# jonassibbesen/rpvg

Measured on AMD Instinct MI355X. Metric: read-pairs quantified/sec, higher is better.
Workload: dtype f64

## Files before the change

include/rpvg_hip.h:

```cpp
#ifndef RPVG_HIP_H
#define RPVG_HIP_H

#include <stdint.h>

#include "rpvg_batch.h"
#include "rpvg_rows.h"
#include "rpvg_index.h"
#include "rpvg_table.h"
#include "rpvg_samples.h"
#include "rpvg_text.h"

#ifdef __cplusplus
extern "C" {
#endif

typedef enum rpvg_hip_status {
    RPVG_HIP_OK = 0,
    RPVG_HIP_ERR_NO_DEVICE = -1,
    RPVG_HIP_ERR_RUNTIME = -2,
    RPVG_HIP_ERR_INVALID = -3,
    RPVG_HIP_ERR_ALLOC = -4,
    RPVG_HIP_ERR_UNSUPPORTED = -5
} rpvg_hip_status;

// ... 354 lines not shown
int rpvg_hip_gibbs_table_view(rpvg_hip_ctx * ctx, rpvg_hip_gibbs_table * table, rpvg_gibbs_table_view * view_out);
int rpvg_hip_gibbs_table_rows(rpvg_hip_ctx * ctx, rpvg_hip_gibbs_table * table, uint64_t first_path, uint64_t num_paths, double * rows_out);
void rpvg_hip_gibbs_table_limits(rpvg_gibbs_table_limits * limits_out);
void rpvg_hip_gibbs_table_free(rpvg_hip_ctx * ctx, rpvg_hip_gibbs_table * table);
int rpvg_hip_gibbs_read_counts_resident(rpvg_hip_ctx * ctx, const rpvg_hip_batch * batch, const rpvg_hip_em_problems * problems,
                                        const double * init_abundances, const double * init_noise_count, const uint32_t * num_samples,
                                        const uint64_t * seeds, uint32_t gibbs_thin_its, double gamma, rpvg_hip_gibbs_samples ** samples_out);
int rpvg_hip_gibbs_samples_get(rpvg_hip_ctx * ctx, const rpvg_hip_gibbs_samples * samples, double * noise_samples, double * abundance_samples);
void rpvg_hip_gibbs_samples_free(rpvg_hip_ctx * ctx, rpvg_hip_gibbs_samples * samples);
int rpvg_hip_gibbs_table_build_resident(rpvg_hip_ctx * ctx, const rpvg_hip_gibbs_samples * samples, const rpvg_hip_em_problems * problems,
                                        uint32_t num_clusters, const uint64_t * cluster_path_off, const double * total_count,
                                        uint32_t num_gibbs_samples, rpvg_hip_gibbs_table ** table_out);

int rpvg_hip_gibbs_table_text(rpvg_hip_ctx * ctx, const rpvg_hip_gibbs_table * table, const rpvg_table_labels * labels, int32_t precision,
                              rpvg_hip_table_text ** text_out);
int rpvg_hip_estimates_table_text(rpvg_hip_ctx * ctx, const rpvg_hip_estimates_table * table, const rpvg_estimates_flat * estimates,
                                  const rpvg_table_labels * labels, int32_t kind, int32_t precision, rpvg_hip_table_text ** text_out);
int rpvg_hip_estimates_set_text(rpvg_hip_ctx * ctx, const rpvg_hip_estimates_table * table, const rpvg_estimates_flat * estimates,
                                const rpvg_table_labels * labels, int32_t kind, uint32_t ploidy, double min_posterior, int32_t precision,
                                rpvg_hip_table_text ** text_out);
int rpvg_hip_table_text_view(rpvg_hip_table_text * text, rpvg_table_text_view * view_out);
int rpvg_hip_table_text_get(rpvg_hip_table_text * text, uint64_t byte_begin, uint64_t byte_end, char * dst);
int rpvg_hip_table_text_guards(rpvg_hip_table_text * text, int32_t * intact_out);
void rpvg_hip_table_text_free(rpvg_hip_table_text * text);

#define RPVG_HIP_COMM_ID_BYTES 128
int rpvg_hip_comm_unique_id(uint8_t * id_out);
int rpvg_hip_comm_init(rpvg_hip_ctx * ctx, const uint8_t * id, int world_size, int rank);
int rpvg_hip_comm_destroy(rpvg_hip_ctx * ctx);
int rpvg_hip_comm_init_all(rpvg_hip_ctx * const * ctxs, int num_contexts);
int rpvg_hip_comm_allreduce_sum_f64(rpvg_hip_ctx * ctx, double * device_buf, uint64_t n);
int rpvg_hip_gather(rpvg_hip_ctx * ctx, const double * local_values, uint64_t local_count, const uint64_t * counts, double * all_values);

int rpvg_hip_synth_dense_cluster(rpvg_hip_ctx * ctx, uint64_t seed, uint64_t num_rows, uint32_t num_paths,
                                 double * device_matrix, uint64_t ld, double * device_counts);
int rpvg_hip_synth_dense_rows(rpvg_hip_ctx * ctx, uint64_t seed, uint64_t row_begin, uint64_t num_rows, uint32_t num_paths,
                              double * device_matrix, uint64_t ld, double * device_counts);

int rpvg_hip_synth_dense_cluster_batch(rpvg_hip_ctx * ctx, uint64_t seed, uint64_t num_rows, uint32_t num_paths,
                                       rpvg_hip_batch ** batch_out);

int rpvg_hip_debug_log(rpvg_hip_ctx * ctx, uint64_t n, const double * x, double * out, int32_t use_table);

#define RPVG_HIP_EM_KERNELS 12
typedef struct rpvg_hip_em_kernel_stats {
    double ms;
    uint64_t launches;
    uint64_t problems;
    uint64_t iterations;
    uint64_t max_iterations;
    double alg_bytes;
} rpvg_hip_em_kernel_stats;
const char * rpvg_hip_em_kernel_name(int index);

typedef struct rpvg_hip_kernel_stats {
    double em_sparse_ms;      uint64_t em_sparse_launches;   double em_sparse_alg_bytes;
    double em_dense_ms;       uint64_t em_dense_launches;    double em_dense_alg_bytes;
    double loglik_ms;         uint64_t loglik_launches;      double loglik_evals;
    double build_ms;          uint64_t build_launches;
    double h2d_ms;            double h2d_bytes;
    uint64_t em_iterations_total;
    double search_pairs_possible; double search_pairs_table; double search_pairs_kept;
    rpvg_hip_em_kernel_stats em_kernel[RPVG_HIP_EM_KERNELS];
    double collapse_ms;
    double busy_ms;
    double gibbs_ms;
    double search_tile_ms;    uint64_t search_tile_launches;
    uint64_t gibbs_calls_completed;
    uint64_t gibbs_count_grid_problems;
    uint64_t gibbs_count_grid_iterations;
    uint64_t cover_grid_problems;
    uint64_t cover_grid_rounds;
    uint64_t text_exact_cells;
    uint64_t nested_full_calls;
    uint64_t nested_full_sets;
    uint64_t nested_full_retained;
} rpvg_hip_kernel_stats;

int rpvg_hip_stats_get(rpvg_hip_ctx * ctx, rpvg_hip_kernel_stats * stats_out);
int rpvg_hip_stats_reset(rpvg_hip_ctx * ctx);
int rpvg_hip_stats_intervals(rpvg_hip_ctx * ctx, uint64_t capacity, double * start_ms, double * stop_ms, int32_t * family,
                             uint64_t * count_out);

#ifdef __cplusplus
}
#endif

#endif
```

rpvg_amd/csrc/bounded_search.hip:

```cpp

#include "common.hpp"
#include "search_plan.hpp"

#include <algorithm>
#include <cstdlib>
#include <map>
#include <memory>
#include <mutex>
#include <numeric>

using namespace rpvg_hip_detail;
using namespace rpvg_search;

namespace {
std::mutex g_search_gate_mutex;
const rpvg_hip_ctx * g_search_gate_owner = nullptr;
}

static bool searchLaunchesEarly() {
    static const bool early = RPVG_EXPERIMENT_ENV("RPVG_HIP_SEARCH_LAUNCH_EARLY") != nullptr;
    return early;
}

constexpr uint64_t kSearchGateRows = 1ull << 17;

static void searchGateEnter(rpvg_hip_ctx * ctx, hipStream_t stream, const uint64_t matrix_rows) {
    static const bool open_gate = RPVG_EXPERIMENT_ENV("RPVG_HIP_NO_SEARCH_GATE") != nullptr;
    ctx->search_gate_held = !open_gate && matrix_rows >= kSearchGateRows;
    if (!ctx->search_gate_held) return;
    hipEvent_t previous = nullptr;
    {
        std::lock_guard<std::mutex> lock(g_search_gate_mutex);
        if (g_search_gate_owner && g_search_gate_owner != ctx && g_search_gate_owner->device == ctx->device) {
            previous = g_search_gate_owner->search_done;
            (void) hipStreamWaitEvent(stream, previous, 0);
        }
    }
    if (previous && !searchLaunchesEarly()) (void) waitEvent(previous);
}

static void searchGateLeave(rpvg_hip_ctx * ctx, hipStream_t stream) {
    if (!ctx->search_gate_held) return;
    ctx->search_gate_held = false;
    std::lock_guard<std::mutex> lock(g_search_gate_mutex);
    (void) hipEventRecord(ctx->search_done, stream);
    g_search_gate_owner = ctx;
}

void searchGateForget(const rpvg_hip_ctx * ctx) {
    std::lock_guard<std::mutex> lock(g_search_gate_mutex);
    if (g_search_gate_owner == ctx) g_search_gate_owner = nullptr;
}

struct rpvg_hip_pair_posteriors {
    std::vector<uint64_t> pair_off;
    void * block = nullptr;
    bool block_pinned = false;
    const uint32_t * first = nullptr, * second = nullptr;
    const double * posterior = nullptr;
    ~rpvg_hip_pair_posteriors() {
        if (block && block_pinned) pinnedFree(block);
        else std::free(block);
    }
};

namespace {

constexpr uint32_t kLdsRows = 2048;
constexpr uint32_t kSmallRowLdsCols = 128;
constexpr uint32_t kRowLdsCols = 512;

__device__ __forceinline__ double waveSum(double v) { return waveSumF64(v); }

__device__ __forceinline__ double addLog(const double log_x, const double log_y) {
    return log_x > log_y ? log_x + log1p(exp(log_y - log_x)) : log_y + log1p(exp(log_x - log_y));
}


template <int kBlock, typename ValueFn>
__device__ __forceinline__ double blockLogSumExp(const uint32_t n, ValueFn value, double * scratch) {
    const double lowest = -1.7976931348623157e308;
    const int lane = threadIdx.x & 63, wave = threadIdx.x >> 6;
    double mx = lowest;
    for (uint32_t k = threadIdx.x; k < n; k += kBlock) mx = fmax(mx, value(k));
#pragma unroll
    for (int d = 32; d >= 1; d >>= 1) mx = fmax(mx, __shfl_xor(mx, d, 64));
    __syncthreads();
    if (lane == 0) scratch[wave] = mx;
    __syncthreads();
#pragma unroll
    for (int w2 = 0; w2 < kBlock / 64; ++w2) mx = fmax(mx, scratch[w2]);
    double sum = 0.0;
    for (uint32_t k = threadIdx.x; k < n; k += kBlock) {
        const double v = value(k);
        if (v > lowest) sum += exp(v - mx);
    }
    sum = waveSum(sum);
    __syncthreads();
    if (lane == 0) scratch[wave] = sum;
    __syncthreads();
    double total = 0.0;
#pragma unroll
    for (int w2 = 0; w2 < kBlock / 64; ++w2) total += scratch[w2];
    return (n == 0 || !(mx > lowest)) ? lowest : mx + log(total);
}

struct SearchArgs {
    const uint32_t * order;
    uint32_t count;
    GroupMatricesView g;
    const uint64_t * col_off;
    const uint32_t * col_count;
    const uint64_t * pair_cap_off;
    double min_log_likelihood_diff;
    uint32_t stage_rows;
    uint32_t row_lds_cols;
    double * log_freq;
    double * marginal;
    double * optimistic_raw;
    double * optimistic;
    uint32_t * col_order;
    uint32_t * out_first;
    uint32_t * out_second;
    double * out_value;
    uint32_t * out_count;
    unsigned long long * log_evals;
};

constexpr int kTileFirst = 4;

template <int kGroup>
__device__ __forceinline__ void tilePairSums(const LogTableEntry * lt, const double * lds_count, const double * lds_base, const uint32_t stride,
                                             const double * __restrict__ cnt, const double * __restrict__ nz,
                                             const double * const (&col_a)[kTileFirst], const double * __restrict__ col_b, const uint32_t staged,
// ... 803 lines not shown
}

int searchFailed(const hipError_t e) {
    setError("rpvg_hip_bounded_pair_posteriors: %s", hipGetErrorString(e));
    return (e == hipErrorOutOfMemory) ? RPVG_HIP_ERR_ALLOC : RPVG_HIP_ERR_RUNTIME;
}

void showSearchClasses(const rpvg_hip_groups * groups, const PairSearchPlan & plan) {
    const std::vector<uint32_t> & order = plan.order;
    const uint32_t M = static_cast<uint32_t>(order.size()), num_big = plan.num_big, num_medium = plan.num_medium;
    auto show = [&](const char * name, uint32_t first, uint32_t count) {
        double evals = 0;
        for (uint32_t i = first; i < first + count; ++i) evals += 0.5 * groups->h_num_rows[order[i]] * groups->h_num_cols[order[i]] * groups->h_num_cols[order[i]];
        std::fprintf(stderr, "[search classes] %-6s %6u matrices, %.3g pair-row evaluations if nothing is skipped; largest:", name, count, evals);
        for (uint32_t i = first; i < first + std::min<uint32_t>(count, 6); ++i) std::fprintf(stderr, " %llux%u", static_cast<unsigned long long>(groups->h_num_rows[order[i]]), groups->h_num_cols[order[i]]);
        std::fprintf(stderr, "\n");
    };
    show("table", 0, num_big);
    if (plan.pair_tiles) {
        struct Bucket { uint64_t matrices = 0; double rows = 0, evals = 0, lane_rows = 0, slot_rows = 0; };
        std::map<uint32_t, Bucket> buckets;
        for (uint32_t i = 0; i < num_big; ++i) {
            const double R = static_cast<double>(groups->h_num_rows[order[i]]);
            const uint32_t G = groups->h_num_cols[order[i]];
            uint32_t key = 1;
            while (key < G) key <<= 1;
            Bucket & b = buckets[key];
            const uint32_t tiles = tileCount(G);
            b.matrices += 1;
            b.rows += R;
            b.evals += R * (0.5 * G * (G + 1));
            std::vector<std::pair<uint32_t, uint32_t> > ranges;
            planTileRanges(tiles, &ranges);
            for (auto & range : ranges) b.lane_rows += R / (kTileBlock / range.second) * kTileBlock;
            b.slot_rows += R * tiles * 16;
        }
        for (auto & kv : buckets) {
            const Bucket & b = kv.second;
            std::fprintf(stderr, "[search classes]   columns <= %4u: %6llu matrices, %9.0f rows, %.3g evaluations, pairs / tile slots %.2f, tile slots / lane slots %.2f\n",
                         kv.first, static_cast<unsigned long long>(b.matrices), b.rows, b.evals, b.evals / b.slot_rows, b.slot_rows / (16.0 * b.lane_rows));
        }
    }
    show("medium", num_big, num_medium);
    show("small", num_big + num_medium, M - num_big - num_medium);
}

unsigned long long * searchLogEvals(const PairSearchWork & w) { return reinterpret_cast<unsigned long long *>(w.d_tail.ptr + w.evals_word); }

hipError_t launchTablePart(rpvg_hip_ctx * ctx, const rpvg_hip_groups * groups, const GroupMatricesView & view, const PairSearchPlan & plan,
                           PairSearchWork & w, const bool runs_behind_search) {
    hipError_t e = hipSuccess;
    auto ok = [&](hipError_t r) { if (e == hipSuccess) e = r; return e == hipSuccess; };
    hipStream_t st = ctx->stream;
    const SearchParts parts = {w.d_part_pair.ptr, w.d_part_marg.ptr, w.d_part_opt.ptr, w.d_big_pair_part_off.ptr, w.d_big_col_part_off.ptr, plan.chunk_rows};
    const uint32_t items = static_cast<uint32_t>(plan.item_matrix.size());
    if (plan.pair_tiles) {
        PairTileWork pw;
        pw.item_matrix = w.d_item_matrix.ptr;
        pw.item_chunk = w.d_item_chunk.ptr;
        pw.item_tiles = w.d_item_col.ptr;
        pw.count = items;
        pw.g = view;
        pw.parts = parts;
        pw.log_evals = searchLogEvals(w);
#ifdef RPVG_HIP_EXPERIMENTS
        pw.debug_skip = RPVG_EXPERIMENT_ENV("RPVG_HIP_PAIR_DEBUG") ? static_cast<uint32_t>(std::atoi(RPVG_EXPERIMENT_ENV("RPVG_HIP_PAIR_DEBUG"))) : 0u;
#endif
        static const size_t tile_lds_bytes = []() {
            const char * env = RPVG_EXPERIMENT_ENV("RPVG_HIP_PAIR_LDS_KB");
            return std::max<size_t>(kTileLdsDoubles * sizeof(double), env ? static_cast<size_t>(std::atoi(env)) * 1024 : 0);
        }();
        if (tile_lds_bytes > 64 * 1024) {
            e = hipFuncSetAttribute(reinterpret_cast<const void *>(&pairTile2Kernel), hipFuncAttributeMaxDynamicSharedMemorySize, static_cast<int>(tile_lds_bytes));
            if (e != hipSuccess) return e;
        }
        const int tile_span = ctx->spanBegin(FAM_TILE, st);
        pairTile2Kernel<<<dim3(pw.count), dim3(kTileBlock), tile_lds_bytes, st>>>(pw);
        ctx->spanEnd(tile_span);
#ifdef RPVG_HIP_EXPERIMENTS
        for (int k = RPVG_EXPERIMENT_ENV("RPVG_HIP_PAIR_REPEAT") ? std::atoi(RPVG_EXPERIMENT_ENV("RPVG_HIP_PAIR_REPEAT")) : 0; k > 0; --k) {
            pairTile2Kernel<<<dim3(pw.count), dim3(kTileBlock), tile_lds_bytes, st>>>(pw);
        }
#endif
    } else {
        TableWork tw;
        tw.item_matrix = w.d_item_matrix.ptr;
        tw.item_col = w.d_item_col.ptr;
        tw.item_chunk = w.d_item_chunk.ptr;
        tw.count = items;
        tw.g = view;
        tw.parts = parts;
        tw.log_evals = searchLogEvals(w);
        pairTableKernel<<<dim3(((tw.count + 7) / 8) * 8), dim3(256), 0, st>>>(tw);
    }
    if (runs_behind_search) {
        if (groups->collapse_done) {
            HostScope wait_scope("search: wait for the runs of the matrices' collapse");
            ok(searchLaunchesEarly() ? hipStreamWaitEvent(st, groups->collapse_done, 0) : waitEvent(groups->collapse_done));
        }
        ok(groups->held_back_runs(st, &parts));
        groups->held_back_runs = nullptr;
    }

    ResolveArgs ra;
    ra.big_matrix = w.d_order.ptr;
    ra.count = plan.num_big;
    ra.g = view;
    ra.col_off = w.d_col_off.ptr;
    ra.col_count = w.d_col_count.ptr;
    ra.pair_cap_off = w.d_pair_cap_off.ptr;
    ra.parts = parts;
    ra.min_log_likelihood_diff = w.min_log_likelihood_diff;
    ra.log_freq = w.d_lf.ptr;
    ra.marginal = w.d_marg.ptr;
    ra.col_order = w.d_col_order.ptr;
    ra.seq_value = w.d_seq.ptr;
    ra.out_first = w.d_out_first.ptr;
    ra.out_second = w.d_out_second.ptr;
    ra.out_value = w.d_out_value.ptr;
    ra.out_count = w.d_tail.ptr;
    resolveTableKernel<<<dim3(plan.num_big), dim3(256), 0, st>>>(ra);
    return e;
}

void launchSequentialParts(rpvg_hip_ctx * ctx, const GroupMatricesView & view, const PairSearchPlan & plan, PairSearchWork & w) {
    static const int search_streams = []() {
        const char * env = RPVG_EXPERIMENT_ENV("RPVG_HIP_SEARCH_STREAMS");
        return env ? std::max(1, std::min(3, std::atoi(env))) : 3;
    }();
    hipStream_t s_medium = search_streams == 1 ? ctx->stream : ctx->aux[0];
    hipStream_t s_small = search_streams == 1 ? ctx->stream : (search_streams == 2 ? ctx->aux[0] : ctx->aux[1]);
    SearchArgs args;
    args.g = view;
    args.col_off = w.d_col_off.ptr;
    args.col_count = w.d_col_count.ptr;
    args.pair_cap_off = w.d_pair_cap_off.ptr;
    args.min_log_likelihood_diff = w.min_log_likelihood_diff;
    args.log_freq = w.d_lf.ptr;
    args.marginal = w.d_marg.ptr;
    args.optimistic_raw = w.d_opt_raw.ptr;
    args.optimistic = w.d_opt.ptr;
    args.col_order = w.d_col_order.ptr;
    args.out_first = w.d_out_first.ptr;
    args.out_second = w.d_out_second.ptr;
    args.out_value = w.d_out_value.ptr;
    args.out_count = w.d_tail.ptr;
    args.log_evals = searchLogEvals(w);
    auto search_lds_bytes = [](uint32_t stage_rows, uint32_t row_cols) { return static_cast<size_t>((kTileFirst + 1) * stage_rows + kTileFirst * row_cols) * sizeof(double); };
    {
        static std::once_flag once;
        std::call_once(once, [&]() {
            (void) hipFuncSetAttribute(reinterpret_cast<const void *>(&boundedSearchKernel<1024, 64>), hipFuncAttributeMaxDynamicSharedMemorySize,
                                       static_cast<int>(search_lds_bytes(kLdsRows, kRowLdsCols)));
        });
    }
    const uint32_t num_small = w.M - plan.num_big - plan.num_medium;
    if (plan.num_medium > 0) {
        args.order = w.d_order.ptr + plan.num_big;
        args.count = plan.num_medium;
        args.stage_rows = kLdsRows;
        args.row_lds_cols = kRowLdsCols;
        boundedSearchKernel<1024, 64><<<dim3(plan.num_medium), dim3(1024), search_lds_bytes(kLdsRows, kRowLdsCols), s_medium>>>(args);
    }
    if (num_small > 0) {
        args.order = w.d_order.ptr + plan.num_big + plan.num_medium;
        args.count = num_small;
// ... 3 lines not shown
    }
}

}

namespace rpvg_hip_detail {

int queuePairSearch(rpvg_hip_ctx * ctx, const rpvg_hip_groups * groups, const uint32_t * column_counts, const double min_rel_likelihood,
                    PairSearchWork & w) {
    std::unique_ptr<HostScope> scope(new HostScope("bounded search: host order + work items"));
    const uint32_t M = groups->num_matrices;
    w.M = M;
    w.min_log_likelihood_diff = std::log(min_rel_likelihood);
    if (!column_counts && M > 0 && !groups->d_column_counts) {
        setError("rpvg_hip_bounded_pair_posteriors: column_counts is NULL");
        return RPVG_HIP_ERR_INVALID;
    }
    const uint64_t num_columns = std::accumulate(groups->h_num_cols.begin(), groups->h_num_cols.begin() + M, uint64_t(0));
    for (uint64_t c = 0; column_counts && c < num_columns; ++c) {
        if (column_counts[c] == 0) {
            setError("rpvg_hip_bounded_pair_posteriors: column %llu has a zero count", static_cast<unsigned long long>(c));
            return RPVG_HIP_ERR_INVALID;
        }
    }
    w.plan = planPairSearch(groups->h_num_rows.data(), groups->h_num_cols.data(), M, min_rel_likelihood, pairSearchKnobs());
    const PairSearchPlan & plan = w.plan;
    if (RPVG_EXPERIMENT_ENV("RPVG_HIP_SEARCH_CLASSES")) showSearchClasses(groups, plan);

    scope.reset(new HostScope("bounded search: uploads + launches"));
    hipError_t e = hipSetDevice(ctx->device);
    hipStream_t st = ctx->stream;
    auto ok = [&](hipError_t r) { if (e == hipSuccess) e = r; return e == hipSuccess; };

    UploadPack & pack = w.pack;
    const uint64_t columns = plan.col_off[M], pair_cap = plan.pair_cap_off[M];
    pack.add(w.d_order, plan.order.data(), M);
    pack.add(w.d_col_off, plan.col_off.data(), M + 1);
    pack.add(w.d_pair_cap_off, plan.pair_cap_off.data(), M + 1);
    if (column_counts) pack.add(w.d_col_count, column_counts, columns);
    if (plan.num_big > 0) {
        pack.add(w.d_item_matrix, plan.item_matrix.data(), plan.item_matrix.size());
        pack.add(w.d_item_col, plan.item_col.data(), plan.item_col.size());
        pack.add(w.d_item_chunk, plan.item_chunk.data(), plan.item_chunk.size());
        pack.add(w.d_big_col_part_off, plan.big_col_part_off.data(), M);
        pack.add(w.d_big_pair_part_off, plan.big_pair_part_off.data(), M);
    }
    w.evals_word = (M + 1) & ~1u;
    w.tail_words = w.evals_word + 4;
    pack.addZero(w.d_tail, w.tail_words);
    if (w.extra_u64_count) pack.add(w.d_extra_u64, w.extra_u64, w.extra_u64_count);
    if (w.extra_zero_bytes) pack.addZero(w.d_extra_zero, w.extra_zero_bytes);
    int span = ctx->spanBegin(FAM_H2D);
    ok(pack.commit(st));
    if (!column_counts) w.d_col_count.borrow(const_cast<uint32_t *>(groups->d_column_counts), columns);
    ctx->spanEnd(span);
    ctx->stats.h2d_bytes += static_cast<double>(M * 20 + columns * 4);
    ok(w.d_lf.alloc(columns));
    ok(w.d_marg.alloc(columns));
    ok(w.d_opt_raw.alloc(columns));
    ok(w.d_opt.alloc(columns));
    ok(w.d_col_order.alloc(columns));
    ok(w.d_out_first.alloc(pair_cap));
    ok(w.d_out_second.alloc(pair_cap));
    ok(w.d_out_value.alloc(pair_cap));
    if (e != hipSuccess) return searchFailed(e);
    if (plan.num_big > 0) {
        ok(w.d_part_marg.alloc(plan.col_part_total));
        ok(w.d_part_opt.alloc(plan.col_part_total));
        ok(w.d_part_pair.alloc(plan.pair_part_total));
        ok(w.d_seq.alloc(pair_cap));
    }
    if (e != hipSuccess) return searchFailed(e);

    const bool side_kernels = M > plan.num_big;
    const bool runs_behind_search = static_cast<bool>(groups->held_back_runs) && plan.pair_tiles && plan.num_big == M;
    if (!runs_behind_search) {
        ok(groups->waitCollapse(st));
        if (groups->collapse_done && !searchLaunchesEarly()) {
            HostScope wait_scope("search: wait for the collapse of the matrices");
            ok(waitEvent(groups->collapse_done));
        }
    }
    span = ctx->spanBegin(FAM_LOGLIK);
    searchGateEnter(ctx, st, std::accumulate(groups->h_num_rows.begin(), groups->h_num_rows.end(), uint64_t(0)));
    if (side_kernels) ok(ctx->forkAux());
    const GroupMatricesView view = groups->view();
    if (plan.num_big > 0) ok(launchTablePart(ctx, groups, view, plan, w, runs_behind_search && e == hipSuccess));
    launchSequentialParts(ctx, view, plan, w);
    if (side_kernels) ok(ctx->joinAux());
    ctx->spanEnd(span);
    ctx->stats.loglik_launches += (plan.num_big > 0 ? 2 : 0) + (plan.num_medium > 0) + (M > plan.num_big + plan.num_medium);
    ok(hipGetLastError());
    if (e != hipSuccess) {
        (void) hipStreamSynchronize(st);
        searchFailed(e);
        return RPVG_HIP_ERR_RUNTIME;
    }
    return RPVG_HIP_OK;
}

void leavePairSearch(rpvg_hip_ctx * ctx) { searchGateLeave(ctx, ctx->stream); }

void accountPairSearch(rpvg_hip_ctx * ctx, const rpvg_hip_groups * groups, const PairSearchWork & w, const unsigned long long log_evals,
                       const uint64_t kept_pairs) {
    ctx->stats.loglik_evals += static_cast<double>(log_evals);
    for (uint32_t i = 0; i < w.M; ++i) {
        const double G = groups->h_num_cols[w.plan.order[i]];
        ctx->stats.search_pairs_possible += G * (G + 1) / 2;
        if (i < w.plan.num_big) ctx->stats.search_pairs_table += G * (G + 1) / 2;
    }
    ctx->stats.search_pairs_kept += static_cast<double>(kept_pairs);
}

}

extern "C" int rpvg_hip_bounded_pair_posteriors(rpvg_hip_ctx * ctx, const rpvg_hip_groups * groups,
                                                const uint32_t * column_counts, double min_rel_likelihood,
                                                rpvg_hip_pair_posteriors ** result_out) {
    RPVG_REQUIRE(ctx && groups && result_out, "rpvg_hip_bounded_pair_posteriors: NULL argument");
    *result_out = nullptr;
    RPVG_REQUIRE(min_rel_likelihood > 0, "rpvg_hip_bounded_pair_posteriors: min_rel_likelihood must be positive");
    const uint32_t M = groups->num_matrices;
    rpvg_hip_pair_posteriors * res = new (std::nothrow) rpvg_hip_pair_posteriors();
    if (!res) {
        setError("rpvg_hip_bounded_pair_posteriors: out of host memory");
        return RPVG_HIP_ERR_ALLOC;
    }
    res->pair_off.assign(M + 1, 0);
    if (M == 0) {
        *result_out = res;
        return RPVG_HIP_OK;
    }
    if (!column_counts && !groups->d_column_counts) {
        delete res;
        setError("rpvg_hip_bounded_pair_posteriors: column_counts is NULL");
        return RPVG_HIP_ERR_INVALID;
    }

    std::lock_guard<std::mutex> lock(ctx->mutex);
    PairSearchWork w;
    {
        const int rc = queuePairSearch(ctx, groups, column_counts, min_rel_likelihood, w);
        if (rc != RPVG_HIP_OK) {
            delete res;
            return rc;
        }
    }
    hipError_t e = hipSuccess;
    hipStream_t st = ctx->stream;
    auto ok = [&](hipError_t r) { if (e == hipSuccess) e = r; return e == hipSuccess; };
    std::unique_ptr<HostScope> scope;
    const std::vector<uint64_t> & pair_cap_off = w.plan.pair_cap_off;
    const uint32_t evals_word = w.evals_word, tail_words = w.tail_words;
    auto & d_tail = w.d_tail; auto & d_pair_cap_off = w.d_pair_cap_off; auto & d_out_first = w.d_out_first;
    auto & d_out_second = w.d_out_second; auto & d_out_value = w.d_out_value;
    DeviceBuffer<uint64_t> d_pair_off;

    const char * with_counts_env = std::getenv("RPVG_HIP_PAIRS_WITH_COUNTS");
    const size_t kPairsWithTheCounts = with_counts_env ? static_cast<size_t>(std::atof(with_counts_env)) : (size_t(1) << 20);
    const size_t tail_bytes = tail_words * sizeof(uint32_t), tail_room = (tail_bytes + 255) & ~size_t(255);
    const size_t block_capacity = static_cast<size_t>(pair_cap_off[M]) * 16;
    const size_t first_copy = tail_room + std::min(block_capacity, kPairsWithTheCounts);
    DeviceBuffer<unsigned char> d_result;
    ok(d_pair_off.alloc(M + 1));
    ok(d_result.alloc(tail_room + block_capacity));
    void * host_result = nullptr;
    if (e == hipSuccess && pinnedAlloc(&host_result, first_copy) != hipSuccess) e = hipErrorOutOfMemory;
    if (e == hipSuccess) {
        const bool check_build = !groups->build_checked && groups->build_error_flag.ptr;
        pairOffsetsKernel<<<dim3(1), dim3(1024), 0, st>>>(M, d_tail.ptr, d_pair_off.ptr, check_build ? groups->build_error_flag.ptr : nullptr,
                                                         d_tail.ptr + evals_word + 2, reinterpret_cast<uint32_t *>(d_result.ptr), tail_words);
        compactPairsBlockKernel<<<dim3(M), dim3(64), 0, st>>>(M, d_pair_cap_off.ptr, d_pair_off.ptr, d_out_first.ptr, d_out_second.ptr,
                                                             d_out_value.ptr, d_result.ptr + tail_room);
        ok(hipGetLastError());
        ok(hipMemcpyAsync(host_result, d_result.ptr, first_copy, hipMemcpyDeviceToHost, st));
    }
    searchGateLeave(ctx, st);
    scope.reset(new HostScope("bounded search: wait for the kernels"));
    ok(waitStream(st));
    if (e == hipSuccess) {
        const uint32_t * counts = static_cast<const uint32_t *>(host_result);
        unsigned long long log_evals = 0;
        std::memcpy(&log_evals, counts + evals_word, sizeof(log_evals));
        const uint32_t build_bad = counts[evals_word + 2];
        for (uint32_t m = 0; m < M; ++m) res->pair_off[m + 1] = res->pair_off[m] + counts[m];
        if (build_bad) {
            pinnedFree(host_result);
            delete res;
            setError(build_bad == 2 ? "rpvg_hip_groups_build: a group lists a path twice" : "rpvg_hip_groups_build: a group refers to a path outside its cluster");
            return RPVG_HIP_ERR_INVALID;
        }
        groups->build_checked = true;
        const uint64_t total = res->pair_off[M];
        const unsigned char * pairs = nullptr;
        if (total * 16 <= first_copy - tail_room) {
            res->block = host_result;
            res->block_pinned = true;
            host_result = nullptr;
            pairs = static_cast<const unsigned char *>(res->block) + tail_room;
        } else {
            scope.reset(new HostScope("bounded search: download pairs"));
            if (pinnedAlloc(&res->block, total * 16) == hipSuccess) {
                res->block_pinned = true;
            } else {
                res->block = std::malloc(total * 16);
                if (!res->block) e = hipErrorOutOfMemory;
            }
            if (e == hipSuccess) {
                ok(hipMemcpyAsync(res->block, d_result.ptr + tail_room, total * 16, hipMemcpyDeviceToHost, st));
                ok(waitStream(st));
                pairs = static_cast<const unsigned char *>(res->block);
            }
        }
        if (e == hipSuccess) {
            res->posterior = reinterpret_cast<const double *>(pairs);
            res->first = reinterpret_cast<const uint32_t *>(pairs + total * sizeof(double));
            res->second = res->first + total;
        }
        accountPairSearch(ctx, groups, w, log_evals, total);
    }
    if (host_result) pinnedFree(host_result);
    if (e != hipSuccess) {
        delete res;
// ... 18 lines not shown
```

rpvg_amd/csrc/common.hpp:

```cpp
#ifndef RPVG_HIP_COMMON_HPP
#define RPVG_HIP_COMMON_HPP

#include <hip/hip_runtime.h>

#include <algorithm>
#include <chrono>
#include <cstdarg>
#include <cstdint>
#include <cstdio>
#include <cstdlib>
#include <cstring>
#include <memory>
#include <mutex>
#include <new>
#include <string>
#include <functional>
#include <vector>

#include "../../include/rpvg_hip.h"
#include "search_plan.hpp"
#include "em_plan.hpp"
#include "batch_forms.hpp"

namespace rpvg_hip_detail {

void setError(const char * fmt, ...);

#define RPVG_HIP_CHECK(expr)                                                                                  \
    do {                                                                                                      \
        hipError_t err__ = (expr);                                                                            \
        if (err__ != hipSuccess) {                                                                            \
            rpvg_hip_detail::setError("%s failed at %s:%d: %s", #expr, __FILE__, __LINE__, hipGetErrorString(err__)); \
               \
            (void) hipDeviceSynchronize();                                                                    \
            return RPVG_HIP_ERR_RUNTIME;                                                                      \
        }                                                                                                     \
    } while (0)

#define RPVG_REQUIRE(cond, ...)                       \
    do {                                              \
        if (!(cond)) {                                \
            rpvg_hip_detail::setError(__VA_ARGS__);   \
            return RPVG_HIP_ERR_INVALID;              \
        }                                             \
    } while (0)

#ifdef RPVG_HIP_EXPERIMENTS
#define RPVG_EXPERIMENT_ENV(name) std::getenv(name)
#else
#define RPVG_EXPERIMENT_ENV(name) (static_cast<const char *>(nullptr))
#endif

int hardwareQueues();

hipError_t waitEvent(hipEvent_t event);
hipError_t waitStream(hipStream_t stream);

hipError_t zeroAsync(void * ptr, size_t bytes, hipStream_t stream);

hipError_t poolAlloc(void ** ptr, size_t bytes);
void poolFree(void * ptr);
void poolTrim(int device);

hipError_t pinnedAlloc(void ** ptr, size_t bytes);
void pinnedFree(void * ptr);
size_t pinnedCapacity(const void * ptr);
void pinnedTrim();
bool stagedUploads();
bool hostIsPinned(const void * host, size_t bytes);
void copyToStaging(void * staging, const void * host, size_t bytes);
void registerCopyStream(hipStream_t stream, hipStream_t copy_stream, hipEvent_t copied);
void forgetCopyStream(hipStream_t stream);
hipError_t stagedCopy(void * device_dst, const void * pinned_src, size_t bytes, hipStream_t stream);

template <typename T>
struct DeviceBuffer {
    T * ptr = nullptr;
    size_t count = 0;
    void * staging = nullptr;
    bool borrowed = false;
    DeviceBuffer() {}
    DeviceBuffer(const DeviceBuffer &) = delete;
    DeviceBuffer & operator=(const DeviceBuffer &) = delete;
    ~DeviceBuffer() { release(); }
    void release() {
        if (ptr && !borrowed) poolFree(ptr);
        if (staging) pinnedFree(staging);
        ptr = nullptr;
        staging = nullptr;
        count = 0;
        borrowed = false;
    }
    hipError_t alloc(size_t n) {
        release();
        count = n;
        if (n == 0) return hipSuccess;
        return poolAlloc(reinterpret_cast<void **>(&ptr), n * sizeof(T));
    }
    void borrow(T * p, size_t n) {
        release();
        ptr = n ? p : nullptr;
        count = n;
        borrowed = true;
// ... 309 lines not shown
                                                  LogProduct (&pr)[kOut], double (&acc)[kOut]) {
    constexpr uint32_t kSegment = kGroup * kFoldFactors;
    for (IndexT seg = begin; seg < fast_end; seg += kSegment) {
        const IndexT seg_end = (fast_end - seg) < kSegment ? fast_end : seg + kSegment;
        for (IndexT i = seg + lane; i < seg_end; i += kGroup) {
            double xs[kOut];
            x(i, xs);
#pragma unroll
            for (int t = 0; t < kOut; ++t) pr[t].mul(xs[t]);
        }
#pragma unroll
        for (int t = 0; t < kOut; ++t) pr[t].fold();
    }
    for (IndexT i = (begin < fast_end ? fast_end : begin) + lane; i < mid_end; i += kGroup) {
        double xs[kOut];
        x(i, xs);
        const int c = static_cast<int>(cnt[i]);
        for (int k = 0; k < c; ++k) {
#pragma unroll
            for (int t = 0; t < kOut; ++t) pr[t].mul(xs[t]);
        }
#pragma unroll
        for (int t = 0; t < kOut; ++t) pr[t].fold();
    }
    for (IndexT i = (begin < mid_end ? mid_end : begin) + lane; i < end; i += kGroup) {
        double xs[kOut];
        x(i, xs);
        const double c = cnt[i];
#pragma unroll
        for (int t = 0; t < kOut; ++t) acc[t] = fma(c, logPositive(xs[t], lt), acc[t]);
    }
}

constexpr int kCollapseKeyFractionBits = 22;
constexpr int kCollapseProjectionBits = kCollapseKeyFractionBits + 2;
constexpr int kCollapseLargestBits = 20;
constexpr int kCollapseLargestFractionBits = 27;
constexpr int kCollapseMatrixShift = kCollapseProjectionBits + kCollapseLargestBits;
constexpr uint32_t kCollapseMaxMatrices = 1u << 20;

__host__ __device__ inline double collapseWeight(const uint32_t column) {
    return static_cast<double>(((column * 0x9E3779B1u) >> 8) & 0xFFFFu) * (1.0 / 32768.0);
}

__host__ __device__ inline uint64_t collapseSortKey(const uint32_t matrix, const double key, const double largest) {
    const double k = key < 0.0 ? 0.0 : (key > 3.999999 ? 3.999999 : key);
    const double l = largest < 0.0 ? 0.0 : (largest > 0.999999 ? 0.999999 : largest);
    return (static_cast<uint64_t>(matrix) << kCollapseMatrixShift) |
           (static_cast<uint64_t>(k * static_cast<double>(1ull << kCollapseKeyFractionBits)) << kCollapseLargestBits) |
           (static_cast<uint64_t>(l * static_cast<double>(1ull << kCollapseLargestFractionBits)) & ((1ull << kCollapseLargestBits) - 1));
}

__device__ __forceinline__ double mulRounded(const double a, const double b) {
#pragma clang fp contract(off)
    return a * b;
}
__device__ __forceinline__ double addRounded(const double a, const double b) {
#pragma clang fp contract(off)
    return a + b;
}

template <int BLOCK>
__device__ __forceinline__ uint32_t blockExclusiveSum(const uint32_t v, uint32_t & total, uint32_t * scratch) {
    const int lane = threadIdx.x & 63, wave = threadIdx.x >> 6;
    uint32_t incl = v;
#pragma unroll
    for (int d = 1; d < 64; d <<= 1) {
        const uint32_t up = __shfl_up(incl, d, 64);
        if (lane >= d) incl += up;
    }
    __syncthreads();
    if (lane == 63) scratch[wave] = incl;
    __syncthreads();
    uint32_t before = 0, all = 0;
#pragma unroll
    for (int w = 0; w < BLOCK / 64; ++w) {
        if (w < wave) before += scratch[w];
        all += scratch[w];
    }
    total = all;
    return before + incl - v;
}

enum KernelFamily { FAM_EM_SPARSE = 0, FAM_EM_DENSE, FAM_LOGLIK, FAM_BUILD, FAM_H2D, FAM_COLLAPSE, FAM_EM_KERNEL, FAM_GIBBS, FAM_TILE, FAM_COUNT };

struct TimedSpan {
    hipEvent_t start, stop;
    int family;
    int sub;
};

struct TimedInterval {
    double start_ms, stop_ms;
    int family;
    uint64_t clock;
};

}

namespace rpvg_hip_detail {
struct SubsetEmHints {
    double subsets_per_matrix = 0, list_per_path = 0, rows_per_row = 0, entries_per_entry = 0;
    bool retry = false;
    unsigned long long retry_subsets = 0, retry_list_length = 0, retry_rows = 0, retry_entries = 0;
};
}

struct rpvg_hip_ctx {
    static constexpr int kAuxStreams = 6;
    rpvg_hip_detail::SubsetEmHints subset_hints;
    rpvg_hip_detail::SubsetEmHints subset_full_hints;
    bool search_gate_held = false;
    int device = 0;
    hipStream_t stream = nullptr;
    hipStream_t aux[kAuxStreams] = {};
    int aux_count = kAuxStreams;
    hipStream_t grid_stream[2] = {nullptr, nullptr};
    hipEvent_t grid_ready = nullptr;
    hipStream_t collapse_stream = nullptr;
    hipStream_t copy_stream = nullptr;
    hipEvent_t copied = nullptr;
    hipEvent_t fork_event = nullptr;
    hipEvent_t search_done = nullptr;
    hipEvent_t join_event[kAuxStreams] = {};
    hipError_t forkAux();
    hipError_t joinAux();
    hipError_t joinAuxOnHost();
    hipDeviceProp_t props;
    std::mutex mutex;
    void * comm = nullptr;
    int comm_world = 1, comm_rank = 0;
    int allReduceSumF64(double * device_buf, uint64_t n);
    std::vector<rpvg_hip_detail::TimedSpan> spans;
    std::vector<hipStream_t> span_streams;
    int span_level = 2;
    int open_spans = 0;
    void accountSpan(const rpvg_hip_detail::TimedSpan & span, const void * clock_base, uint64_t clock_id);
    void foldFinishedSpans();
    std::vector<rpvg_hip_detail::TimedInterval> intervals;
    rpvg_hip_kernel_stats stats;
    rpvg_hip_independent_stats independent_stats{};
    rpvg_hip_detail::SubsetEmHints subset_independent_hints;

    int spanBegin(int family, hipStream_t on = nullptr, int sub = -1);
    void spanEnd(int idx);
    int foldSpans();
};

namespace rpvg_hip_detail {
struct PathSourcesPending {
    DeviceBuffer<uint64_t> d_path_source_off;
    DeviceBuffer<uint32_t> d_source_id, d_sizes;
    DeviceBuffer<uint16_t> d_source_id16;
    DeviceBuffer<unsigned long long> d_arena;
    unsigned long long arena_words = 0, num_sources = 0, num_sources_narrow = 0;
    void * h_sizes = nullptr;
    uint32_t K = 0;
    bool copied = false, queued = false;
    ~PathSourcesPending() { if (h_sizes) pinnedFree(h_sizes); }
};
}

struct rpvg_hip_batch {
    uint32_t num_clusters = 0;
    uint64_t num_rows = 0, num_entries = 0, num_paths = 0;
    std::vector<uint64_t> h_cluster_row_off, h_cluster_path_off, h_cluster_ent_off;
    rpvg_hip_detail::DeviceBuffer<uint64_t> cluster_row_off;
    rpvg_hip_detail::DeviceBuffer<uint64_t> cluster_path_off;
    rpvg_hip_detail::DeviceBuffer<double> row_count;
    rpvg_hip_detail::DeviceBuffer<double> row_noise;
    rpvg_hip_detail::DeviceBuffer<uint64_t> row_ent_off;
    rpvg_hip_detail::DeviceBuffer<uint32_t> ent_path;
    rpvg_hip_detail::DeviceBuffer<double> ent_prob;
    std::vector<double> h_cluster_total;
    bool has_source_columns = false;
    rpvg_hip_detail::DeviceBuffer<uint32_t> path_group_id;
    rpvg_hip_detail::DeviceBuffer<uint64_t> cluster_src_off;
    rpvg_hip_detail::DeviceBuffer<uint32_t> src_col_count;
    rpvg_hip_detail::DeviceBuffer<uint32_t> src_col_end;
    rpvg_hip_detail::DeviceBuffer<uint32_t> src_col_path;
    std::vector<uint64_t> h_cluster_src_off;
    std::vector<uint32_t> h_src_num_cols, h_src_col_paths, h_src_max_col_paths;
    struct UploadInProgress {
        rpvg_batch_forms::BatchForms forms;
        rpvg_hip_detail::DeviceBuffer<uint32_t> d_row_count_u32, d_row_grp_off32, d_grp_idx_off32;
        rpvg_hip_detail::DeviceBuffer<uint64_t> d_row_grp_off, d_grp_idx_off;
        rpvg_hip_detail::DeviceBuffer<double> d_grp_prob;
        rpvg_hip_detail::DeviceBuffer<uint8_t> d_row_grp_count8, d_grp_idx_count8;
        rpvg_hip_detail::DeviceBuffer<uint16_t> d_path_idx16, d_row_noise16;
        rpvg_hip_detail::DeviceBuffer<double> d_row_noise_table;
        rpvg_hip_detail::DeviceBuffer<uint8_t> d_row_count8;
        rpvg_hip_detail::DeviceBuffer<uint32_t> d_escape_row, d_escape_count;
        rpvg_hip_detail::PathSourcesPending path_sources;
        rpvg_hip_detail::DeviceBuffer<unsigned long long> d_first_bad_row;
        rpvg_hip_detail::DeviceBuffer<double> d_cluster_total;
        rpvg_hip_detail::DeviceBuffer<uint64_t> d_cluster_ent_off;
        rpvg_hip_detail::DeviceBuffer<unsigned char> scan_scratch_rows, scan_scratch_groups;
        void * h_results = nullptr;
        hipEvent_t finished = nullptr;
        ~UploadInProgress() {
            if (finished) {
                (void) hipEventSynchronize(finished);
                (void) hipEventDestroy(finished);
            }
            if (h_results) rpvg_hip_detail::pinnedFree(h_results);
        }
    };
    std::unique_ptr<UploadInProgress> upload;
};

void searchGateForget(const rpvg_hip_ctx * ctx);

struct GroupMatrix {
    const double * values, * rowmax, * row_count, * row_noise;
    uint64_t R, fast_end, mid_end;
    uint32_t G;
};
struct GroupMatricesView {
    const uint64_t * mat_val_off;
    const uint64_t * mat_row_off;
    const uint32_t * mat_fast;
    const uint32_t * mat_mid;
    const uint64_t * mat_rows;
    const uint32_t * mat_cols;
// ... 206 lines not shown
    uint32_t rows, entries;
    uint32_t merged, pad;
    uint64_t row_base, ent_base, col_begin;
    double total_mass, zero_mass;
};

struct EmGridStorage {
    EmProblemsView problems;
    double * abundances;
    double * noise_count;
    uint32_t * iterations;
    const EmFusedDense * fused = nullptr;
    uint32_t num_fused = 0;
};

uint64_t emGridMinWork();
uint64_t gibbsGridMinWork();
bool emGridDenseRoute(uint32_t columns, uint32_t rows, uint32_t entries);
int runEmGridProblems(rpvg_hip_ctx * ctx, hipStream_t st, const EmGridProblem * problems, uint32_t count, const EmGridStorage & storage,
                      uint32_t max_em_its, double max_rel_em_conv);

struct GibbsGridProblem {
    uint32_t problem, columns;
    uint32_t rows, entries;
    uint32_t num_samples, pad;
    uint64_t col_begin;
    uint64_t sample_off, abund_sample_off;
    uint64_t seed;
};
struct GibbsGridStorage {
    EmProblemsView problems;
    const double * init_abundances;
    const double * init_noise_count;
    double * noise_samples;
    double * abundance_samples;
};
int runGibbsGridProblems(rpvg_hip_ctx * ctx, hipStream_t st, const GibbsGridProblem * problems, uint32_t count, const GibbsGridStorage & storage,
                         uint32_t gibbs_thin_its, double gamma);

struct DenseEmRun {
    const double * matrix = nullptr;
    uint64_t num_rows = 0;
    uint32_t num_cols = 0;
    uint64_t ld = 0;
    const double * counts = nullptr;
    double total_count = 0, zero_mass = 0;
    uint32_t max_em_its = 0;
    double max_rel_em_conv = 0;
    bool sharded = false;
    DeviceBuffer<double> d_a;
    EmGridControl control = {};
};
int emDenseIterate(rpvg_hip_ctx * ctx, const char * who, DenseEmRun & run);

int queueEmSolve(rpvg_hip_ctx * ctx, const rpvg_hip_batch * batch, const EmProblemList & list, uint32_t max_em_its,
                 double max_rel_em_conv, const EmOutputs & out, EmSolveWork & work, double collapse_precision = 0.0);
EmSolveKnobs emSolveKnobs();
int queueEmFill(rpvg_hip_ctx * ctx, const rpvg_hip_batch * batch, const EmProblemList & list, const EmOutputs & out, EmSolveWork & work,
                const EmSolveKnobs & knobs, const EmFillPlan & plan, bool fused_look, int & build_span);
EmSolveShape emSolveShape(const rpvg_hip_ctx * ctx, const EmProblemList & list, bool collapse_wanted);

struct HostProblemSet {
    EmProblemList list;
    EmSolveWork work;
    DeviceBuffer<uint32_t> d_cluster, d_col_path, d_item_problem;
    DeviceBuffer<uint64_t> d_col_off, d_row_base, d_ent_base, d_seg_first;
    UploadPack uploads;
    uint64_t n_cols_total = 0;
};
int prepareHostProblems(rpvg_hip_ctx * ctx, const rpvg_hip_batch * batch, const rpvg_hip_em_problems * problems,
                        HostProblemSet & ps, const EmOutputs & out, const char * who);
void accountEmSolve(rpvg_hip_ctx * ctx, uint32_t P, const uint64_t * col_off, const uint32_t * kept_rows, const uint32_t * kept_entries,
                    const uint32_t * iterations);

struct PairSearchWork {
    uint32_t M = 0, evals_word = 0, tail_words = 0;
    double min_log_likelihood_diff = 0;
    rpvg_search::PairSearchPlan plan;
    DeviceBuffer<uint32_t> d_order, d_col_count, d_col_order, d_out_first, d_out_second, d_item_matrix, d_item_col, d_item_chunk;
    DeviceBuffer<uint32_t> d_tail;
    DeviceBuffer<uint64_t> d_col_off, d_pair_cap_off, d_big_col_part_off, d_big_pair_part_off;
    DeviceBuffer<double> d_lf, d_marg, d_opt_raw, d_opt, d_out_value, d_part_marg, d_part_opt, d_part_pair, d_seq;
    UploadPack pack;
    const uint64_t * extra_u64 = nullptr;
    size_t extra_u64_count = 0, extra_zero_bytes = 0;
    DeviceBuffer<uint64_t> d_extra_u64;
    DeviceBuffer<unsigned char> d_extra_zero;
};
int queuePairSearch(rpvg_hip_ctx * ctx, const rpvg_hip_groups * groups, const uint32_t * column_counts, double min_rel_likelihood,
                    PairSearchWork & w);
void leavePairSearch(rpvg_hip_ctx * ctx);
void accountPairSearch(rpvg_hip_ctx * ctx, const rpvg_hip_groups * groups, const PairSearchWork & w, unsigned long long log_evals, uint64_t kept_pairs);

struct CsrCollapseInput {
    uint32_t num_problems_bound = 0;
    const uint32_t * num_problems_dev = nullptr;
    uint64_t rows_capacity = 0;
    EmProblemsView problems;
    uint32_t num_items_bound = 0;
    const uint32_t * num_items_dev = nullptr;
    const uint64_t * seg_first = nullptr;
    const uint32_t * item_problem = nullptr;
    uint32_t segment_rows = 0;
    uint64_t max_rows_bound = 0;
};
struct CsrCollapseWork {
    DeviceBuffer<double> merged_count;
    DeviceBuffer<uint32_t> problem_merged;
    DeviceBuffer<uint32_t> info;
    std::shared_ptr<void> temporaries;
};
hipError_t queueCsrCollapse(rpvg_hip_ctx * ctx, const CsrCollapseInput & in, double precision, CsrCollapseWork & work, hipStream_t stream,
                            hipEvent_t sorted = nullptr);

std::unique_ptr<rpvg_hip_batch> newBatchShell(uint32_t num_clusters, uint64_t num_rows, uint64_t num_entries, uint64_t num_paths, hipError_t & e);
struct GroupedRows {
    uint64_t num_groups = 0;
    const void * row_grp_off = nullptr;
    const void * grp_idx_off = nullptr;
    bool row_off32 = false, grp_off32 = false;
    const double * grp_prob = nullptr;
    const uint32_t * row_count_u32 = nullptr;
};
hipError_t queueGroupedRows(hipStream_t stream, const GroupedRows & rows, rpvg_hip_batch * b, unsigned long long * d_first_bad_row, uint64_t * d_cluster_ent_off);

hipError_t queueClusterTotals(hipStream_t stream, uint32_t num_clusters, const uint64_t * d_cluster_row_off, const uint32_t * d_row_count_u32, double * d_totals);
hipError_t queuePathSourceCopies(rpvg_hip_ctx * ctx, rpvg_hip_batch * b, const rpvg_cluster_batch * hb, PathSourcesPending & pending);
hipError_t queuePathSourceKernels(rpvg_hip_ctx * ctx, rpvg_hip_batch * b, PathSourcesPending & pending, hipStream_t stream);
hipError_t reservePathSources(rpvg_hip_batch * b, uint32_t num_clusters, uint64_t num_paths, uint64_t num_sources, PathSourcesPending & pending);
int finishPathSources(rpvg_hip_batch * b, PathSourcesPending & pending);

hipError_t queueRowCollapse(rpvg_hip_ctx * ctx, rpvg_hip_groups * groups, uint64_t total_rows, double precision, hipStream_t stream, bool hold_back_runs = false);
}

#endif
```

rpvg_amd/csrc/context.hip:

```cpp

#include "common.hpp"

#include <sys/prctl.h>
#include <time.h>

#include <algorithm>
#include <thread>

#include <map>

namespace rpvg_hip_detail {

static thread_local char g_last_error[1024] = "";

void setError(const char * fmt, ...) {
    va_list ap;
    va_start(ap, fmt);
    vsnprintf(g_last_error, sizeof(g_last_error), fmt, ap);
    va_end(ap);
}

namespace {

struct DevicePool {
// ... 290 lines not shown

hipError_t rpvg_hip_ctx::joinAux() {
    hipError_t e = hipSuccess;
    for (int i = 0; i < aux_count && e == hipSuccess; ++i) {
        e = hipEventRecord(join_event[i], aux[i]);
        if (e == hipSuccess) e = hipStreamWaitEvent(stream, join_event[i], 0);
    }
    return e;
}

hipError_t rpvg_hip_ctx::joinAuxOnHost() {
    hipError_t e = hipSuccess;
    for (int i = 0; i < aux_count && e == hipSuccess; ++i) e = hipEventRecord(join_event[i], aux[i]);
    for (int i = 0; i < aux_count && e == hipSuccess; ++i) e = rpvg_hip_detail::waitEvent(join_event[i]);
    for (int i = 0; i < aux_count && e == hipSuccess; ++i) e = hipStreamWaitEvent(stream, join_event[i], 0);
    return e;
}

namespace rpvg_hip_detail {
namespace {
struct DeviceClock {
    hipEvent_t base = nullptr;
    uint64_t id = 0;
    std::chrono::steady_clock::time_point taken;
};
std::mutex g_clock_mutex;
std::map<int, DeviceClock> g_clocks;

DeviceClock deviceClock(const int device, hipStream_t stream, const bool renew_if_old) {
    std::lock_guard<std::mutex> lock(g_clock_mutex);
    DeviceClock & clock = g_clocks[device];
    const auto now = std::chrono::steady_clock::now();
    if (!clock.base || (renew_if_old && now - clock.taken > std::chrono::seconds(5))) {
        hipEvent_t base = nullptr;
        if (hipEventCreate(&base) == hipSuccess && hipEventRecord(base, stream) == hipSuccess && hipEventSynchronize(base) == hipSuccess) {
            clock.base = base;
            clock.id++;
            clock.taken = now;
        }
    }
    return clock;
}
}
}

int rpvg_hip_ctx::spanBegin(int family, hipStream_t on, int sub) {
    if (span_level <= 0 || (span_level == 1 && family != FAM_EM_KERNEL)) return -1;
    if (open_spans == 0 && spans.size() >= 1024) foldFinishedSpans();
    TimedSpan s;
    s.family = family;
    s.sub = sub;
    if (hipEventCreate(&s.start) != hipSuccess) return -1;
    if (hipEventCreate(&s.stop) != hipSuccess) {
        (void) hipEventDestroy(s.start);
        return -1;
    }
    if (!on) on = stream;
    (void) hipEventRecord(s.start, on);
    spans.push_back(s);
    span_streams.push_back(on);
    ++open_spans;
    return static_cast<int>(spans.size()) - 1;
}

void rpvg_hip_ctx::spanEnd(int idx) {
    if (idx < 0) return;
    (void) hipEventRecord(spans[idx].stop, span_streams[idx]);
    if (open_spans > 0) --open_spans;
}

void rpvg_hip_ctx::accountSpan(const rpvg_hip_detail::TimedSpan & s, const void * clock_base, const uint64_t clock_id) {
    constexpr size_t kMaxIntervals = 1u << 20;
    float ms = 0;
    if (hipEventElapsedTime(&ms, s.start, s.stop) != hipSuccess) return;
    switch (s.family) {
        case FAM_EM_SPARSE: stats.em_sparse_ms += ms; break;
        case FAM_EM_DENSE: stats.em_dense_ms += ms; break;
        case FAM_LOGLIK: stats.loglik_ms += ms; break;
        case FAM_BUILD: stats.build_ms += ms; break;
        case FAM_H2D: stats.h2d_ms += ms; break;
        case FAM_COLLAPSE: stats.collapse_ms += ms; break;
        case FAM_GIBBS: stats.gibbs_ms += ms; break;
        case FAM_TILE: stats.search_tile_ms += ms; stats.search_tile_launches += 1; break;
        case FAM_EM_KERNEL:
            if (s.sub >= 0 && s.sub < RPVG_HIP_EM_KERNELS) stats.em_kernel[s.sub].ms += ms;
            break;
        default: break;
    }
    float at = 0;
    hipEvent_t base = static_cast<hipEvent_t>(const_cast<void *>(clock_base));
    if (s.family != FAM_EM_KERNEL && s.family != FAM_GIBBS && base && intervals.size() < kMaxIntervals &&
        hipEventElapsedTime(&at, base, s.start) == hipSuccess) {
        intervals.push_back(TimedInterval{static_cast<double>(at), static_cast<double>(at) + ms, s.family, clock_id});
    }
}

void rpvg_hip_ctx::foldFinishedSpans() {
    const DeviceClock clock = deviceClock(device, stream, false);
    size_t kept = 0;
    for (size_t i = 0; i < spans.size(); ++i) {
        if (hipEventQuery(spans[i].stop) == hipSuccess) {
            accountSpan(spans[i], clock.base, clock.id);
            (void) hipEventDestroy(spans[i].start);
            (void) hipEventDestroy(spans[i].stop);
        } else {
            (void) hipGetLastError();
            spans[kept] = spans[i];
            span_streams[kept] = span_streams[i];
            ++kept;
        }
    }
    (void) hipGetLastError();
    spans.resize(kept);
    span_streams.resize(kept);
}

int rpvg_hip_ctx::foldSpans() {
    RPVG_HIP_CHECK(hipStreamSynchronize(stream));
    if (collapse_stream) RPVG_HIP_CHECK(hipStreamSynchronize(collapse_stream));
    const DeviceClock clock = deviceClock(device, stream, false);
    for (auto & s : spans) {
        (void) hipEventSynchronize(s.stop);
        accountSpan(s, clock.base, clock.id);
        (void) hipGetLastError();
        (void) hipEventDestroy(s.start);
        (void) hipEventDestroy(s.stop);
    }
    spans.clear();
    span_streams.clear();
    open_spans = 0;
    std::vector<std::pair<double, double>> iv;
    for (auto & t : intervals) {
        if (t.clock == clock.id) iv.emplace_back(t.start_ms, t.stop_ms);
    }
    std::sort(iv.begin(), iv.end());
    double busy = 0, cur_s = 0, cur_e = -1;
    for (auto & x : iv) {
        if (cur_e < cur_s || x.first > cur_e) {
            if (cur_e >= cur_s) busy += cur_e - cur_s;
            cur_s = x.first;
            cur_e = x.second;
        } else if (x.second > cur_e) {
            cur_e = x.second;
        }
    }
    if (cur_e >= cur_s) busy += cur_e - cur_s;
    stats.busy_ms = busy;
    return RPVG_HIP_OK;
}

extern "C" {

int rpvg_hip_device_count(int * count) {
    RPVG_REQUIRE(count != nullptr, "rpvg_hip_device_count: count is NULL");
    int n = 0;
    hipError_t e = hipGetDeviceCount(&n);
    if (e != hipSuccess) {
        setError("hipGetDeviceCount failed: %s", hipGetErrorString(e));
        *count = 0;
        return RPVG_HIP_ERR_NO_DEVICE;
    }
    *count = n;
    return RPVG_HIP_OK;
}

namespace {
hipError_t createMainStream(hipStream_t * stream, const bool highest_priority) {
    const char * env = RPVG_EXPERIMENT_ENV("RPVG_HIP_MAIN_PRIORITY");
    if (!highest_priority && (!env || std::atoi(env) == 0)) return hipStreamCreateWithFlags(stream, hipStreamNonBlocking);
    int least = 0, greatest = 0;
    if (hipDeviceGetStreamPriorityRange(&least, &greatest) != hipSuccess || least == greatest) {
        (void) hipGetLastError();
        return hipStreamCreateWithFlags(stream, hipStreamNonBlocking);
    }
    return hipStreamCreateWithPriority(stream, hipStreamNonBlocking, greatest);
}

bool ownQueueForMainStream(const bool uploader, const int side_streams) {
    static const bool pooled = std::getenv("RPVG_HIP_POOLED_MAIN_QUEUE") != nullptr && std::atoi(std::getenv("RPVG_HIP_POOLED_MAIN_QUEUE")) != 0;
    return !uploader && side_streams < rpvg_hip_ctx::kAuxStreams && !pooled;
}

hipError_t createOwnQueueStream(hipStream_t * stream, const int num_cus) {
    uint32_t every_cu[32];
    for (uint32_t & word : every_cu) word = 0xffffffffu;
    const uint32_t words = static_cast<uint32_t>(std::min(32, std::max(1, (num_cus + 31) / 32)));
    hipError_t e = hipExtStreamCreateWithCUMask(stream, words, every_cu);
    if (e != hipSuccess) {
        (void) hipGetLastError();
        e = hipStreamCreateWithFlags(stream, hipStreamNonBlocking);
    }
    return e;
}

int createContext(int device, bool uploader, int side_streams, rpvg_hip_ctx ** ctx_out);
}

int rpvg_hip_create(int device, rpvg_hip_ctx ** ctx_out) { return createContext(device, false, rpvg_hip_ctx::kAuxStreams, ctx_out); }

int rpvg_hip_create_uploader(int device, rpvg_hip_ctx ** ctx_out) { return createContext(device, true, 1, ctx_out); }

int rpvg_hip_create_with_streams(int device, int side_streams, rpvg_hip_ctx ** ctx_out) {
    RPVG_REQUIRE(side_streams >= 1 && side_streams <= rpvg_hip_ctx::kAuxStreams, "rpvg_hip_create_with_streams: 1 to %d side streams", rpvg_hip_ctx::kAuxStreams);
    return createContext(device, false, side_streams, ctx_out);
}

namespace {
int createContext(int device, const bool uploader, const int side_streams, rpvg_hip_ctx ** ctx_out) {
    RPVG_REQUIRE(ctx_out != nullptr, "rpvg_hip_create: ctx_out is NULL");
    *ctx_out = nullptr;
    int n = 0;
    hipError_t e = hipGetDeviceCount(&n);
    if (e != hipSuccess || n <= 0) {
        setError("rpvg_hip_create: no HIP device available (%s); this engine has no CPU fallback",
                 e != hipSuccess ? hipGetErrorString(e) : "device count is 0");
        return RPVG_HIP_ERR_NO_DEVICE;
    }
    RPVG_REQUIRE(device >= 0 && device < n, "rpvg_hip_create: device %d out of range [0, %d)", device, n);
    rpvg_hip_ctx * ctx = new (std::nothrow) rpvg_hip_ctx();
    if (!ctx) {
        setError("rpvg_hip_create: out of host memory");
        return RPVG_HIP_ERR_ALLOC;
    }
    ctx->device = device;
    memset(&ctx->stats, 0, sizeof(ctx->stats));
    {
        const char * env = std::getenv("RPVG_HIP_SPANS");
        ctx->span_level = env ? std::max(0, std::min(2, std::atoi(env))) : ((uploader || side_streams < rpvg_hip_ctx::kAuxStreams) ? 1 : 2);
    }
    if ((e = hipSetDevice(device)) != hipSuccess || (e = hipGetDeviceProperties(&ctx->props, device)) != hipSuccess ||
        (e = ownQueueForMainStream(uploader, side_streams) ? createOwnQueueStream(&ctx->stream, ctx->props.multiProcessorCount) : createMainStream(&ctx->stream, uploader)) != hipSuccess) {
        setError("rpvg_hip_create: %s", hipGetErrorString(e));
        delete ctx;
        return RPVG_HIP_ERR_RUNTIME;
    }
    ctx->aux_count = side_streams;
    for (int i = 0; i < rpvg_hip_ctx::kAuxStreams && e == hipSuccess; ++i) {
        if (i < side_streams) {
            e = hipStreamCreateWithFlags(&ctx->aux[i], hipStreamNonBlocking);
            if (e == hipSuccess) e = hipEventCreateWithFlags(&ctx->join_event[i], hipEventDisableTiming);
        } else {
            ctx->aux[i] = ctx->aux[i % side_streams];
        }
    }
    if (e == hipSuccess) e = createMainStream(&ctx->collapse_stream, RPVG_EXPERIMENT_ENV("RPVG_HIP_COLLAPSE_PRIORITY") == nullptr || std::atoi(RPVG_EXPERIMENT_ENV("RPVG_HIP_COLLAPSE_PRIORITY")) != 0);
    if (e == hipSuccess) e = hipEventCreateWithFlags(&ctx->fork_event, hipEventDisableTiming);
    if (e == hipSuccess) e = hipEventCreateWithFlags(&ctx->search_done, hipEventDisableTiming);
    if (e == hipSuccess) e = hipStreamCreateWithFlags(&ctx->copy_stream, hipStreamNonBlocking);
    if (e == hipSuccess) e = hipEventCreateWithFlags(&ctx->copied, hipEventDisableTiming);
    if (e == hipSuccess) {
        registerCopyStream(ctx->stream, ctx->copy_stream, ctx->copied);
        for (int i = 0; i < ctx->aux_count; ++i) registerCopyStream(ctx->aux[i], ctx->copy_stream, ctx->copied);
    }
    if (e != hipSuccess) {
        setError("rpvg_hip_create: %s", hipGetErrorString(e));
        delete ctx;
        return RPVG_HIP_ERR_RUNTIME;
    }
    if (strncmp(ctx->props.gcnArchName, "gfx950", 6) != 0) {
        setError("rpvg_hip_create: device %d is %s; this library is built for gfx950 only", device, ctx->props.gcnArchName);
        (void) hipStreamDestroy(ctx->stream);
        delete ctx;
        return RPVG_HIP_ERR_NO_DEVICE;
    }
    {
        std::lock_guard<std::mutex> lock(g_pool_mutex);
        g_device_contexts[device]++;
    }
    *ctx_out = ctx;
    return RPVG_HIP_OK;
}
}

void rpvg_hip_destroy(rpvg_hip_ctx * ctx) {
    if (!ctx) return;
    const bool trace = std::getenv("RPVG_AMD_TRACE_EXIT") != nullptr;
#define RPVG_EXIT_STEP(what) do { if (trace) std::fprintf(stderr, "[exit]   rpvg_hip_destroy: %s\n", what); } while (0)
    RPVG_EXIT_STEP("begin");
    (void) hipSetDevice(ctx->device);
    (void) ctx->foldSpans();
    RPVG_EXIT_STEP("spans folded");
    (void) rpvg_hip_comm_destroy(ctx);
    if (ctx->stream) forgetCopyStream(ctx->stream);
    for (int i = 0; i < ctx->aux_count; ++i) {
        if (ctx->aux[i]) forgetCopyStream(ctx->aux[i]);
    }
    if (ctx->copy_stream) {
        (void) hipStreamSynchronize(ctx->copy_stream);
        (void) hipStreamDestroy(ctx->copy_stream);
    }
    RPVG_EXIT_STEP("copy stream destroyed");
    if (ctx->copied) (void) hipEventDestroy(ctx->copied);
    if (ctx->stream) (void) hipStreamSynchronize(ctx->stream);
    for (int i = 0; i < ctx->aux_count; ++i) {
        if (ctx->aux[i]) (void) hipStreamSynchronize(ctx->aux[i]);
    }
    if (ctx->collapse_stream) (void) hipStreamSynchronize(ctx->collapse_stream);
    RPVG_EXIT_STEP("streams drained");
    for (int i = 0; i < ctx->aux_count; ++i) {
        if (ctx->aux[i]) (void) hipStreamDestroy(ctx->aux[i]);
        RPVG_EXIT_STEP("a side stream destroyed");
        if (ctx->join_event[i]) (void) hipEventDestroy(ctx->join_event[i]);
    }
    if (ctx->collapse_stream) (void) hipStreamDestroy(ctx->collapse_stream);
    RPVG_EXIT_STEP("side and collapse streams destroyed");
    if (ctx->stream) (void) hipStreamDestroy(ctx->stream);
    RPVG_EXIT_STEP("main stream destroyed");
    if (ctx->fork_event) (void) hipEventDestroy(ctx->fork_event);
    for (hipStream_t grid_stream : ctx->grid_stream) {
        if (grid_stream) {
            (void) hipStreamSynchronize(grid_stream);
            (void) hipStreamDestroy(grid_stream);
        }
    }
    if (ctx->grid_ready) (void) hipEventDestroy(ctx->grid_ready);
    searchGateForget(ctx);
    if (ctx->search_done) (void) hipEventDestroy(ctx->search_done);
    bool last = false;
    {
        std::lock_guard<std::mutex> lock(g_pool_mutex);
        last = (--g_device_contexts[ctx->device] <= 0);
    }
    RPVG_EXIT_STEP("events destroyed");
    if (last) {
        poolTrim(ctx->device);
        RPVG_EXIT_STEP("pool trimmed");
        bool any = false;
        {
            std::lock_guard<std::mutex> lock(g_pool_mutex);
            for (auto & kv : g_device_contexts) any = any || kv.second > 0;
        }
        if (!any) pinnedTrim();
        RPVG_EXIT_STEP("pinned blocks trimmed");
    }
    delete ctx;
    RPVG_EXIT_STEP("done");
#undef RPVG_EXIT_STEP
}

const char * rpvg_hip_last_error(void) { return g_last_error; }

int rpvg_hip_synchronize(rpvg_hip_ctx * ctx) {
    RPVG_REQUIRE(ctx != nullptr, "rpvg_hip_synchronize: ctx is NULL");
    std::lock_guard<std::mutex> lock(ctx->mutex);
    RPVG_HIP_CHECK(hipSetDevice(ctx->device));
    RPVG_HIP_CHECK(hipStreamSynchronize(ctx->stream));
    if (ctx->collapse_stream) RPVG_HIP_CHECK(hipStreamSynchronize(ctx->collapse_stream));
    return RPVG_HIP_OK;
}

int rpvg_hip_device_info(rpvg_hip_ctx * ctx, char * name, uint32_t name_cap, uint32_t * num_cus, uint64_t * mem_bytes) {
    RPVG_REQUIRE(ctx != nullptr, "rpvg_hip_device_info: ctx is NULL");
    if (name && name_cap) {
        snprintf(name, name_cap, "%s (%s)", ctx->props.name, ctx->props.gcnArchName);
    }
    if (num_cus) *num_cus = ctx->props.multiProcessorCount;
    if (mem_bytes) *mem_bytes = ctx->props.totalGlobalMem;
    return RPVG_HIP_OK;
}

int rpvg_hip_malloc(rpvg_hip_ctx * ctx, uint64_t bytes, void ** device_ptr_out) {
    RPVG_REQUIRE(ctx != nullptr && device_ptr_out != nullptr, "rpvg_hip_malloc: NULL argument");
    std::lock_guard<std::mutex> lock(ctx->mutex);
    RPVG_HIP_CHECK(hipSetDevice(ctx->device));
    hipError_t e = hipMalloc(device_ptr_out, bytes);
    if (e != hipSuccess) {
        setError("rpvg_hip_malloc: %llu bytes: %s", static_cast<unsigned long long>(bytes), hipGetErrorString(e));
        return RPVG_HIP_ERR_ALLOC;
    }
    return RPVG_HIP_OK;
}

int rpvg_hip_free(rpvg_hip_ctx * ctx, void * device_ptr) {
    RPVG_REQUIRE(ctx != nullptr, "rpvg_hip_free: ctx is NULL");
    std::lock_guard<std::mutex> lock(ctx->mutex);
    RPVG_HIP_CHECK(hipSetDevice(ctx->device));
    RPVG_HIP_CHECK(hipStreamSynchronize(ctx->stream));
    RPVG_HIP_CHECK(hipFree(device_ptr));
    return RPVG_HIP_OK;
}

int rpvg_hip_memcpy_h2d(rpvg_hip_ctx * ctx, void * device_dst, const void * host_src, uint64_t bytes) {
    RPVG_REQUIRE(ctx != nullptr, "rpvg_hip_memcpy_h2d: ctx is NULL");
    std::lock_guard<std::mutex> lock(ctx->mutex);
    RPVG_HIP_CHECK(hipSetDevice(ctx->device));
    RPVG_HIP_CHECK(hipMemcpyAsync(device_dst, host_src, bytes, hipMemcpyHostToDevice, ctx->stream));
    RPVG_HIP_CHECK(hipStreamSynchronize(ctx->stream));
    return RPVG_HIP_OK;
}

int rpvg_hip_memcpy_d2h(rpvg_hip_ctx * ctx, void * host_dst, const void * device_src, uint64_t bytes) {
    RPVG_REQUIRE(ctx != nullptr, "rpvg_hip_memcpy_d2h: ctx is NULL");
    std::lock_guard<std::mutex> lock(ctx->mutex);
    RPVG_HIP_CHECK(hipSetDevice(ctx->device));
    RPVG_HIP_CHECK(hipMemcpyAsync(host_dst, device_src, bytes, hipMemcpyDeviceToHost, ctx->stream));
    RPVG_HIP_CHECK(hipStreamSynchronize(ctx->stream));
    return RPVG_HIP_OK;
}

extern "C" int rpvg_hip_host_register(void * host, uint64_t bytes) {
    RPVG_REQUIRE(host && bytes > 0, "rpvg_hip_host_register: NULL or empty range");
    RPVG_HIP_CHECK(hipHostRegister(host, bytes, hipHostRegisterDefault));
    std::lock_guard<std::mutex> lock(g_registered_mutex);
    g_registered[static_cast<const char *>(host)] = bytes;
    return RPVG_HIP_OK;
}

extern "C" int rpvg_hip_host_unregister(void * host) {
    RPVG_REQUIRE(host, "rpvg_hip_host_unregister: NULL");
    {
        std::lock_guard<std::mutex> lock(g_registered_mutex);
        RPVG_REQUIRE(g_registered.erase(static_cast<const char *>(host)) == 1, "rpvg_hip_host_unregister: the range was not registered here");
    }
    RPVG_HIP_CHECK(hipHostUnregister(host));
    return RPVG_HIP_OK;
}

void rpvg_hip_thread_wait_spin_us(uint32_t microseconds) { t_spin_us = microseconds; }

int rpvg_hip_pinned_alloc(uint64_t bytes, void ** host_out) {
    RPVG_REQUIRE(host_out != nullptr, "rpvg_hip_pinned_alloc: host_out is NULL");
    *host_out = nullptr;
    const hipError_t e = pinnedAlloc(host_out, std::max<uint64_t>(bytes, 8));
    if (e != hipSuccess) {
        setError("rpvg_hip_pinned_alloc: %llu bytes: %s", static_cast<unsigned long long>(bytes), hipGetErrorString(e));
        return RPVG_HIP_ERR_ALLOC;
    }
    return RPVG_HIP_OK;
}

void rpvg_hip_pinned_free(void * host) { pinnedFree(host); }

int rpvg_hip_stats_get(rpvg_hip_ctx * ctx, rpvg_hip_kernel_stats * stats_out) {
    RPVG_REQUIRE(ctx != nullptr && stats_out != nullptr, "rpvg_hip_stats_get: NULL argument");
    std::lock_guard<std::mutex> lock(ctx->mutex);
    RPVG_HIP_CHECK(hipSetDevice(ctx->device));
    int rc = ctx->foldSpans();
    if (rc != RPVG_HIP_OK) return rc;
    *stats_out = ctx->stats;
    return RPVG_HIP_OK;
}

int rpvg_hip_stats_reset(rpvg_hip_ctx * ctx) {
    RPVG_REQUIRE(ctx != nullptr, "rpvg_hip_stats_reset: ctx is NULL");
    std::lock_guard<std::mutex> lock(ctx->mutex);
    RPVG_HIP_CHECK(hipSetDevice(ctx->device));
    int rc = ctx->foldSpans();
    if (rc != RPVG_HIP_OK) return rc;
    memset(&ctx->stats, 0, sizeof(ctx->stats));
    ctx->independent_stats = rpvg_hip_independent_stats{};
    ctx->intervals.clear();
    (void) deviceClock(ctx->device, ctx->stream, true);
    return RPVG_HIP_OK;
}

int rpvg_hip_stats_intervals(rpvg_hip_ctx * ctx, uint64_t capacity, double * start_ms, double * stop_ms, int32_t * family,
                             uint64_t * count_out) {
    RPVG_REQUIRE(ctx != nullptr && count_out != nullptr, "rpvg_hip_stats_intervals: NULL argument");
    std::lock_guard<std::mutex> lock(ctx->mutex);
    RPVG_HIP_CHECK(hipSetDevice(ctx->device));
    int rc = ctx->foldSpans();
    if (rc != RPVG_HIP_OK) return rc;
    const DeviceClock clock = deviceClock(ctx->device, ctx->stream, false);
    uint64_t n = 0;
    for (auto & t : ctx->intervals) {
        if (t.clock != clock.id) continue;
        if (n < capacity) {
            if (start_ms) start_ms[n] = t.start_ms;
            if (stop_ms) stop_ms[n] = t.stop_ms;
            if (family) family[n] = t.family;
        }
        ++n;
    }
    *count_out = n;
    return RPVG_HIP_OK;
}

}
```

rpvg_amd/csrc/subset_em.hip:

```cpp

#include "common.hpp"
#include "subset_pack.hpp"

#include <cmath>
#include <memory>

using namespace rpvg_hip_detail;

namespace {

constexpr uint32_t kMaxSelected = 1024;

struct MergedList {
    const uint32_t * a;
    const uint32_t * b;
    uint32_t na, nb, i, j;
    __device__ __forceinline__ MergedList(const uint32_t * a_in, uint32_t na_in, const uint32_t * b_in, uint32_t nb_in)
        : a(a_in), b(b_in), na(na_in), nb(nb_in), i(0), j(0) {}
    __device__ __forceinline__ bool done() const { return i >= na && j >= nb; }
    __device__ __forceinline__ uint32_t next() {
        if (j >= nb || (i < na && a[i] <= b[j])) return a[i++];
        return b[j++];
    }
};
// ... 472 lines not shown
    }
    if (tid == 0) set_count[m] = Q;
}

}


static int nestedSubsetEmAttempt(rpvg_hip_ctx * ctx, const rpvg_hip_batch * batch, const rpvg_hip_groups * groups,
                                 const uint32_t * column_counts, double min_rel_likelihood, double min_hap_prob,
                                 uint32_t max_em_its, double max_rel_em_conv, double collapse_precision,
                                 rpvg_hip_subset_em ** result_out, bool * did_not_fit, PairSearchWork & search, const bool second_attempt) {
    *did_not_fit = false;
    RPVG_REQUIRE(min_rel_likelihood > 0, "rpvg_hip_nested_subset_em: min_rel_likelihood must be positive");
    RPVG_REQUIRE(max_em_its > 0, "rpvg_hip_nested_subset_em: max_em_its must be positive");
    RPVG_REQUIRE(groups->batch == batch, "rpvg_hip_nested_subset_em: the matrices were built on another batch");
    const uint32_t M = groups->num_matrices;
    RPVG_REQUIRE(M == 0 || column_counts || groups->d_column_counts, "rpvg_hip_nested_subset_em: column_counts is NULL");
    std::unique_ptr<rpvg_hip_subset_em> res(new (std::nothrow) rpvg_hip_subset_em());
    if (!res) {
        setError("rpvg_hip_nested_subset_em: out of host memory");
        return RPVG_HIP_ERR_ALLOC;
    }
    res->num_matrices = M;

    const bool disabled = std::getenv("RPVG_HIP_NO_DEVICE_SUBSETS") != nullptr;
    if (disabled || !(min_hap_prob * kMaxSelected >= 1.0)) {
        setError("rpvg_hip_nested_subset_em: not taken (min_hap_prob %g admits more than %u subsets per cluster, or RPVG_HIP_NO_DEVICE_SUBSETS)",
                 min_hap_prob, kMaxSelected);
        return RPVG_HIP_ERR_UNSUPPORTED;
    }
    std::unique_ptr<HostScope> scope(new HostScope("subset em: bounds"));
    uint64_t slots = 0, lane_rows = 0, lane_entries = 0, lane_paths = 0, max_cluster_work = 0;
    uint32_t max_paths = 0;
    std::vector<uint64_t> slot_off(M + 1, 0);
    for (uint32_t m = 0; m < M; ++m) {
        const uint64_t G = groups->h_num_cols[m];
        slot_off[m + 1] = slot_off[m] + std::min<uint64_t>(G * (G + 1) / 2, kMaxSelected);
        const uint32_t k = groups->h_cluster[m];
        lane_rows += batch->h_cluster_row_off[k + 1] - batch->h_cluster_row_off[k];
        lane_entries += batch->h_cluster_ent_off[k + 1] - batch->h_cluster_ent_off[k];
        lane_paths += groups->h_num_paths[m];
        max_paths = std::max(max_paths, groups->h_num_paths[m]);
        max_cluster_work = std::max<uint64_t>(max_cluster_work, (batch->h_cluster_row_off[k + 1] - batch->h_cluster_row_off[k]) +
                                                                    (batch->h_cluster_ent_off[k + 1] - batch->h_cluster_ent_off[k]));
    }
    slots = slot_off[M];
    if (M > 0 && 8ull * (5ull * (static_cast<uint64_t>(max_paths) + 1) + 6) > 156 * 1024) {
        setError("rpvg_hip_nested_subset_em: not taken (a cluster with %u paths: EM vectors in global memory)", max_paths);
        return RPVG_HIP_ERR_UNSUPPORTED;
    }

    std::lock_guard<std::mutex> lock(ctx->mutex);
    RPVG_HIP_CHECK(hipSetDevice(ctx->device));
    hipStream_t st = ctx->stream;
    if (M == 0) {
        *result_out = res.release();
        return RPVG_HIP_OK;
    }
    SubsetEmHints & hints = ctx->subset_hints;
    auto planned = [](const double per_unit, const unsigned long long units, const double headroom) {
        return static_cast<unsigned long long>(std::ceil(per_unit * headroom * static_cast<double>(units)));
    };
    unsigned long long cap_subsets = std::min<unsigned long long>(slots, hints.subsets_per_matrix > 0 ? planned(hints.subsets_per_matrix, M, 1.25) + 256 : std::max<unsigned long long>(8ull * M, 16384));
    unsigned long long cap_length = std::max<unsigned long long>(planned(hints.list_per_path, lane_paths, 2.0), std::max<unsigned long long>(8 * lane_paths, 1u << 20));
    unsigned long long cap_rows = hints.rows_per_row > 0 ? planned(hints.rows_per_row, lane_rows, 1.25) + 65536 : 8 * lane_rows;
    unsigned long long cap_entries = hints.entries_per_entry > 0 ? planned(hints.entries_per_entry, lane_entries, 1.25) + 65536 : 8 * lane_entries;
    if (hints.retry) {
        cap_subsets = std::min<unsigned long long>(slots, std::max(cap_subsets, hints.retry_subsets + 64));
        cap_length = std::max(cap_length, hints.retry_list_length + 64);
        cap_rows = std::max(cap_rows, hints.retry_rows + 64);
        cap_entries = std::max(cap_entries, hints.retry_entries + 64);
        hints.retry = false;
    }
    const unsigned long long cap_columns = cap_length;
    const unsigned long long cap_items = cap_rows / emFillSegmentRows() + cap_subsets;

    scope.reset(new HostScope("subset em: search + kernels queued"));
    const size_t header_room = 256;
    int rc = RPVG_HIP_OK;
    if (!second_attempt) {
        search.extra_u64 = slot_off.data();
        search.extra_u64_count = M + 1;
        search.extra_zero_bytes = header_room + emQueuesBytes();
        rc = queuePairSearch(ctx, groups, column_counts, min_rel_likelihood, search);
        if (rc != RPVG_HIP_OK) return rc;
    } else {
        const hipError_t zeroed = zeroAsync(search.d_extra_zero.ptr, search.extra_zero_bytes, st);
        if (zeroed != hipSuccess) {
            setError("rpvg_hip_nested_subset_em: %s", hipGetErrorString(zeroed));
            return RPVG_HIP_ERR_RUNTIME;
        }
    }

    hipError_t e = hipSuccess;
    auto ok = [&](hipError_t r) { if (e == hipSuccess) e = r; return e == hipSuccess; };
    const uint64_t * d_slot_off = search.d_extra_u64.ptr;
    SubsetHeader * header = reinterpret_cast<SubsetHeader *>(search.d_extra_zero.ptr);
    static_assert(sizeof(SubsetHeader) <= 256, "room for the header");
    DeviceBuffer<uint32_t> d_slot_first, d_slot_second, d_slot_length, d_slot_columns;
    DeviceBuffer<double> d_slot_weight;
    DeviceBuffer<unsigned char> d_totals, d_bases, d_packed;
    ok(d_slot_first.alloc(slots));
    ok(d_slot_second.alloc(slots));
    ok(d_slot_length.alloc(slots));
    ok(d_slot_columns.alloc(slots));
    ok(d_slot_weight.alloc(slots));
    ok(d_totals.alloc(sizeof(MatrixTotals) * M));
    ok(d_bases.alloc(sizeof(MatrixTotals) * M));
    DeviceBuffer<uint32_t> d_big_matrices;
    ok(d_big_matrices.alloc(M));
    DeviceBuffer<uint32_t> d_sub_cluster, d_path, d_col_path, d_iters, d_kept_rows, d_kept_entries;
    DeviceBuffer<double> d_sub_weight, d_abund, d_noise, d_total;
    DeviceBuffer<uint64_t> d_path_off, d_col_off, d_row_base, d_ent_base, d_subset_off, d_seg_first;
    DeviceBuffer<uint32_t> d_item_problem;
    ok(d_sub_cluster.alloc(cap_subsets));
    ok(d_sub_weight.alloc(cap_subsets));
    ok(d_path_off.alloc(cap_subsets + 1));
    ok(d_col_off.alloc(cap_subsets + 1));
    ok(d_row_base.alloc(cap_subsets));
    ok(d_ent_base.alloc(cap_subsets));
    ok(d_subset_off.alloc(M + 1));
    ok(d_seg_first.alloc(cap_subsets + 1));
    ok(d_item_problem.alloc(cap_items));
    ok(d_path.alloc(cap_length));
    ok(d_col_path.alloc(cap_columns));
    ok(d_abund.alloc(cap_columns));
    ok(d_noise.alloc(cap_subsets));
    ok(d_total.alloc(cap_subsets));
    ok(d_iters.alloc(cap_subsets));
    ok(d_kept_rows.alloc(cap_subsets));
    ok(d_kept_entries.alloc(cap_subsets));
    const size_t packed_capacity = packedLayout(M, cap_subsets, cap_length, cap_columns).bytes;
    ok(d_packed.alloc(packed_capacity));
    const bool merge_here = batch->path_group_id.ptr != nullptr && max_paths < (1u << kMergePathBits) - 2;
    DeviceBuffer<unsigned long long> d_merge_key;
    DeviceBuffer<uint32_t> d_merge_pos;
    DeviceBuffer<double> d_merge_a0, d_merge_a1;
    if (merge_here) {
        ok(d_merge_key.alloc(2 * cap_length + 2));
        ok(d_merge_pos.alloc(2 * cap_length + 2));
        ok(d_merge_a0.alloc(cap_length));
        ok(d_merge_a1.alloc(cap_length));
    }
    void * pinned_header = nullptr;
    if (e == hipSuccess && pinnedAlloc(&pinned_header, sizeof(SubsetHeader)) != hipSuccess) e = hipErrorOutOfMemory;
    hipEvent_t header_here = nullptr;
    if (e == hipSuccess) ok(hipEventCreateWithFlags(&header_here, hipEventDisableTiming));
    if (e != hipSuccess) {
        setError("rpvg_hip_nested_subset_em: %s", hipGetErrorString(e));
        (void) hipStreamSynchronize(st);
        leavePairSearch(ctx);
        if (pinned_header) pinnedFree(pinned_header);
        if (header_here) (void) hipEventDestroy(header_here);
        return (e == hipErrorOutOfMemory) ? RPVG_HIP_ERR_ALLOC : RPVG_HIP_ERR_RUNTIME;
    }
    MatrixTotals * totals = reinterpret_cast<MatrixTotals *>(d_totals.ptr);
    MatrixTotals * bases = reinterpret_cast<MatrixTotals *>(d_bases.ptr);

    std::unique_ptr<HostScope> part_scope(new HostScope("subset em: select + offsets + expand queued"));
    int span = ctx->spanBegin(FAM_BUILD);
    SelectArgs sa;
    sa.num_matrices = M;
    sa.pair_count = search.d_tail.ptr;
    sa.pair_cap_off = search.d_pair_cap_off.ptr;
    sa.pair_first = search.d_out_first.ptr;
    sa.pair_second = search.d_out_second.ptr;
    sa.pair_value = search.d_out_value.ptr;
    sa.group_off = groups->d_group_off;
    sa.group_path_off = groups->d_group_path_off;
    sa.group_path = groups->d_group_path;
    sa.cluster = groups->d_cluster;
    sa.mat_rows = groups->mat_rows.ptr;
    sa.cluster_row_off = batch->cluster_row_off.ptr;
    sa.row_ent_off = batch->row_ent_off.ptr;
    sa.slot_off = d_slot_off;
    sa.min_hap_prob = min_hap_prob;
    sa.segment_rows = emFillSegmentRows();
    sa.slot_first = d_slot_first.ptr;
    sa.slot_second = d_slot_second.ptr;
    sa.slot_weight = d_slot_weight.ptr;
    sa.slot_length = d_slot_length.ptr;
    sa.slot_columns = d_slot_columns.ptr;
    sa.totals = totals;
    sa.header = header;
    sa.big_matrices = d_big_matrices.ptr;
    subsetSelectSmallKernel<<<dim3(M), dim3(64), 0, st>>>(sa);
    subsetSelectWideKernel<<<dim3(std::min<uint32_t>(M, 128)), dim3(256), 0, st>>>(sa);
    const bool check_build = !groups->build_checked && groups->build_error_flag.ptr;
    OffsetsArgs oa;
    oa.pair_count = search.d_tail.ptr;
    oa.log_evals = reinterpret_cast<const unsigned long long *>(search.d_tail.ptr + search.evals_word);
    oa.build_error = check_build ? groups->build_error_flag.ptr : nullptr;
    oa.num_matrices = M;
    oa.totals = totals;
    oa.bases = bases;
    oa.header = header;
    oa.cap_subsets = cap_subsets;
    oa.cap_length = cap_length;
    oa.cap_columns = cap_columns;
    oa.cap_rows = cap_rows;
    oa.cap_entries = cap_entries;
    oa.cap_items = cap_items;
    oa.seg_first = d_seg_first.ptr;
    oa.path_off = d_path_off.ptr;
    oa.col_off = d_col_off.ptr;
    subsetOffsetsKernel<<<dim3(1), dim3(1024), 0, st>>>(oa);
    SubsetHeader * h_header = static_cast<SubsetHeader *>(pinned_header);
    ok(hipMemcpyAsync(h_header, header, sizeof(SubsetHeader), hipMemcpyDeviceToHost, st));
    ok(hipEventRecord(header_here, st));
    ExpandArgs ea;
    ea.num_matrices = M;
    ea.header = header;
    ea.totals = totals;
    ea.bases = bases;
    ea.slot_off = d_slot_off;
    ea.slot_first = d_slot_first.ptr;
    ea.slot_second = d_slot_second.ptr;
    ea.slot_weight = d_slot_weight.ptr;
    ea.slot_length = d_slot_length.ptr;
    ea.slot_columns = d_slot_columns.ptr;
    ea.group_off = groups->d_group_off;
    ea.group_path_off = groups->d_group_path_off;
    ea.group_path = groups->d_group_path;
    ea.cluster = groups->d_cluster;
    ea.cluster_row_off = batch->cluster_row_off.ptr;
    ea.row_ent_off = batch->row_ent_off.ptr;
    ea.sub_cluster = d_sub_cluster.ptr;
    ea.sub_weight = d_sub_weight.ptr;
    ea.path_off = d_path_off.ptr;
    ea.path = d_path.ptr;
    ea.col_off = d_col_off.ptr;
    ea.col_path = d_col_path.ptr;
    ea.row_base = d_row_base.ptr;
    ea.ent_base = d_ent_base.ptr;
    ea.seg_first = d_seg_first.ptr;
    ea.item_problem = d_item_problem.ptr;
    ea.segment_rows = emFillSegmentRows();
    ea.subset_off = d_subset_off.ptr;
    subsetExpandKernel<<<dim3(M), dim3(256), 0, st>>>(ea);
    ok(hipGetLastError());
    ctx->spanEnd(span);
    ctx->stats.build_launches += 4;
    leavePairSearch(ctx);

    part_scope.reset();
    EmProblemList list;
    list.P_bound = static_cast<uint32_t>(std::min<unsigned long long>(cap_subsets, 0xfffffffeull));
    list.d_num_problems = &header->num_problems;
    list.d_cluster = d_sub_cluster.ptr;
    list.d_col_off = d_col_off.ptr;
    list.d_col_path = d_col_path.ptr;
    list.d_row_base = d_row_base.ptr;
    list.d_ent_base = d_ent_base.ptr;
    list.rows_capacity = cap_rows;
    list.entries_capacity = cap_entries;
    list.d_seg_first = d_seg_first.ptr;
    list.d_item_problem = d_item_problem.ptr;
    list.items_bound = static_cast<uint32_t>(std::min<unsigned long long>(cap_items, 0xfffffffeull));
    list.d_num_items = &header->num_items;
    list.max_cols = max_paths + 1;
    list.max_cluster_paths = max_paths;
    list.max_cluster_work = max_cluster_work;
    list.wide_capacity = 0;
    EmOutputs out{d_abund.ptr, d_noise.ptr, d_iters.ptr, d_kept_rows.ptr, d_kept_entries.ptr, d_total.ptr};
    EmSolveWork work;
    work.zeroed_queues = search.d_extra_zero.ptr + header_room;
    if (e == hipSuccess) {
        rc = queueEmSolve(ctx, batch, list, max_em_its, max_rel_em_conv, out, work, collapse_precision);
        if (rc != RPVG_HIP_OK) {
            (void) hipStreamSynchronize(st);
            (void) hipEventDestroy(header_here);
            pinnedFree(pinned_header);
            return rc;
        }
    }
    part_scope.reset(new HostScope("subset em: merge + pack queued"));
    static_assert(sizeof(SubsetHeader) <= 192, "the merge's flag word sits behind the header");
    uint32_t * d_merge_bad = reinterpret_cast<uint32_t *>(search.d_extra_zero.ptr + 192);
    if (merge_here && e == hipSuccess) {
        MergeArgs ma;
        ma.header = header;
        ma.num_matrices = M;
        ma.subset_off = d_subset_off.ptr;
        ma.weight = d_sub_weight.ptr;
        ma.path_off = d_path_off.ptr;
        ma.path = d_path.ptr;
        ma.col_off = d_col_off.ptr;
        ma.col_path = d_col_path.ptr;
        ma.abundances = d_abund.ptr;
        ma.noise = d_noise.ptr;
        ma.total = d_total.ptr;
        ma.cluster = groups->d_cluster;
        ma.cluster_path_off = batch->cluster_path_off.ptr;
        ma.path_group_id = batch->path_group_id.ptr;
        ma.sort_key = d_merge_key.ptr;
        ma.sort_pos = d_merge_pos.ptr;
        ma.rec_a0 = d_merge_a0.ptr;
        ma.rec_a1 = d_merge_a1.ptr;
        ma.merge_bad = d_merge_bad;
        ma.packed = d_packed.ptr;
        const int merge_span = ctx->spanBegin(FAM_BUILD);
        subsetMergeKernel<<<dim3(M), dim3(256), 0, st>>>(ma);
        ctx->spanEnd(merge_span);
        ctx->stats.build_launches += 1;
    }
    PackArgs pa;
    pa.merge_bad = merge_here ? d_merge_bad : nullptr;
    pa.header = header;
    pa.num_matrices = M;
    pa.subset_off = d_subset_off.ptr;
    pa.weight = d_sub_weight.ptr;
    pa.path_off = d_path_off.ptr;
    pa.col_off = d_col_off.ptr;
    pa.abundances = d_abund.ptr;
    pa.noise = d_noise.ptr;
    pa.total = d_total.ptr;
    pa.path = d_path.ptr;
    pa.col_path = d_col_path.ptr;
    pa.iterations = d_iters.ptr;
    pa.kept_rows = d_kept_rows.ptr;
    pa.kept_entries = d_kept_entries.ptr;
    pa.packed = d_packed.ptr;
// ... 121 lines not shown
```

rpvg_amd/engine.py:

```python
from __future__ import annotations

import ctypes as C
import os
from typing import List, NamedTuple, Optional, Tuple

import numpy as np

from . import hip
from .batch import CClusterBatch, CEstimatesView, CParams, ClusterBatch, ClusterEstimates, decode_view

_HERE = os.path.dirname(os.path.abspath(__file__))
LIB_PATH = os.path.join(_HERE, "host", "librpvg_amd_harness.so")

MODELS = ("transcripts", "strains", "haplotype-transcripts", "haplotypes")

_lib = None


def lib() -> C.CDLL:
    global _lib
    if _lib is None:
        if not os.path.exists(LIB_PATH):
            raise hip.EngineError(f"{LIB_PATH} is missing: build it with __graft_entry__.build() (there is no CPU fallback)")
        hip.lib()
        L = C.CDLL(LIB_PATH)
        L.rpvg_amd_last_error.restype = C.c_char_p
        L.rpvg_amd_engine_create.restype = C.c_void_p
        L.rpvg_amd_engine_create.argtypes = [C.c_int]
        L.rpvg_amd_engine_create_uploader.restype = C.c_void_p
        L.rpvg_amd_engine_create_uploader.argtypes = [C.c_int]
        L.rpvg_amd_engine_destroy.argtypes = [C.c_void_p]
        L.rpvg_amd_engine_ctx.restype = C.c_void_p
        L.rpvg_amd_engine_ctx.argtypes = [C.c_void_p]
        L.rpvg_amd_engine_stats_get.argtypes = [C.c_void_p, C.c_void_p]
        L.rpvg_amd_engine_stats_reset.argtypes = [C.c_void_p]
        L.rpvg_amd_engine_independent_stats_get.argtypes = [C.c_void_p, C.c_void_p]
        L.rpvg_amd_run_generators_after.restype = C.c_int
        L.rpvg_amd_run_generators_after.argtypes = [C.c_void_p, C.c_void_p, C.c_char_p, C.POINTER(CParams), C.POINTER(C.c_uint32)]
        L.rpvg_amd_host_threads.restype = C.c_int
        L.rpvg_amd_batch_prepare.restype = C.c_void_p
        L.rpvg_amd_batch_prepare.argtypes = [C.c_void_p, C.POINTER(CClusterBatch), C.c_int]
        L.rpvg_amd_batch_free.argtypes = [C.c_void_p]
        L.rpvg_amd_batch_reupload.argtypes = [C.c_void_p, C.c_void_p, C.POINTER(CClusterBatch), C.POINTER(C.c_double)]
        L.rpvg_amd_batch_prepare_from_alignments.restype = C.c_void_p
        L.rpvg_amd_batch_prepare_from_alignments.argtypes = [C.c_void_p, C.c_void_p, C.POINTER(CClusterBatch), C.c_double, C.c_double,
                                                             C.c_double, C.c_uint32, C.c_int, C.c_double, C.c_double,
                                                             C.POINTER(C.c_double)]
        L.rpvg_amd_batch_prepare_from_alignments_fit.restype = C.c_void_p
        L.rpvg_amd_batch_prepare_from_alignments_fit.argtypes = [C.c_void_p, C.c_void_p, C.POINTER(CClusterBatch), C.c_void_p, C.c_uint32, C.c_int,
                                                                 C.c_void_p, C.c_double, C.c_double, C.POINTER(hip.CFragLengthFit),
                                                                 C.c_void_p, C.POINTER(C.c_double)]
        L.rpvg_amd_batch_prepare_from_alignments_fitted.restype = C.c_void_p
        L.rpvg_amd_batch_prepare_from_alignments_fitted.argtypes = [C.c_void_p, C.c_void_p, C.POINTER(CClusterBatch), C.c_double, C.c_double,
                                                                    C.c_double, C.c_double, C.c_double, C.POINTER(C.c_double)]
        L.rpvg_amd_batch_prepare_from_fragments.restype = C.c_void_p
        L.rpvg_amd_batch_prepare_from_fragments.argtypes = [C.c_void_p, C.c_void_p, C.c_uint32, C.c_void_p, C.c_void_p, C.c_void_p, C.c_uint64,
                                                            C.POINTER(CClusterBatch), C.c_double, C.c_double, C.c_double, C.c_uint32,
                                                            C.c_double, C.c_double, C.c_void_p, C.c_void_p, C.c_void_p, C.c_void_p,
                                                            C.POINTER(C.c_double)]
        L.rpvg_amd_batch_prepare_from_fragments_table.restype = C.c_void_p
        L.rpvg_amd_batch_prepare_from_fragments_table.argtypes = [C.c_void_p, C.c_void_p, C.c_uint32, C.c_void_p, C.c_void_p, C.c_void_p, C.c_uint64,
                                                                  C.c_void_p, C.c_int, C.c_double, C.c_double, C.c_double, C.c_uint32,
                                                                  C.c_double, C.c_double, C.c_void_p, C.c_void_p, C.c_void_p, C.c_void_p,
                                                                  C.POINTER(C.c_double)]
        L.rpvg_amd_batch_has_source_columns.restype = C.c_int
        L.rpvg_amd_batch_has_source_columns.argtypes = [C.c_void_p]
        L.rpvg_amd_batch_prepare_synth_dense.restype = C.c_void_p
        L.rpvg_amd_batch_prepare_synth_dense.argtypes = [C.c_void_p, C.c_uint64, C.c_uint64, C.c_uint32]
        L.rpvg_amd_run.restype = C.c_void_p
        L.rpvg_amd_run.argtypes = [C.c_void_p, C.c_void_p, C.c_char_p, C.POINTER(CParams), C.POINTER(C.c_double)]
        L.rpvg_amd_run_team.restype = C.c_int
        L.rpvg_amd_run_team.argtypes = [C.c_void_p, C.c_void_p, C.c_char_p, C.POINTER(CParams), C.c_int, C.POINTER(C.c_double)]
        L.rpvg_amd_run_team_result.restype = C.c_void_p
        L.rpvg_amd_run_team_result.argtypes = [C.c_void_p]
        L.rpvg_amd_run_inplace.restype = C.c_int
        L.rpvg_amd_run_inplace.argtypes = [C.c_void_p, C.c_void_p, C.c_char_p, C.POINTER(CParams), C.POINTER(C.c_double)]
        L.rpvg_amd_run_from_alignments_inplace.restype = C.c_int
        L.rpvg_amd_run_from_alignments_inplace.argtypes = [C.c_void_p, C.c_void_p, C.c_char_p, C.POINTER(CParams), C.POINTER(C.c_double),
                                                           C.POINTER(C.c_double)]
        L.rpvg_amd_group_create.restype = C.c_void_p
        L.rpvg_amd_group_create.argtypes = [C.POINTER(C.c_int), C.c_int]
        L.rpvg_amd_group_destroy.argtypes = [C.c_void_p]
        L.rpvg_amd_group_has_communicator.argtypes = [C.c_void_p]
        L.rpvg_amd_group_run.restype = C.c_void_p
        L.rpvg_amd_group_run.argtypes = [C.c_void_p, C.POINTER(CClusterBatch), C.c_char_p, C.POINTER(CParams), C.POINTER(C.c_double)]
        L.rpvg_amd_group_partition.argtypes = [C.c_void_p, C.c_void_p, C.c_uint64]
        L.rpvg_amd_group_gather.argtypes = [C.c_void_p, C.c_void_p, C.c_uint64, C.POINTER(C.c_uint64), C.POINTER(C.c_double)]
        L.rpvg_amd_pipeline_create.restype = C.c_void_p
        L.rpvg_amd_pipeline_create.argtypes = [C.c_int, C.c_char_p, C.POINTER(CParams), C.c_int]
        L.rpvg_amd_pipeline_destroy.argtypes = [C.c_void_p]
        L.rpvg_amd_pipeline_workers.argtypes = [C.c_void_p]
        L.rpvg_amd_pipeline_prepare_slots.argtypes = [C.c_void_p, C.POINTER(CClusterBatch), C.c_int]
        L.rpvg_amd_pipeline_submit.argtypes = [C.c_void_p, C.POINTER(CClusterBatch), C.c_int]
        L.rpvg_amd_pipeline_prepare_slot.argtypes = [C.c_void_p, C.POINTER(CClusterBatch), C.c_int]
        L.rpvg_amd_pipeline_wait.argtypes = [C.c_void_p]
        L.rpvg_amd_pipeline_result.restype = C.c_void_p
        L.rpvg_amd_pipeline_result.argtypes = [C.c_void_p, C.c_int]
        L.rpvg_amd_pipeline_stats_get.argtypes = [C.c_void_p, C.c_void_p, C.POINTER(C.c_double)]
        L.rpvg_amd_pipeline_stats_reset.argtypes = [C.c_void_p]
        L.rpvg_amd_pipeline_completions.argtypes = [C.c_void_p, C.c_void_p, C.c_uint64, C.POINTER(C.c_uint64)]
        L.rpvg_amd_result_view.argtypes = [C.c_void_p, C.POINTER(CEstimatesView)]
        L.rpvg_amd_result_free.argtypes = [C.c_void_p]
        _lib = L
    return _lib


class FragLengthFit(NamedTuple):
    loc: float
    scale: float
    shape: float
    max_length: int
    valid: bool
    stats: dict


def _fit_tuple(fit) -> FragLengthFit:
    return FragLengthFit(fit.loc, fit.scale, fit.shape, fit.max_length, bool(fit.valid),
                         dict(sample_size=fit.sample_size, iterations=fit.iterations, evaluations=fit.evaluations))


def _err() -> str:
    return lib().rpvg_amd_last_error().decode()


class Engine:

    def __init__(self, device: int = 0, uploader: bool = False):
        self.handle = lib().rpvg_amd_engine_create_uploader(device) if uploader else lib().rpvg_amd_engine_create(device)
        if not self.handle:
            raise hip.EngineError(f"engine create failed: {_err()}")

    def close(self):
        if self.handle:
            lib().rpvg_amd_engine_destroy(self.handle)
            self.handle = None

    def __del__(self):
        try:
            self.close()
        except Exception:
            pass

    def _ctx(self):
        return C.c_void_p(lib().rpvg_amd_engine_ctx(self.handle))

    def stats(self) -> dict:
        s = hip.CKernelStats()
        if lib().rpvg_amd_engine_stats_get(self.handle, C.byref(s)) != 0:
            raise hip.EngineError(f"stats failed: {_err()}")
        return s.as_dict()

    def independent_stats(self) -> dict:
        s = hip.CIndependentStats()
        if lib().rpvg_amd_engine_independent_stats_get(self.handle, C.byref(s)) != 0:
            raise hip.EngineError(f"stats failed: {_err()}")
        return {n: int(getattr(s, n)) for n, _ in s._fields_}

    def reset_stats(self):
        if lib().rpvg_amd_engine_stats_reset(self.handle) != 0:
            raise hip.EngineError(f"stats reset failed: {_err()}")

    def info(self) -> Tuple[str, int, int]:
        name = C.create_string_buffer(256)
        cus, mem = C.c_uint32(0), C.c_uint64(0)
        hip._check(hip.lib().rpvg_hip_device_info(self._ctx(), name, 256, C.byref(cus), C.byref(mem)), "rpvg_hip_device_info")
        return name.value.decode(), cus.value, mem.value

    def prepare(self, batch: ClusterBatch, per_cluster: bool = False) -> "PreparedBatch":
        return PreparedBatch(self, batch, per_cluster)

    def fit_frag_length(self, counts, skew_normal: bool = True) -> FragLengthFit:
        return _fit_tuple(hip.frag_length_fit(self._ctx(), counts, skew_normal))

    def effective_lengths(self, path_lengths, frag) -> np.ndarray:
        return hip.effective_lengths(self._ctx(), path_lengths, float(frag[0]), float(frag[1]), float(frag[2]))

    def prepare_from_alignments(self, alignments, path_info: ClusterBatch, frag=None, is_single_end: bool = False,
                                min_noise_prob: float = 1e-4, prob_precision: float = 1e-8, frag_counts=None, path_lengths=None,
                                skew_normal: bool = True) -> "PreparedBatch":
        if frag is not None and frag_counts is not None:
            raise ValueError("prepare_from_alignments: frag and frag_counts exclude each other")
        if (frag_counts is None) != (path_lengths is None):
            raise ValueError("prepare_from_alignments: frag_counts and path_lengths come together")
        if frag_counts is not None and is_single_end:
            raise ValueError("prepare_from_alignments: a single-end run has no fragment lengths to fit")
        prep = PreparedBatch.__new__(PreparedBatch)
        prep.engine = self
        prep.batch = path_info
        ca, cb = alignments.as_c(), path_info.as_c()
        secs = C.c_double(0)
        if frag_counts is not None:
            counts = np.ascontiguousarray(frag_counts, dtype=np.uint32)
            lengths = np.ascontiguousarray(path_lengths, dtype=np.uint32)
            if lengths.size != len(alignments.path_effective_length):
                raise ValueError("prepare_from_alignments: one path length per path")
            fit = hip.CFragLengthFit()
            eff = np.zeros(lengths.size, dtype=np.float64)
            prep.handle = lib().rpvg_amd_batch_prepare_from_alignments_fit(
                self.handle, C.byref(ca), C.byref(cb), C.c_void_p(counts.ctypes.data if counts.size else None), counts.size,
                1 if skew_normal else 0, C.c_void_p(lengths.ctypes.data if lengths.size else None), min_noise_prob, prob_precision,
                C.byref(fit), C.c_void_p(eff.ctypes.data if eff.size else None), C.byref(secs))
            if not prep.handle:
                raise hip.EngineError(f"batch prepare from alignments failed: {_err()}")
            prep.frag_fit = _fit_tuple(fit)
            prep.path_effective_length = eff
            prep.row_construction_seconds = secs.value
            return prep
        if isinstance(frag, FragLengthFit):
            if is_single_end or not frag.valid:
                raise ValueError("prepare_from_alignments: a fitted distribution must be valid and belongs to a paired-end run")
            prep.handle = lib().rpvg_amd_batch_prepare_from_alignments_fitted(
                self.handle, C.byref(ca), C.byref(cb), frag.loc, frag.scale, frag.shape, min_noise_prob, prob_precision, C.byref(secs))
            if not prep.handle:
                raise hip.EngineError(f"batch prepare from alignments failed: {_err()}")
            prep.row_construction_seconds = secs.value
            return prep
        if frag is None:
            frag = (300.0, 50.0, 0.0, 10)
        prep.handle = lib().rpvg_amd_batch_prepare_from_alignments(
            self.handle, C.byref(ca), C.byref(cb), frag[0], frag[1], frag[2], int(frag[3]), 1 if is_single_end else 0,
            min_noise_prob, prob_precision, C.byref(secs))
        if not prep.handle:
            raise hip.EngineError(f"batch prepare from alignments failed: {_err()}")
        prep.row_construction_seconds = secs.value
        return prep

    def prepare_from_fragments(self, chunks, index_params, path_info: Optional[ClusterBatch] = None, extra_sets=None, frag=None,
                               min_noise_prob: float = 1e-4, prob_precision: float = 1e-8, path_table=None,
                               collapse_names: bool = False) -> "PreparedBatch":
        from . import index as index_mod
        if (path_table is None) == (path_info is None):
            raise ValueError("prepare_from_fragments: either path_info or path_table")
        if collapse_names and (path_table is None or path_table.name_id is None):
            raise ValueError("prepare_from_fragments: collapse_names needs a path_table with name_id")
        chunks = list(chunks)
        cchunks = (index_mod.CFragmentLists * max(len(chunks), 1))(*[c.as_c() for c in chunks])
        cparams = index_params.as_c()
        sets = list(extra_sets or [])
        off = np.zeros(len(sets) + 1, dtype=np.uint64)
# ... 121 lines not shown
            raise hip.EngineError(f"group run({model}) failed: {_err()}")
        try:
            view = CEstimatesView()
            lib().rpvg_amd_result_view(h, C.byref(view))
            out = decode_view(view)
        finally:
            lib().rpvg_amd_result_free(h)
        self.num_clusters = batch.num_clusters
        return out, secs.value

    def partition(self):
        import numpy as np
        out = np.zeros(self.num_clusters, dtype=np.uint32)
        if lib().rpvg_amd_group_partition(self.handle, C.c_void_p(out.ctypes.data), self.num_clusters) != 0:
            raise hip.EngineError(f"group partition failed: {_err()}")
        return out

    def gather(self, capacity: int):
        import numpy as np
        out = np.zeros(max(1, capacity), dtype=np.float64)
        count, total = C.c_uint64(0), C.c_double(0)
        if lib().rpvg_amd_group_gather(self.handle, C.c_void_p(out.ctypes.data), capacity, C.byref(count), C.byref(total)) != 0:
            raise hip.EngineError(f"group gather failed: {_err()}")
        return out[:count.value].copy(), total.value


class Pipeline:

    def __init__(self, model: str, params: CParams, device: int = 0, workers: int = 0):
        self.handle = lib().rpvg_amd_pipeline_create(device, model.encode(), C.byref(params), workers)
        if not self.handle:
            raise hip.EngineError(f"pipeline create failed: {_err()}")
        self._keep = []

    @property
    def workers(self) -> int:
        return int(lib().rpvg_amd_pipeline_workers(self.handle))

    def prepare_slots(self, batch: ClusterBatch, slots: int):
        cb = batch.as_c()
        if lib().rpvg_amd_pipeline_prepare_slots(self.handle, C.byref(cb), slots) != 0:
            raise hip.EngineError(f"pipeline prepare failed: {_err()}")

    def prepare_slot(self, slot: int, part):
        cb = part.as_c(True)
        if lib().rpvg_amd_pipeline_prepare_slot(self.handle, C.byref(cb), slot) != 0:
            raise hip.EngineError(f"pipeline prepare failed: {_err()}")

    def submit(self, batch, slot: int, compact: bool = False, narrow: bool = False):
        cb = batch.as_c(compact, narrow) if narrow else batch.as_c(compact)
        self._keep.append((batch, cb))
        if lib().rpvg_amd_pipeline_submit(self.handle, C.byref(cb), slot) != 0:
            raise hip.EngineError(f"pipeline submit failed: {_err()}")

    def wait(self):
        rc = lib().rpvg_amd_pipeline_wait(self.handle)
        self._keep.clear()
        if rc != 0:
            raise hip.EngineError(f"pipeline batch failed: {_err()}")

    def result(self, slot: int) -> List[ClusterEstimates]:
        h = lib().rpvg_amd_pipeline_result(self.handle, slot)
        if not h:
            raise hip.EngineError(f"pipeline result failed: {_err()}")
        try:
            view = CEstimatesView()
            lib().rpvg_amd_result_view(h, C.byref(view))
            return decode_view(view)
        finally:
            lib().rpvg_amd_result_free(h)

    def stats(self) -> dict:
        s = hip.CKernelStats()
        up = (C.c_double * 6)()
        if lib().rpvg_amd_pipeline_stats_get(self.handle, C.byref(s), up) != 0:
            raise hip.EngineError(f"pipeline stats failed: {_err()}")
        out = s.as_dict()
        out["upload_seconds_per_batch"] = up[0]
        out["upload_copies_ms_per_batch"] = up[1]
        out["upload_kernels_ms_per_batch"] = up[2]
        out["worker_finish_ms_per_batch"], out["worker_estimate_ms_per_batch"], out["worker_idle_ms_per_batch"] = up[3] * 1e3, up[4] * 1e3, up[5] * 1e3
        return out

    def reset_stats(self):
        if lib().rpvg_amd_pipeline_stats_reset(self.handle) != 0:
            raise hip.EngineError(f"pipeline stats reset failed: {_err()}")

    def completions(self, capacity: int = 4096):
        import numpy as np
        out = np.zeros(capacity, dtype=np.float64)
        count = C.c_uint64(0)
        lib().rpvg_amd_pipeline_completions(self.handle, C.c_void_p(out.ctypes.data), capacity, C.byref(count))
        return out[:min(capacity, count.value)].copy()

    def close(self):
        if self.handle:
            lib().rpvg_amd_pipeline_destroy(self.handle)
            self.handle = None

    def __del__(self):
        try:
            self.close()
        except Exception:
            pass


class PreparedBatch:
    def __init__(self, engine: Engine, batch: ClusterBatch, per_cluster: bool):
        self.engine = engine
        self.batch = batch
        cb = batch.as_c()
        self.handle = lib().rpvg_amd_batch_prepare(engine.handle, C.byref(cb), 1 if per_cluster else 0)
        if not self.handle:
            raise hip.EngineError(f"batch prepare failed: {_err()}")

    def reupload(self, engine: "Engine", batch: Optional[ClusterBatch] = None, compact: bool = False) -> float:
        if batch is None and self.batch is None:
            raise ValueError("reupload: this batch was prepared without a host batch (path_table=...): pass the batch to upload")
        cb = (batch or self.batch).as_c(compact)
        secs = C.c_double(0)
        if lib().rpvg_amd_batch_reupload(engine.handle, self.handle, C.byref(cb), C.byref(secs)) != 0:
            raise hip.EngineError(f"batch reupload failed: {_err()}")
        return secs.value

    @property
    def has_source_columns(self) -> bool:
        return bool(lib().rpvg_amd_batch_has_source_columns(self.handle))

    def free(self):
        if self.handle:
            lib().rpvg_amd_batch_free(self.handle)
            self.handle = None

    def __del__(self):
        try:
            self.free()
        except Exception:
            pass


def run(model: str, params: CParams, batch: ClusterBatch, device: int = 0, per_cluster: bool = False) -> List[ClusterEstimates]:
    eng = Engine(device)
    try:
        prep = eng.prepare(batch, per_cluster)
        try:
            out, _ = eng.run(model, params, prep)
        finally:
            prep.free()
    finally:
        eng.close()
    return out
```

rpvg_amd/hip.py:

```python
from __future__ import annotations

import ctypes as C
import os
from typing import List, Optional, Sequence, Tuple

import numpy as np

from .batch import CClusterBatch, ClusterBatch

_HERE = os.path.dirname(os.path.abspath(__file__))
LIB_PATH = os.path.join(_HERE, "csrc", "librpvg_hip.so")

EXPORTS = [
    "rpvg_hip_device_count", "rpvg_hip_create", "rpvg_hip_create_uploader", "rpvg_hip_destroy", "rpvg_hip_last_error", "rpvg_hip_synchronize",
    "rpvg_hip_device_info", "rpvg_hip_malloc", "rpvg_hip_free", "rpvg_hip_memcpy_h2d", "rpvg_hip_memcpy_d2h",
    "rpvg_hip_batch_upload", "rpvg_hip_batch_free", "rpvg_hip_em_solve", "rpvg_hip_em_dense",
    "rpvg_hip_dense_from_cluster", "rpvg_hip_groups_build", "rpvg_hip_groups_free", "rpvg_hip_groups_collapse_info", "rpvg_hip_group_loglik",
    "rpvg_hip_synth_dense_cluster", "rpvg_hip_stats_get", "rpvg_hip_stats_reset", "rpvg_hip_stats_intervals", "rpvg_hip_em_kernel_name",
    "rpvg_hip_gibbs_read_counts", "rpvg_hip_min_path_cover", "rpvg_hip_min_path_cover_any", "rpvg_hip_cover_limits", "rpvg_hip_bounded_pair_posteriors", "rpvg_hip_pair_posteriors_get", "rpvg_hip_pair_posteriors_free",
    "rpvg_hip_em_dense_sharded", "rpvg_hip_synth_dense_rows", "rpvg_hip_synth_dense_cluster_batch", "rpvg_hip_comm_unique_id", "rpvg_hip_comm_init",
    "rpvg_hip_comm_destroy", "rpvg_hip_comm_allreduce_sum_f64", "rpvg_hip_comm_init_all", "rpvg_hip_gather", "rpvg_hip_host_register", "rpvg_hip_host_unregister", "rpvg_hip_group_conditionals",
    "rpvg_hip_group_gibbs", "rpvg_hip_group_gibbs_polyploid", "rpvg_hip_gibbs_sets_get", "rpvg_hip_gibbs_sets_free",
    "rpvg_hip_alignments_upload", "rpvg_hip_alignments_free", "rpvg_hip_read_rows_build", "rpvg_hip_read_rows_to_batch",
    "rpvg_hip_read_rows_view", "rpvg_hip_read_rows_sizes", "rpvg_hip_read_rows_free", "rpvg_hip_path_clusters", "rpvg_hip_debug_log",
    "rpvg_hip_nested_subset_em", "rpvg_hip_subset_em_get", "rpvg_hip_subset_em_free",
    "rpvg_hip_nested_full_subset_em", "rpvg_hip_subset_em_get_sets",
    "rpvg_hip_nested_independent_subset_em", "rpvg_hip_subset_em_get_independent", "rpvg_hip_independent_draws_get",
    "rpvg_hip_independent_limits", "rpvg_hip_independent_stats_get",
    "rpvg_hip_batch_cluster_totals", "rpvg_hip_batch_has_source_columns", "rpvg_hip_batch_source_columns_sizes",
    "rpvg_hip_batch_source_columns_get", "rpvg_hip_groups_build_from_sources", "rpvg_hip_groups_build_single_paths", "rpvg_hip_batch_upload_begin", "rpvg_hip_batch_upload_finish", "rpvg_hip_create_with_streams",
    "rpvg_hip_batch_upload_finish_queue", "rpvg_hip_batch_upload_finish_wait",
    "rpvg_hip_batch_upload_segments", "rpvg_hip_pinned_alloc", "rpvg_hip_pinned_free", "rpvg_hip_thread_wait_spin_us",
    "rpvg_hip_group_full_posteriors", "rpvg_hip_full_set_count",
    "rpvg_hip_frag_length_fit", "rpvg_hip_frag_length_table", "rpvg_hip_frag_length_table_get", "rpvg_hip_frag_length_table_free",
    "rpvg_hip_effective_lengths", "rpvg_hip_alignments_set_effective_lengths", "rpvg_hip_frag_length_eval",
    "rpvg_hip_align_index_create", "rpvg_hip_align_index_free", "rpvg_hip_align_index_add", "rpvg_hip_align_index_finish",
    "rpvg_hip_align_index_frag_counts", "rpvg_hip_align_index_view", "rpvg_hip_align_index_alignments",
    "rpvg_hip_path_table_upload", "rpvg_hip_path_table_free", "rpvg_hip_read_rows_to_batch_with_paths", "rpvg_hip_batch_path_group_ids",
    "rpvg_hip_name_groups_limits", "rpvg_hip_align_index_name_groups", "rpvg_hip_name_groups_view", "rpvg_hip_name_groups_free",
    "rpvg_hip_estimates_table_build", "rpvg_hip_estimates_table_tpm", "rpvg_hip_estimates_table_view", "rpvg_hip_estimates_table_limits",
    "rpvg_hip_estimates_table_free",
    "rpvg_hip_gibbs_table_build", "rpvg_hip_gibbs_table_view", "rpvg_hip_gibbs_table_rows", "rpvg_hip_gibbs_table_limits", "rpvg_hip_gibbs_table_free",
    "rpvg_hip_gibbs_read_counts_resident", "rpvg_hip_gibbs_samples_get", "rpvg_hip_gibbs_samples_free", "rpvg_hip_gibbs_table_build_resident",
    "rpvg_hip_gibbs_table_text", "rpvg_hip_estimates_table_text", "rpvg_hip_table_text_view", "rpvg_hip_table_text_get", "rpvg_hip_table_text_guards",
    "rpvg_hip_table_text_free", "rpvg_hip_estimates_set_text",
    "rpvg_hip_align_index_alignments_collapsed",
    "rpvg_hip_batch_rows_sizes", "rpvg_hip_batch_rows_get",
    "rpvg_hip_segment_sort_words",
]

COMM_ID_BYTES = 128


class EngineError(RuntimeError):
    pass


class CEmProblems(C.Structure):
    _fields_ = [("num_problems", C.c_uint32), ("cluster", C.c_void_p), ("col_off", C.c_void_p), ("col_path", C.c_void_p),
                ("collapse_precision", C.c_double)]


class CEmResults(C.Structure):
    _fields_ = [("abundances", C.c_void_p), ("noise_count", C.c_void_p), ("total_count", C.c_void_p),
                ("iterations", C.c_void_p)]


class CGroupSpec(C.Structure):
    _fields_ = [("num_matrices", C.c_uint32), ("cluster", C.c_void_p), ("group_off", C.c_void_p),
                ("group_path_off", C.c_void_p), ("group_path", C.c_void_p), ("normalise", C.c_int32),
                ("collapse_precision", C.c_double)]


class CGibbsSpec(C.Structure):
    _fields_ = [("num_problems", C.c_uint32), ("group_size", C.c_uint32), ("matrix", C.c_void_p), ("num_chains", C.c_void_p),
                ("num_burn_its", C.c_void_p), ("num_gibbs_its", C.c_void_p), ("log_freq", C.c_void_p), ("num_generators", C.c_uint32),
                ("generator_problem_off", C.c_void_p), ("generator_problem", C.c_void_p), ("generator_words", C.c_void_p)]


class CGibbsSetsView(C.Structure):
    _fields_ = [("num_problems", C.c_uint32), ("group_size", C.c_uint32), ("set_off", C.POINTER(C.c_uint64)),
                ("first", C.POINTER(C.c_uint32)), ("second", C.POINTER(C.c_uint32)), ("count", C.POINTER(C.c_uint32)),
                ("words_consumed", C.POINTER(C.c_uint64)), ("generator_state", C.POINTER(C.c_uint32)), ("rounds", C.c_uint32),
                ("conditionals", C.c_uint64), ("members", C.POINTER(C.c_uint32))]


class CPairPosteriorsView(C.Structure):
    _fields_ = [("num_matrices", C.c_uint32), ("pair_off", C.POINTER(C.c_uint64)), ("first", C.POINTER(C.c_uint32)),
                ("second", C.POINTER(C.c_uint32)), ("posterior", C.POINTER(C.c_double))]


class CSubsetEmSetsView(C.Structure):
    _fields_ = [("num_matrices", C.c_uint32), ("group_size", C.c_uint32), ("subset_off", C.POINTER(C.c_uint64)),
                ("weight", C.POINTER(C.c_double)), ("path_off", C.POINTER(C.c_uint64)), ("path", C.POINTER(C.c_uint32)),
                ("col_off", C.POINTER(C.c_uint64)), ("col_path", C.POINTER(C.c_uint32)), ("abundances", C.POINTER(C.c_double)),
                ("noise_count", C.POINTER(C.c_double)), ("total_count", C.POINTER(C.c_double)), ("iterations", C.POINTER(C.c_uint32)),
                ("retained_off", C.POINTER(C.c_uint64)), ("retained_rank", C.POINTER(C.c_uint64)),
                ("retained_posterior", C.POINTER(C.c_double)), ("set_count", C.POINTER(C.c_uint32)),
                ("cluster_noise_count", C.POINTER(C.c_double)), ("set_size", C.POINTER(C.c_uint32)), ("set_member", C.POINTER(C.c_uint32)),
                ("set_posterior", C.POINTER(C.c_double)), ("set_abundance", C.POINTER(C.c_double))]


class CIndependentSpec(C.Structure):
    _fields_ = [("num_clusters", C.c_uint32), ("matrix_off", C.c_void_p), ("group_size", C.c_uint32), ("column_counts", C.c_void_p),
                ("log_freq", C.c_void_p), ("min_hap_prob", C.c_double), ("max_em_its", C.c_uint32), ("max_rel_em_conv", C.c_double),
                ("collapse_precision", C.c_double), ("generator_words", C.c_void_p), ("keep_draws", C.c_int32)]


class CSubsetEmIndependentView(C.Structure):
    _fields_ = [("num_clusters", C.c_uint32), ("group_size", C.c_uint32), ("num_samples", C.c_uint32), ("subset_off", C.POINTER(C.c_uint64)),
                ("weight", C.POINTER(C.c_double)), ("path_off", C.POINTER(C.c_uint64)), ("path", C.POINTER(C.c_uint32)),
                ("col_off", C.POINTER(C.c_uint64)), ("col_path", C.POINTER(C.c_uint32)), ("abundances", C.POINTER(C.c_double)),
                ("noise_count", C.POINTER(C.c_double)), ("total_count", C.POINTER(C.c_double)), ("iterations", C.POINTER(C.c_uint32)),
                ("set_count", C.POINTER(C.c_uint32)), ("cluster_noise_count", C.POINTER(C.c_double)), ("set_size", C.POINTER(C.c_uint32)),
                ("set_member", C.POINTER(C.c_uint32)), ("set_posterior", C.POINTER(C.c_double)), ("set_abundance", C.POINTER(C.c_double)),
                ("sample_count", C.POINTER(C.c_uint32)), ("words_consumed", C.POINTER(C.c_uint64)), ("generator_state", C.POINTER(C.c_uint32))]


class CIndependentLimits(C.Structure):
    _fields_ = [("max_group_size", C.c_uint32), ("max_samples", C.c_uint32), ("max_transcript_sets", C.c_uint64), ("words_per_draw", C.c_uint32),
                ("state_words", C.c_uint32), ("max_work_bytes", C.c_uint64)]


class CIndependentStats(C.Structure):
    _fields_ = [("calls_completed", C.c_uint64), ("draws", C.c_uint64), ("subsets", C.c_uint64)]


def independent_limits() -> CIndependentLimits:
    out = CIndependentLimits()
    lib().rpvg_hip_independent_limits(C.byref(out))
    return out


EM_KERNELS = 12


class CEmKernelStats(C.Structure):
    _fields_ = [("ms", C.c_double), ("launches", C.c_uint64), ("problems", C.c_uint64), ("iterations", C.c_uint64),
                ("max_iterations", C.c_uint64), ("alg_bytes", C.c_double)]


class CKernelStats(C.Structure):
    _fields_ = [
        ("em_sparse_ms", C.c_double), ("em_sparse_launches", C.c_uint64), ("em_sparse_alg_bytes", C.c_double),
        ("em_dense_ms", C.c_double), ("em_dense_launches", C.c_uint64), ("em_dense_alg_bytes", C.c_double),
        ("loglik_ms", C.c_double), ("loglik_launches", C.c_uint64), ("loglik_evals", C.c_double),
        ("build_ms", C.c_double), ("build_launches", C.c_uint64),
        ("h2d_ms", C.c_double), ("h2d_bytes", C.c_double),
        ("em_iterations_total", C.c_uint64),
        ("search_pairs_possible", C.c_double), ("search_pairs_table", C.c_double), ("search_pairs_kept", C.c_double),
        ("em_kernel", CEmKernelStats * EM_KERNELS),
        ("collapse_ms", C.c_double), ("busy_ms", C.c_double), ("gibbs_ms", C.c_double),
        ("search_tile_ms", C.c_double), ("search_tile_launches", C.c_uint64),
        ("gibbs_calls_completed", C.c_uint64),
        ("gibbs_count_grid_problems", C.c_uint64), ("gibbs_count_grid_iterations", C.c_uint64),
        ("cover_grid_problems", C.c_uint64), ("cover_grid_rounds", C.c_uint64),
        ("text_exact_cells", C.c_uint64),
        ("nested_full_calls", C.c_uint64), ("nested_full_sets", C.c_uint64), ("nested_full_retained", C.c_uint64),
    ]

    def as_dict(self):
        d = {n: getattr(self, n) for n, _ in self._fields_ if n != "em_kernel"}
        d["em_kernel"] = {em_kernel_name(i): {n: getattr(self.em_kernel[i], n) for n, _ in CEmKernelStats._fields_} for i in range(EM_KERNELS)}
        return d


GRID_NEVER = 2 ** 64 - 1


class CCoverLimits(C.Structure):
    _fields_ = [("workgroup_max_paths", C.c_uint32), ("chunk_rounds", C.c_uint32), ("default_grid_min_work", C.c_uint64),
                ("grid_max_rows", C.c_uint64), ("grid_max_entries", C.c_uint64), ("pick_block", C.c_uint32), ("pick_per_thread", C.c_uint32),
                ("pick_max_blocks", C.c_uint32), ("strike_block", C.c_uint32), ("strike_max_blocks", C.c_uint32), ("hist_max_paths", C.c_uint32)]


def cover_limits() -> CCoverLimits:
    out = CCoverLimits()
    lib().rpvg_hip_cover_limits(C.byref(out))
    return out


def em_kernel_name(index: int) -> str:
    f = lib().rpvg_hip_em_kernel_name
    f.restype = C.c_char_p
    return f(index).decode()


_lib = None


def lib() -> C.CDLL:
    global _lib
    if _lib is None:
        if not os.path.exists(LIB_PATH):
            raise EngineError(f"{LIB_PATH} is missing: build it with `python -c 'import __graft_entry__ as g; g.build()'` "
                              "(there is no CPU fallback)")
        L = C.CDLL(LIB_PATH)
        L.rpvg_hip_last_error.restype = C.c_char_p
        L.rpvg_hip_full_set_count.restype = C.c_uint64
        L.rpvg_hip_cover_limits.restype = None
        L.rpvg_hip_independent_limits.restype = None
        for name in EXPORTS:
            getattr(L, name)
        _lib = L
    return _lib


def _check(rc: int, what: str):
# ... 352 lines not shown
                                           C.c_void_p(flag.ctypes.data if flag is not None else None),
                                           C.c_void_p(out.ctypes.data)), "rpvg_hip_group_loglik")
        return out

    def conditionals(self, matrix, others, width: int, divisor: float, num_cols) -> List[np.ndarray]:
        mt = np.ascontiguousarray(matrix, dtype=np.uint32)
        oth = np.ascontiguousarray(others, dtype=np.uint32).reshape(len(mt), max(width - 1, 0))
        sizes = [int(num_cols[int(m)]) for m in mt]
        out = np.zeros(sum(sizes), dtype=np.float64)
        _check(lib().rpvg_hip_group_conditionals(self.ctx.handle, self.handle, C.c_uint32(len(mt)), C.c_void_p(mt.ctypes.data),
                                                 C.c_void_p(oth.ctypes.data if oth.size else None), C.c_uint32(width),
                                                 C.c_double(divisor), C.c_void_p(out.ctypes.data)),
               "rpvg_hip_group_conditionals")
        return np.split(out, np.cumsum(sizes)[:-1]) if sizes else []

    def full_posteriors(self, matrix, group_size: int, log_freq, num_cols) -> List[np.ndarray]:
        mt = np.ascontiguousarray(matrix, dtype=np.uint32)
        lf = np.ascontiguousarray(np.concatenate([np.asarray(x, dtype=np.float64) for x in log_freq]) if len(log_freq) else np.zeros(0))
        sizes = [int(lib().rpvg_hip_full_set_count(C.c_uint32(int(num_cols[int(m)])), C.c_uint32(group_size))) for m in mt]
        out = np.zeros(sum(s for s in sizes if s <= 0x7fffffff), dtype=np.float64)
        _check(lib().rpvg_hip_group_full_posteriors(self.ctx.handle, self.handle, C.c_uint32(len(mt)), C.c_void_p(mt.ctypes.data),
                                                    C.c_uint32(group_size), C.c_void_p(lf.ctypes.data if lf.size else None),
                                                    C.c_void_p(out.ctypes.data if out.size else None)),
               "rpvg_hip_group_full_posteriors")
        return np.split(out, np.cumsum(sizes)[:-1]) if sizes else []

    def nested_full_subset_em(self, group_size: int, log_freq, min_hap_prob: float, max_em_its: int = 10000, max_rel_em_conv: float = 1e-3,
                              collapse_precision: float = 0.0) -> dict:
        lf = np.ascontiguousarray(np.concatenate([np.asarray(x, dtype=np.float64) for x in log_freq]) if len(log_freq) else np.zeros(0))
        h = C.c_void_p()
        _check(lib().rpvg_hip_nested_full_subset_em(self.ctx.handle, self.batch.handle, self.handle, C.c_uint32(group_size),
                                                    C.c_void_p(lf.ctypes.data if lf.size else None), C.c_double(float(min_hap_prob)),
                                                    C.c_uint32(max_em_its), C.c_double(float(max_rel_em_conv)),
                                                    C.c_double(float(collapse_precision)), C.byref(h)), "rpvg_hip_nested_full_subset_em")
        try:
            v = CSubsetEmSetsView()
            _check(lib().rpvg_hip_subset_em_get_sets(h, C.byref(v)), "rpvg_hip_subset_em_get_sets")
            M, g = int(v.num_matrices), int(v.group_size)

            def take(pointer, n, dtype, shape=None):
                if n == 0 or not pointer:
                    return np.zeros(shape if shape is not None else (0,), dtype=dtype)
                a = np.ctypeslib.as_array(pointer, shape=(n,)).copy()
                return a.reshape(shape) if shape is not None else a

            out = {"num_matrices": M, "group_size": g}
            if M == 0:
                out.update({"subset_off": np.zeros(1, np.uint64), "path_off": np.zeros(1, np.uint64), "col_off": np.zeros(1, np.uint64),
                            "retained_off": np.zeros(1, np.uint64)})
                for name, dtype in (("weight", np.float64), ("path", np.uint32), ("col_path", np.uint32), ("abundances", np.float64),
                                    ("noise_count", np.float64), ("total_count", np.float64), ("iterations", np.uint32),
                                    ("retained_rank", np.uint64), ("retained_posterior", np.float64), ("set_count", np.uint32),
                                    ("cluster_noise_count", np.float64), ("set_size", np.uint32), ("set_posterior", np.float64)):
                    out[name] = np.zeros(0, dtype)
                out["set_member"] = np.zeros((0, g), np.uint32)
                out["set_abundance"] = np.zeros((0, g), np.float64)
                return out
            out["subset_off"] = take(v.subset_off, M + 1, np.uint64)
            S = int(out["subset_off"][-1])
            out["path_off"] = take(v.path_off, S + 1, np.uint64)
            out["col_off"] = take(v.col_off, S + 1, np.uint64)
            L, Cn = int(out["path_off"][-1]), int(out["col_off"][-1])
            out["weight"] = take(v.weight, S, np.float64)
            out["path"] = take(v.path, L, np.uint32)
            out["col_path"] = take(v.col_path, Cn, np.uint32)
            out["abundances"] = take(v.abundances, Cn, np.float64)
            out["noise_count"] = take(v.noise_count, S, np.float64)
            out["total_count"] = take(v.total_count, S, np.float64)
            out["iterations"] = take(v.iterations, S, np.uint32)
            out["retained_off"] = take(v.retained_off, M + 1, np.uint64)
            R = int(out["retained_off"][-1])
            out["retained_rank"] = take(v.retained_rank, R, np.uint64)
            out["retained_posterior"] = take(v.retained_posterior, R, np.float64)
            out["set_count"] = take(v.set_count, M, np.uint32)
            out["cluster_noise_count"] = take(v.cluster_noise_count, M, np.float64)
            out["set_size"] = take(v.set_size, L, np.uint32)
            out["set_member"] = take(v.set_member, L * g, np.uint32, (L, g))
            out["set_posterior"] = take(v.set_posterior, L, np.float64)
            out["set_abundance"] = take(v.set_abundance, L * g, np.float64, (L, g))
            return out
        finally:
            lib().rpvg_hip_subset_em_free(h)

    def nested_independent_subset_em(self, matrix_off, group_size: int, min_hap_prob: float, generator_words, column_counts=None, log_freq=None,
                                     max_em_its: int = 10000, max_rel_em_conv: float = 1e-3, collapse_precision: float = 0.0,
                                     keep_draws: bool = False) -> dict:
        mo = np.ascontiguousarray(matrix_off, dtype=np.uint32)
        K = len(mo) - 1
        gw = np.ascontiguousarray(generator_words, dtype=np.uint32).reshape(K, 624)
        cc = None if column_counts is None else np.ascontiguousarray(column_counts, dtype=np.uint32)
        lf = None
        if log_freq is not None:
            lf = np.ascontiguousarray(np.concatenate([np.asarray(x, dtype=np.float64) for x in log_freq]) if len(log_freq) else np.zeros(0))
        spec = CIndependentSpec(K, mo.ctypes.data, group_size, cc.ctypes.data if cc is not None and cc.size else None,
                                lf.ctypes.data if lf is not None and lf.size else None, float(min_hap_prob), max_em_its, float(max_rel_em_conv),
                                float(collapse_precision), gw.ctypes.data if gw.size else None, 1 if keep_draws else 0)
        h = C.c_void_p()
        _check(lib().rpvg_hip_nested_independent_subset_em(self.ctx.handle, self.batch.handle, self.handle, C.byref(spec), C.byref(h)),
               "rpvg_hip_nested_independent_subset_em")
        try:
            v = CSubsetEmIndependentView()
            _check(lib().rpvg_hip_subset_em_get_independent(h, C.byref(v)), "rpvg_hip_subset_em_get_independent")
            g = int(v.group_size)

            def take(pointer, n, dtype, shape=None):
                if n == 0 or not pointer:
                    return np.zeros(shape if shape is not None else (0,), dtype=dtype)
                a = np.ctypeslib.as_array(pointer, shape=(n,)).copy()
                return a.reshape(shape) if shape is not None else a

            out = {"num_clusters": K, "group_size": g, "num_samples": int(v.num_samples)}
            out["subset_off"] = take(v.subset_off, K + 1, np.uint64) if K else np.zeros(1, np.uint64)
            S = int(out["subset_off"][-1])
            out["path_off"] = take(v.path_off, S + 1, np.uint64) if K else np.zeros(1, np.uint64)
            out["col_off"] = take(v.col_off, S + 1, np.uint64) if K else np.zeros(1, np.uint64)
            L, Cn = int(out["path_off"][-1]), int(out["col_off"][-1])
            out["weight"] = take(v.weight, S, np.float64)
            out["path"] = take(v.path, L, np.uint32)
            out["col_path"] = take(v.col_path, Cn, np.uint32)
            out["abundances"] = take(v.abundances, Cn, np.float64)
            out["noise_count"] = take(v.noise_count, S, np.float64)
            out["total_count"] = take(v.total_count, S, np.float64)
            out["iterations"] = take(v.iterations, S, np.uint32)
            out["set_count"] = take(v.set_count, K, np.uint32)
            out["cluster_noise_count"] = take(v.cluster_noise_count, K, np.float64)
            out["set_size"] = take(v.set_size, L, np.uint32)
            out["set_member"] = take(v.set_member, L * g, np.uint32, (L, g))
            out["set_posterior"] = take(v.set_posterior, L, np.float64)
            out["set_abundance"] = take(v.set_abundance, L * g, np.float64, (L, g))
            out["sample_count"] = take(v.sample_count, S, np.uint32)
            out["words_consumed"] = take(v.words_consumed, K, np.uint64)
            out["generator_state"] = take(v.generator_state, K * 624, np.uint32, (K, 624))
            if keep_draws:
                out["draws"] = []
                for k in range(K):
                    T = int(mo[k + 1]) - int(mo[k])
                    d = np.zeros(max(out["num_samples"] * T, 1), dtype=np.uint32)
                    _check(lib().rpvg_hip_independent_draws_get(h, C.c_uint32(k), C.c_void_p(d.ctypes.data)), "rpvg_hip_independent_draws_get")
                    out["draws"].append(d[:out["num_samples"] * T].reshape(out["num_samples"], T))
            return out
        finally:
            lib().rpvg_hip_subset_em_free(h)

    def gibbs(self, matrix, group_size: int, num_chains, num_burn_its, num_gibbs_its, log_freq, generator_problems, generator_words):
        return self._gibbs("rpvg_hip_group_gibbs", matrix, group_size, num_chains, num_burn_its, num_gibbs_its, log_freq, generator_problems,
                           generator_words)

    def gibbs_polyploid(self, matrix, group_size: int, num_chains, num_burn_its, num_gibbs_its, log_freq, generator_problems, generator_words):
        return self._gibbs("rpvg_hip_group_gibbs_polyploid", matrix, group_size, num_chains, num_burn_its, num_gibbs_its, log_freq,
                           generator_problems, generator_words)

    def _gibbs(self, entry, matrix, group_size, num_chains, num_burn_its, num_gibbs_its, log_freq, generator_problems, generator_words):
        mt = np.ascontiguousarray(matrix, dtype=np.uint32)
        ch = np.ascontiguousarray(num_chains, dtype=np.uint32)
        bu = np.ascontiguousarray(num_burn_its, dtype=np.uint32)
        it = np.ascontiguousarray(num_gibbs_its, dtype=np.uint32)
        lf = np.ascontiguousarray(np.concatenate([np.asarray(x, dtype=np.float64) for x in log_freq]) if len(log_freq) else np.zeros(0))
        goff = np.ascontiguousarray(np.concatenate([[0], np.cumsum([len(g) for g in generator_problems])]), dtype=np.uint32)
        gp = np.ascontiguousarray([p for g in generator_problems for p in g], dtype=np.uint32)
        gw = np.ascontiguousarray(generator_words, dtype=np.uint32).reshape(len(generator_problems), 624)
        spec = CGibbsSpec(len(mt), group_size, mt.ctypes.data, ch.ctypes.data, bu.ctypes.data, it.ctypes.data, lf.ctypes.data,
                          len(generator_problems), goff.ctypes.data, gp.ctypes.data, gw.ctypes.data)
        h = C.c_void_p()
        _check(getattr(lib(), entry)(self.ctx.handle, self.handle, C.byref(spec), C.byref(h)), entry)
        try:
            v = CGibbsSetsView()
# ... 247 lines not shown
        total = C.c_double(0)
        _check(lib().rpvg_hip_dense_from_cluster(self.handle, batch.handle, C.c_uint32(cluster), C.c_void_p(d_matrix),
                                                 C.c_uint64(ld), C.c_void_p(d_counts), C.byref(total)),
               "rpvg_hip_dense_from_cluster")
        return total.value

    def synth_dense_cluster(self, seed: int, R: int, N: int, d_matrix: int, ld: int, d_counts: int):
        _check(lib().rpvg_hip_synth_dense_cluster(self.handle, C.c_uint64(seed), C.c_uint64(R), C.c_uint32(N),
                                                  C.c_void_p(d_matrix), C.c_uint64(ld), C.c_void_p(d_counts)),
               "rpvg_hip_synth_dense_cluster")

    def synth_dense_rows(self, seed: int, row_begin: int, R: int, N: int, d_matrix: int, ld: int, d_counts: int):
        _check(lib().rpvg_hip_synth_dense_rows(self.handle, C.c_uint64(seed), C.c_uint64(row_begin), C.c_uint64(R),
                                               C.c_uint32(N), C.c_void_p(d_matrix), C.c_uint64(ld), C.c_void_p(d_counts)),
               "rpvg_hip_synth_dense_rows")

    def upload_alignments(self, align_batch) -> "DeviceAlignments":
        return DeviceAlignments(self, align_batch)

    def build_rows(self, align_batch, row_params, merge: bool = True):
        dev = align_batch if isinstance(align_batch, DeviceAlignments) else DeviceAlignments(self, align_batch)
        try:
            rows = dev.build_rows(row_params, merge)
            try:
                return rows.download()
            finally:
                rows.free()
        finally:
            if dev is not align_batch:
                dev.free()

    def frag_length_fit(self, counts, skew_normal: bool = True) -> CFragLengthFit:
        return frag_length_fit(self.handle, counts, skew_normal)

    def frag_length_table(self, loc: float, scale: float, shape: float) -> DeviceFragTable:
        return DeviceFragTable(self.handle, loc, scale, shape)

    def effective_lengths(self, path_lengths, loc: float, scale: float, shape: float) -> np.ndarray:
        return effective_lengths(self.handle, path_lengths, loc, scale, shape)

    def frag_length_eval(self, what: str, rows) -> np.ndarray:
        kind = {"cdf": 0, "truncated_mean": 1, "owens_t": 2}[what]
        rows = np.asarray(rows, dtype=np.float64)
        padded = np.zeros((rows.shape[0], 5), dtype=np.float64)
        padded[:, :rows.shape[1]] = rows
        out = np.zeros(rows.shape[0], dtype=np.float64)
        _check(lib().rpvg_hip_frag_length_eval(self.handle, C.c_int(kind), C.c_void_p(padded.ctypes.data), C.c_uint64(rows.shape[0]),
                                               C.c_void_p(out.ctypes.data)), "rpvg_hip_frag_length_eval")
        return out

    def path_clusters(self, num_paths: int, sets):
        off = np.zeros(len(sets) + 1, dtype=np.uint64)
        off[1:] = np.cumsum([len(x) for x in sets])
        flat = np.ascontiguousarray([p for x in sets for p in x], dtype=np.uint32)
        return self.path_clusters_flat(num_paths, off, flat)

    def path_clusters_flat(self, num_paths: int, set_off: np.ndarray, set_path: np.ndarray):
        set_off = np.ascontiguousarray(set_off, dtype=np.uint64)
        set_path = np.ascontiguousarray(set_path, dtype=np.uint32)
        p2c = np.zeros(max(num_paths, 1), dtype=np.uint32)
        coff = np.zeros(num_paths + 1, dtype=np.uint64)
        cpaths = np.zeros(max(num_paths, 1), dtype=np.uint32)
        nc = C.c_uint32(0)
        _check(lib().rpvg_hip_path_clusters(self.handle, C.c_uint32(num_paths), C.c_uint64(len(set_off) - 1),
                                            C.c_void_p(set_off.ctypes.data), C.c_void_p(set_path.ctypes.data if set_path.size else None),
                                            C.c_void_p(p2c.ctypes.data), C.byref(nc), C.c_void_p(coff.ctypes.data),
                                            C.c_void_p(cpaths.ctypes.data)), "rpvg_hip_path_clusters")
        k = nc.value
        members = [cpaths[int(coff[c]):int(coff[c + 1])].tolist() for c in range(k)]
        return p2c[:num_paths].copy(), members

    def debug_log(self, x: np.ndarray, use_table: bool = True) -> np.ndarray:
        x = np.ascontiguousarray(x, dtype=np.float64)
        out = np.zeros_like(x)
        _check(lib().rpvg_hip_debug_log(self.handle, C.c_uint64(x.size), C.c_void_p(x.ctypes.data), C.c_void_p(out.ctypes.data),
                                        C.c_int32(1 if use_table else 0)), "rpvg_hip_debug_log")
        return out

    def stats(self) -> dict:
        s = CKernelStats()
        _check(lib().rpvg_hip_stats_get(self.handle, C.byref(s)), "rpvg_hip_stats_get")
        return s.as_dict()

    def independent_stats(self) -> dict:
        s = CIndependentStats()
        _check(lib().rpvg_hip_independent_stats_get(self.handle, C.byref(s)), "rpvg_hip_independent_stats_get")
        return {n: int(getattr(s, n)) for n, _ in s._fields_}

    def reset_stats(self):
        _check(lib().rpvg_hip_stats_reset(self.handle), "rpvg_hip_stats_reset")
```

rpvg_amd/host/batch_pipeline.cpp:

```cpp
#include "batch_pipeline.hpp"

#include <algorithm>
#include <chrono>
#include <cstdlib>

#include "estimator_factory.hpp"
#include "trace.hpp"

namespace rpvg_amd {

static int defaultWorkers(const rpvg_params & params) {

    const char * env = std::getenv("RPVG_AMD_PIPELINE_WORKERS");
    return env ? std::max(1, std::min(8, std::atoi(env))) : (params.use_hap_gibbs ? 6 : 4);
}

BatchPipeline::BatchPipeline(const int device_in, const std::string & model_in, const rpvg_params & params_in, const int workers) : device(device_in), model(model_in), params(params_in), num_resident(0), num_unfinished(0), stopping(false), first_error(nullptr), upload_seconds(0), finish_seconds(0), estimate_seconds(0), wait_for_batch_seconds(0), upload_batches(0), stats_epoch(std::chrono::steady_clock::now()) {

    const int num_workers = workers > 0 ? std::min(workers, 8) : defaultWorkers(params_in);

    static const int num_uploaders = []() {

        const char * env = std::getenv("RPVG_AMD_PIPELINE_UPLOADERS");
        return env ? std::max(1, std::min(4, std::atoi(env))) : 1;
// ... 278 lines not shown

void BatchPipeline::workerLoop(const int worker) {

    const auto & engine = worker_engines.at(worker);

    hostThreadsOverride() = std::max(1, hostThreads() / static_cast<int>(worker_engines.size()));

    std::unique_ptr<PathEstimator> estimator;

    while (true) {

        std::unique_ptr<Job> job;
        const auto idle_from = std::chrono::steady_clock::now();

        {
            std::unique_lock<std::mutex> lock(mutex);
            changed.wait(lock, [&] { return stopping || !resident.empty(); });

            if (stopping) {

                return;
            }

            job = std::move(resident.front());
            resident.pop_front();
        }

        std::exception_ptr error = nullptr;
        const auto busy_from = std::chrono::steady_clock::now();
        auto finished_at = busy_from;

        try {

            if (!estimator) {

                estimator = makePathEstimator(model, params, engine);
            }

            job->device_batch->finish(engine);
            finished_at = std::chrono::steady_clock::now();
            estimator->estimateBatchSeeded(job->estimates, *job->device_batch, params.rng_seed);

        } catch (...) {

            error = std::current_exception();
        }

        job->device_batch.reset();
        const auto done_at = std::chrono::steady_clock::now();

        std::vector<std::unique_ptr<Job> > dropped;

        {
            std::lock_guard<std::mutex> lock(mutex);

            busy_estimates.erase(job->estimates);
            --num_resident;
            --num_unfinished;
            wait_for_batch_seconds += std::chrono::duration<double>(busy_from - idle_from).count();
            finish_seconds += std::chrono::duration<double>(finished_at - busy_from).count();
            estimate_seconds += std::chrono::duration<double>(done_at - finished_at).count();
            completions.emplace_back(std::chrono::duration<double>(std::chrono::steady_clock::now() - stats_epoch).count());

            if (error) {

                dropped = fail(error);
            }
        }

        changed.notify_all();
    }
}

void BatchPipeline::stats(rpvg_hip_kernel_stats * stats_out) const {

    std::vector<const HipEngine *> engines;

    for (auto & engine: worker_engines) {

        engines.emplace_back(engine.get());
    }

    HipEngine::stats(engines, stats_out);
}

void BatchPipeline::resetStats() const {

    for (auto & engine: worker_engines) {

        engine->resetStats();
    }

    for (auto & engine: uploader_engines) {

        engine->resetStats();
    }

    std::lock_guard<std::mutex> lock(mutex);
    BatchPipeline * self = const_cast<BatchPipeline *>(this);
    self->upload_seconds = 0;
    self->finish_seconds = 0;
    self->estimate_seconds = 0;
    self->wait_for_batch_seconds = 0;
    self->upload_batches = 0;
    self->stats_epoch = std::chrono::steady_clock::now();
    self->completions.clear();
}

void BatchPipeline::workerSeconds(double * finish_out, double * estimate_out, double * idle_out) const {

    std::lock_guard<std::mutex> lock(mutex);
    const double batches = std::max<double>(1, completions.size());

    *finish_out = finish_seconds / batches;
    *estimate_out = estimate_seconds / batches;
    *idle_out = wait_for_batch_seconds / batches;
}

void BatchPipeline::uploadDeviceMs(double * copies_ms_out, double * kernels_ms_out) const {

    *copies_ms_out = 0;
    *kernels_ms_out = 0;

    for (auto & engine: uploader_engines) {

        rpvg_hip_kernel_stats stats;
        engine->stats(&stats);

        *copies_ms_out += stats.h2d_ms;
        *kernels_ms_out += stats.build_ms;
    }
}

std::vector<double> BatchPipeline::completionSeconds() const {

    std::lock_guard<std::mutex> lock(mutex);
    return completions;
}

double BatchPipeline::meanUploadSeconds(uint64_t * batches_out) const {

    std::lock_guard<std::mutex> lock(mutex);

    if (batches_out) {

        *batches_out = upload_batches;
    }

    return upload_batches ? upload_seconds / upload_batches : 0.0;
}

}
```

rpvg_amd/host/batch_pipeline.hpp:

```cpp
#ifndef RPVG_AMD_BATCH_PIPELINE_HPP
#define RPVG_AMD_BATCH_PIPELINE_HPP

#include <chrono>
#include <condition_variable>
#include <deque>
#include <exception>
#include <memory>
#include <mutex>
#include <set>
#include <string>
#include <thread>
#include <vector>

#include "../../include/rpvg_batch.h"
#include "hip_engine.hpp"
#include "path_cluster_estimates.hpp"
#include "path_estimator.hpp"

namespace rpvg_amd {

class BatchPipeline {

    public:

        BatchPipeline(const int device, const std::string & model, const rpvg_params & params, const int workers = 0);
        ~BatchPipeline();

        BatchPipeline(const BatchPipeline &) = delete;
        BatchPipeline & operator=(const BatchPipeline &) = delete;

        void submit(const rpvg_cluster_batch & host_batch, std::vector<PathClusterEstimates> * estimates);

        void wait();

        int numWorkers() const { return worker_threads.size(); }

        void stats(rpvg_hip_kernel_stats * stats_out) const;
        void resetStats() const;

        double meanUploadSeconds(uint64_t * batches_out = nullptr) const;

        void workerSeconds(double * finish_out, double * estimate_out, double * idle_out) const;

        void uploadDeviceMs(double * copies_ms_out, double * kernels_ms_out) const;

        std::vector<double> completionSeconds() const;

    private:

        struct Job {

            rpvg_cluster_batch host_batch;
            std::vector<PathClusterEstimates> * estimates;
            std::unique_ptr<DeviceClusterBatch> device_batch;
        };

        void uploadLoop(const int uploader);
        void queueLoop();
        void workerLoop(const int worker);
        std::vector<std::unique_ptr<Job> > fail(std::exception_ptr error);

        const int device;
        const std::string model;
        const rpvg_params params;

        std::vector<std::shared_ptr<HipEngine> > uploader_engines;
        std::vector<std::shared_ptr<HipEngine> > worker_engines;

        mutable std::mutex mutex;
        std::condition_variable changed;

        std::deque<std::unique_ptr<Job> > to_upload;
        std::deque<std::unique_ptr<Job> > copied;
        std::deque<std::unique_ptr<Job> > resident;
        std::set<const void *> busy_estimates;

        size_t num_resident;
        size_t num_unfinished;
        bool stopping;
        std::exception_ptr first_error;

        double upload_seconds, finish_seconds, estimate_seconds, wait_for_batch_seconds;
        uint64_t upload_batches;
        std::chrono::steady_clock::time_point stats_epoch;
        std::vector<double> completions;

        std::vector<std::thread> upload_threads;
        std::thread queue_thread;
        size_t max_resident;
        std::vector<std::thread> worker_threads;
};

}

#endif
```

rpvg_amd/host/hip_engine.cpp:

```cpp
#include "hip_engine.hpp"

#include <cstdio>
#include <cstring>
#include "trace.hpp"

#include <algorithm>
#include <cassert>
#include <cstdlib>
#include <mutex>

#include <malloc.h>

namespace rpvg_amd {

static void keepHeapTop() {

    static std::once_flag once;

    std::call_once(once, []() {

        if (!std::getenv("MALLOC_TOP_PAD_")) {

            mallopt(M_TOP_PAD, 64 << 20);
        }
// ... 23 lines not shown
    keepHeapTop();

    static const int lean_side_streams = []() {

        const char * env = std::getenv("RPVG_AMD_SIDE_STREAMS");
        return env ? std::max(1, std::min(6, std::atoi(env))) : 3;
    }();

    if (uploader) {

        check(rpvg_hip_create_uploader(device, &context), "rpvg_hip_create");

    } else if (host_lanes_in == 1) {

        check(rpvg_hip_create_with_streams(device, lean_side_streams, &context), "rpvg_hip_create");

    } else {

        check(rpvg_hip_create(device, &context), "rpvg_hip_create");
    }
}

HipEngine::~HipEngine() {

    const bool trace = std::getenv("RPVG_AMD_TRACE_EXIT") != nullptr;
    if (trace) std::fprintf(stderr, "[exit] ~HipEngine begins\n");

    lane_workers.clear();
    if (trace) std::fprintf(stderr, "[exit] lane workers joined\n");

    for (auto & lane_context: laneContexts()) {

        rpvg_hip_destroy(lane_context);
        if (trace) std::fprintf(stderr, "[exit] a lane context destroyed\n");
    }

    rpvg_hip_destroy(context);
    if (trace) std::fprintf(stderr, "[exit] ~HipEngine done\n");
}

std::shared_ptr<HipEngine> HipEngine::processDefault() {

    static std::mutex default_mutex;
    static std::shared_ptr<HipEngine> default_engine;

    std::lock_guard<std::mutex> lock(default_mutex);

    if (!default_engine) {

        const char * device = std::getenv("RPVG_AMD_DEVICE");
        default_engine = std::make_shared<HipEngine>(device ? std::atoi(device) : 0);
    }

    return default_engine;
}

int & HipEngine::currentLane() {

    thread_local int lane = 0;
    return lane;
}

void HipEngine::stats(rpvg_hip_kernel_stats * stats_out) const {

    stats(std::vector<const HipEngine *>(1, this), stats_out);
}

void HipEngine::independentStats(rpvg_hip_independent_stats * stats_out) const {

    std::vector<rpvg_hip_ctx *> contexts(1, context);
    const auto lane_contexts = laneContexts();
    contexts.insert(contexts.end(), lane_contexts.begin(), lane_contexts.end());

    *stats_out = rpvg_hip_independent_stats{0, 0, 0};

    for (auto & ctx: contexts) {

        rpvg_hip_independent_stats lane_stats;
        check(rpvg_hip_independent_stats_get(ctx, &lane_stats), "rpvg_hip_independent_stats_get");

        stats_out->calls_completed += lane_stats.calls_completed;
        stats_out->draws += lane_stats.draws;
        stats_out->subsets += lane_stats.subsets;
    }
}

void HipEngine::stats(const std::vector<const HipEngine *> & engines, rpvg_hip_kernel_stats * stats_out) {

    std::vector<rpvg_hip_ctx *> contexts;

    for (auto & engine: engines) {

        contexts.emplace_back(engine->context);
        const auto lane_contexts = engine->laneContexts();
        contexts.insert(contexts.end(), lane_contexts.begin(), lane_contexts.end());
    }

    assert(!contexts.empty());
    check(rpvg_hip_stats_get(contexts.front(), stats_out), "rpvg_hip_stats_get");

    for (size_t c = 1; c < contexts.size(); ++c) {

        rpvg_hip_kernel_stats lane_stats;
        check(rpvg_hip_stats_get(contexts[c], &lane_stats), "rpvg_hip_stats_get");

        stats_out->em_sparse_ms += lane_stats.em_sparse_ms;
        stats_out->em_sparse_launches += lane_stats.em_sparse_launches;
        stats_out->em_sparse_alg_bytes += lane_stats.em_sparse_alg_bytes;
        stats_out->em_dense_ms += lane_stats.em_dense_ms;
        stats_out->em_dense_launches += lane_stats.em_dense_launches;
        stats_out->em_dense_alg_bytes += lane_stats.em_dense_alg_bytes;
        stats_out->loglik_ms += lane_stats.loglik_ms;
        stats_out->loglik_launches += lane_stats.loglik_launches;
        stats_out->loglik_evals += lane_stats.loglik_evals;
        stats_out->build_ms += lane_stats.build_ms;
        stats_out->build_launches += lane_stats.build_launches;
        stats_out->h2d_ms += lane_stats.h2d_ms;
        stats_out->h2d_bytes += lane_stats.h2d_bytes;
        stats_out->em_iterations_total += lane_stats.em_iterations_total;
        stats_out->search_pairs_possible += lane_stats.search_pairs_possible;
        stats_out->search_pairs_table += lane_stats.search_pairs_table;
        stats_out->search_pairs_kept += lane_stats.search_pairs_kept;
        stats_out->collapse_ms += lane_stats.collapse_ms;
        stats_out->gibbs_ms += lane_stats.gibbs_ms;
        stats_out->search_tile_ms += lane_stats.search_tile_ms;
        stats_out->search_tile_launches += lane_stats.search_tile_launches;
        stats_out->gibbs_calls_completed += lane_stats.gibbs_calls_completed;
        stats_out->gibbs_count_grid_problems += lane_stats.gibbs_count_grid_problems;
        stats_out->gibbs_count_grid_iterations += lane_stats.gibbs_count_grid_iterations;
        stats_out->cover_grid_problems += lane_stats.cover_grid_problems;
        stats_out->cover_grid_rounds += lane_stats.cover_grid_rounds;
        stats_out->text_exact_cells += lane_stats.text_exact_cells;
        stats_out->nested_full_calls += lane_stats.nested_full_calls;
        stats_out->nested_full_sets += lane_stats.nested_full_sets;
        stats_out->nested_full_retained += lane_stats.nested_full_retained;

        for (int i = 0; i < RPVG_HIP_EM_KERNELS; ++i) {

            stats_out->em_kernel[i].ms += lane_stats.em_kernel[i].ms;
            stats_out->em_kernel[i].launches += lane_stats.em_kernel[i].launches;
            stats_out->em_kernel[i].problems += lane_stats.em_kernel[i].problems;
            stats_out->em_kernel[i].iterations += lane_stats.em_kernel[i].iterations;
            stats_out->em_kernel[i].max_iterations += lane_stats.em_kernel[i].max_iterations;
            stats_out->em_kernel[i].alg_bytes += lane_stats.em_kernel[i].alg_bytes;
        }
    }

    std::vector<std::pair<double, double> > spans;

    for (auto & ctx: contexts) {

        uint64_t count = 0;
        check(rpvg_hip_stats_intervals(ctx, 0, nullptr, nullptr, nullptr, &count), "rpvg_hip_stats_intervals");

        std::vector<double> start(count), stop(count);
        check(rpvg_hip_stats_intervals(ctx, count, start.data(), stop.data(), nullptr, &count), "rpvg_hip_stats_intervals");

        for (size_t i = 0; i < std::min<size_t>(count, start.size()); ++i) {

            spans.emplace_back(start[i], stop[i]);
        }
    }

    std::sort(spans.begin(), spans.end());

    double busy = 0;
// ... 597 lines not shown
```

rpvg_amd/host/hip_engine.hpp:

```cpp
#ifndef RPVG_AMD_HIP_ENGINE_HPP
#define RPVG_AMD_HIP_ENGINE_HPP

#include <array>
#include <atomic>
#include <cstdint>
#include <memory>
#include <mutex>
#include <stdexcept>
#include <string>
#include <unordered_map>
#include <vector>

#include "../../include/rpvg_hip.h"
#include "path_cluster_estimates.hpp"
#include "pipeline_lanes.hpp"
#include "read_path_probabilities.hpp"

namespace rpvg_amd {

class EngineError : public std::runtime_error {

    public:

        explicit EngineError(const std::string & what_in) : std::runtime_error(what_in) {}
};

class HipEngine {

    public:

        explicit HipEngine(const int device, const bool uploader = false, const int host_lanes = 0);
        ~HipEngine();

        HipEngine(const HipEngine &) = delete;
        HipEngine & operator=(const HipEngine &) = delete;

        rpvg_hip_ctx * ctx() const {

            const int lane = currentLane();

            if (lane > 0 && static_cast<size_t>(lane) <= lane_contexts.size()) {

                if (rpvg_hip_ctx * lane_context = lane_contexts[lane - 1].load(std::memory_order_acquire)) {

                    return lane_context;
                }
            }

            return context;
        }
        int device() const { return device_id; }
        int hostLanes() const { return host_lanes; }

        static int & currentLane();

        void stats(rpvg_hip_kernel_stats * stats_out) const;
        void resetStats() const;

        void independentStats(rpvg_hip_independent_stats * stats_out) const;

        static void stats(const std::vector<const HipEngine *> & engines, rpvg_hip_kernel_stats * stats_out);

        static int deviceCount();

        static std::shared_ptr<HipEngine> processDefault();

        static void check(const int status, const char * what);

        PipelineWorker & lane(const int lane);

        static constexpr int max_lanes = 4;

        int combinerLane(const int slot);

        static constexpr int max_combiner_slots = 6;

    private:

        rpvg_hip_ctx * context;
        int device_id;
        int host_lanes;

        std::mutex lane_mutex;
        std::array<std::atomic<rpvg_hip_ctx *>, max_lanes - 1 + max_combiner_slots> lane_contexts;
        std::vector<std::unique_ptr<PipelineWorker> > lane_workers;

        std::vector<rpvg_hip_ctx *> laneContexts() const;
};

class FlatClusterRows {

    public:

        FlatClusterRows();

        void addCluster(const std::vector<ReadPathProbabilities> & cluster_probs, const uint32_t num_paths);

        void addCluster(const std::vector<ReadPathProbabilities> & cluster_probs, const std::vector<PathInfo> & paths);

        void append(const FlatClusterRows & other);

        uint32_t numClusters() const { return cluster_row_off.size() - 1; }
        rpvg_cluster_batch view() const;

    private:

        std::vector<uint64_t> cluster_row_off, cluster_path_off, path_source_off;
        std::vector<uint32_t> row_grp_off, grp_idx_off;
        std::vector<uint8_t> row_grp_count, grp_idx_count;
        bool counts_fit;
        std::vector<uint32_t> row_count, path_idx, path_group_id, source_id;
        std::vector<double> row_noise, grp_prob;

        std::vector<uint16_t> path_idx16, source_id16, row_noise16;
        std::vector<uint8_t> row_count8;
        std::vector<uint32_t> row_count_escape_row, row_count_escape_count;
        std::vector<double> row_noise_table;
        std::unordered_map<uint64_t, uint16_t> noise_index;
        bool paths_fit16, sources_fit16, noise_fits16;

        uint16_t noiseIndex(const double noise);
};

class ClusterSegment {

    public:

        ClusterSegment();
        ~ClusterSegment();

        ClusterSegment(const ClusterSegment &) = delete;
        ClusterSegment & operator=(const ClusterSegment &) = delete;

        struct Columns {

            uint32_t num;
            const uint32_t * counts;
            const uint32_t * path_off;
            const uint32_t * paths;
        };

        void flatten(const std::vector<ReadPathProbabilities> & cluster_probs, const std::vector<PathInfo> & paths, const bool with_sources, const Columns * columns = nullptr);

// ... 58 lines not shown
```

rpvg_amd/host/runner_capi.cpp:

```cpp

#include <cassert>
#include <chrono>
#include <cmath>
#include <cstring>
#include <limits>
#include <algorithm>
#include <memory>
#include <stdexcept>
#include <string>
#include <unordered_map>
#include <utility>
#include <vector>

#include "../../include/rpvg_batch.h"
#include "batch_pipeline.hpp"
#include "device_group.hpp"
#include "estimator_factory.hpp"
#include "align_index.hpp"
#include "read_rows.hpp"
#include "runner_handles.hpp"
#include "trace.hpp"

using namespace rpvg_amd;
using namespace rpvg_amd_harness;
// ... 237 lines not shown

        if (collapse_names) {

            prepared->paths.back() = std::move(collapsed_paths.at(i));
        }
    }

    if (cluster_path_off_out) {

        cluster_path_off_out[cluster_paths.size()] = num_cluster_paths;
    }

    if (info_out) {

        *info_out = index.info();
    }

    if (frag_counts_out) {

        const auto counts = index.fragLengthCounts();
        std::copy(counts.begin(), counts.end(), frag_counts_out);
    }

    return guard.release();
}

}

extern "C" {

const char * rpvg_amd_last_error(void) {

    return last_error.c_str();
}

void * rpvg_amd_engine_create(int device) {

    return guardedHandle([&]() -> void * {

        Engine * engine = new Engine();
        engine->hip = std::make_shared<HipEngine>(device);
        return engine;
    });
}

void * rpvg_amd_engine_create_uploader(int device) {

    return guardedHandle([&]() -> void * {

        Engine * engine = new Engine();
        engine->hip = std::make_shared<HipEngine>(device, true);
        return engine;
    });
}

void rpvg_amd_engine_destroy(void * engine) {

    delete static_cast<Engine *>(engine);
}

void * rpvg_amd_engine_ctx(void * engine) {

    return static_cast<Engine *>(engine)->hip->ctx();
}

int rpvg_amd_engine_stats_get(void * engine, rpvg_hip_kernel_stats * stats_out) {

    return guardedInt([&]() -> int {

        static_cast<Engine *>(engine)->hip->stats(stats_out);
        return 0;
    });
}

int rpvg_amd_engine_independent_stats_get(void * engine, rpvg_hip_independent_stats * stats_out) {

    return guardedInt([&]() -> int {

        static_cast<Engine *>(engine)->hip->independentStats(stats_out);
        return 0;
    });
}

int rpvg_amd_engine_stats_reset(void * engine) {

    return guardedInt([&]() -> int {

        static_cast<Engine *>(engine)->hip->resetStats();
        return 0;
    });
}

int rpvg_amd_host_threads() {

    return rpvg_amd::hostThreads();
}

int rpvg_amd_generator_state_check(uint32_t rounds) {

    return rpvg_amd::PathEstimator::generatorStateSelfTest(rounds);
}

void * rpvg_amd_batch_prepare(void * engine, const rpvg_cluster_batch * batch, int keep_rows) {

    return guardedHandle([&]() -> void * {

        PreparedBatch * prepared = new PreparedBatch();
        std::unique_ptr<PreparedBatch> guard(prepared);

        prepared->paths = unpackPaths(*batch);

        if (keep_rows) {

            for (uint32_t i = 0; i < batch->num_clusters; ++i) {

                prepared->rows.emplace_back(unpackRows(*batch, i, 1e-8));
            }

        } else {

            prepared->device.reset(new DeviceClusterBatch(static_cast<Engine *>(engine)->hip, *batch));
        }

        return guard.release();
    });
}

void * rpvg_amd_batch_prepare_from_alignments(void * engine, const rpvg_alignment_batch * alignments, const rpvg_cluster_batch * path_info, double frag_loc, double frag_scale, double frag_shape, uint32_t frag_sd_max_multi, int is_single_end, double min_noise_prob, double prob_precision, double * seconds_out) {

    return guardedHandle([&]() -> void * {

        PreparedBatch * prepared = new PreparedBatch();
        std::unique_ptr<PreparedBatch> guard(prepared);

        prepared->paths = unpackPaths(*path_info);
        assert(prepared->paths.size() == alignments->num_clusters);

        AlignmentBatchBuilder builder;
        fillBuilder(*alignments, prepared->paths, &builder);

        prepared->fragment_length_dist.reset(is_single_end ? new FragmentLengthDist() : new FragmentLengthDist(frag_loc, frag_scale, frag_shape, frag_sd_max_multi));
        prepared->is_single_end = is_single_end != 0;
        prepared->min_noise_prob = min_noise_prob;
        prepared->prob_precision = prob_precision;

        const auto start = std::chrono::steady_clock::now();
        prepared->alignments.reset(new DeviceAlignmentBatch(static_cast<Engine *>(engine)->hip, builder));
        prepared->device = constructReadPathProbabilities(*prepared->alignments, *prepared->fragment_length_dist, prepared->is_single_end, min_noise_prob, prob_precision);

        if (seconds_out) {

            *seconds_out = std::chrono::duration<double>(std::chrono::steady_clock::now() - start).count();
        }

        return guard.release();
    });
}

void * rpvg_amd_batch_prepare_from_alignments_fit(void * engine, const rpvg_alignment_batch * alignments, const rpvg_cluster_batch * path_info, const uint32_t * frag_length_counts, uint32_t num_frag_length_counts, int skew_normal, const uint32_t * path_length, double min_noise_prob, double prob_precision, rpvg_frag_length_fit * fit_out, double * effective_length_out, double * seconds_out) {

    return guardedHandle([&]() -> void * {

        PreparedBatch * prepared = new PreparedBatch();
        std::unique_ptr<PreparedBatch> guard(prepared);

        prepared->paths = unpackPaths(*path_info);
// ... 789 lines not shown

            for (size_t i = 0; i < paths.size(); ++i) {

                slot.at(i).paths = paths.at(i);
            }
        }

        return 0;
    });
}

int rpvg_amd_pipeline_prepare_slot(void * pipeline_handle, const rpvg_cluster_batch * batch, int slot) {

    return guardedInt([&]() -> int {

        Pipeline * pipeline = static_cast<Pipeline *>(pipeline_handle);
        pipeline->pipeline->wait();

        const auto paths = unpackPaths(*batch);

        if (pipeline->slots.size() <= static_cast<size_t>(slot)) {

            pipeline->slots.resize(slot + 1);
        }

        auto & containers = pipeline->slots.at(slot);
        containers.assign(paths.size(), PathClusterEstimates());

        for (size_t i = 0; i < paths.size(); ++i) {

            containers.at(i).paths = paths.at(i);
        }

        return 0;
    });
}

int rpvg_amd_pipeline_submit(void * pipeline_handle, const rpvg_cluster_batch * batch, int slot) {

    return guardedInt([&]() -> int {

        Pipeline * pipeline = static_cast<Pipeline *>(pipeline_handle);
        pipeline->pipeline->submit(*batch, &pipeline->slots.at(slot));
        return 0;
    });
}

int rpvg_amd_pipeline_wait(void * pipeline_handle) {

    return guardedInt([&]() -> int {

        static_cast<Pipeline *>(pipeline_handle)->pipeline->wait();
        return 0;
    });
}

void * rpvg_amd_pipeline_result(void * pipeline_handle, int slot) {

    return guardedHandle([&]() -> void * {

        return packResult(static_cast<Pipeline *>(pipeline_handle)->slots.at(slot));
    });
}

int rpvg_amd_pipeline_stats_get(void * pipeline_handle, rpvg_hip_kernel_stats * stats_out, double * mean_upload_seconds_out) {

    return guardedInt([&]() -> int {

        Pipeline * pipeline = static_cast<Pipeline *>(pipeline_handle);
        pipeline->pipeline->stats(stats_out);

        if (mean_upload_seconds_out) {

            uint64_t batches = 0;
            mean_upload_seconds_out[0] = pipeline->pipeline->meanUploadSeconds(&batches);

            pipeline->pipeline->uploadDeviceMs(mean_upload_seconds_out + 1, mean_upload_seconds_out + 2);
            mean_upload_seconds_out[1] /= std::max<uint64_t>(1, batches);
            mean_upload_seconds_out[2] /= std::max<uint64_t>(1, batches);

            pipeline->pipeline->workerSeconds(mean_upload_seconds_out + 3, mean_upload_seconds_out + 4, mean_upload_seconds_out + 5);
        }

        return 0;
    });
}

int rpvg_amd_pipeline_completions(void * pipeline_handle, double * seconds_out, uint64_t capacity, uint64_t * count_out) {

    const auto completions = static_cast<Pipeline *>(pipeline_handle)->pipeline->completionSeconds();
    *count_out = completions.size();
    std::copy(completions.begin(), completions.begin() + std::min<size_t>(capacity, completions.size()), seconds_out);
    return 0;
}

int rpvg_amd_pipeline_stats_reset(void * pipeline_handle) {

    return guardedInt([&]() -> int {

        static_cast<Pipeline *>(pipeline_handle)->pipeline->resetStats();
        return 0;
    });
}

void rpvg_amd_result_view(void * result_handle, rpvg_estimates_view * out) {

    Result * result = static_cast<Result *>(result_handle);

    out->num_clusters = result->noise_count.size();
    out->set_off = result->set_off.data();
    out->member_off = result->member_off.data();
    out->members = result->members.data();
    out->posteriors = result->posteriors.data();
    out->abund_off = result->abund_off.data();
    out->abundances = result->abundances.data();
    out->noise_count = result->noise_count.data();
    out->total_count = result->total_count.data();
    out->em_off = result->em_off.data();
    out->em_iters = result->em_iters.data();
    out->em_col_off = result->em_col_off.data();
    out->em_cols = result->em_cols.data();
    out->gibbs_off = result->gibbs_off.data();
    out->gibbs_path_off = result->gibbs_path_off.data();
    out->gibbs_path = result->gibbs_path.data();
    out->gibbs_noise_off = result->gibbs_noise_off.data();
    out->gibbs_noise = result->gibbs_noise.data();
    out->gibbs_abund_off = result->gibbs_abund_off.data();
    out->gibbs_abund = result->gibbs_abund.data();
}

void rpvg_amd_result_free(void * result_handle) {

    delete static_cast<Result *>(result_handle);
}

}
```

Baseline: 2.582 billion.

## Release search gate after pair tile kernel with ordered turn queue

Moves the cross-context search gate into a reusable template that hands out ordered turns per device. It releases the gate right after the pair tile kernel instead of at the end of the whole search, so another context's large search can start sooner. An optional env flag moves the search tail onto the priority collapse stream. Gate statistics and timing spans are added. The risk is extra host blocking on the condition variable, plus more contention on the device when searches overlap.

After: 2.516 billion. -2.6%, worse.

```diff
diff --git a/include/rpvg_hip.h b/include/rpvg_hip.h
--- a/include/rpvg_hip.h
+++ b/include/rpvg_hip.h
@@ -460,6 +460,16 @@
 int rpvg_hip_stats_intervals(rpvg_hip_ctx * ctx, uint64_t capacity, double * start_ms, double * stop_ms, int32_t * family,
                              uint64_t * count_out);
 
+typedef struct rpvg_hip_search_gate_stats {
+    uint64_t searches_gated;
+    uint64_t tile_releases;
+    double wait_host_ms;
+    double hold_host_ms;
+    double hold_device_ms;
+    uint64_t hold_device_spans;
+} rpvg_hip_search_gate_stats;
+int rpvg_hip_search_gate_stats_get(rpvg_hip_ctx * ctx, rpvg_hip_search_gate_stats * stats_out);
+
 #ifdef __cplusplus
 }
 #endif
diff --git a/rpvg_amd/csrc/bounded_search.hip b/rpvg_amd/csrc/bounded_search.hip
--- a/rpvg_amd/csrc/bounded_search.hip
+++ b/rpvg_amd/csrc/bounded_search.hip
@@ -13,8 +13,14 @@
 using namespace rpvg_search;
 
 namespace {
-std::mutex g_search_gate_mutex;
-const rpvg_hip_ctx * g_search_gate_owner = nullptr;
+struct HipGateOps {
+    using Event = hipEvent_t;
+    using Stream = hipStream_t;
+    void record(hipEvent_t event, hipStream_t stream) { (void) hipEventRecord(event, stream); }
+    void streamWait(hipStream_t stream, hipEvent_t event) { (void) hipStreamWaitEvent(stream, event, 0); }
+    void hostWait(hipEvent_t event) { (void) waitEvent(event); }
+};
+rpvg_search_gate::Gate<HipGateOps> g_search_gate;
 }
 
 static bool searchLaunchesEarly() {
@@ -22,34 +28,58 @@
     return early;
 }
 
-constexpr uint64_t kSearchGateRows = 1ull << 17;
-
-static void searchGateEnter(rpvg_hip_ctx * ctx, hipStream_t stream, const uint64_t matrix_rows) {
+static bool searchGateWhole() {
+    const char * env = std::getenv("RPVG_HIP_SEARCH_GATE_WHOLE");
+    return env && std::atoi(env) != 0;
+}
+
+static void searchGateEnter(rpvg_hip_ctx * ctx, hipStream_t stream, const uint64_t matrix_rows, const bool release_behind_tile) {
     static const bool open_gate = RPVG_EXPERIMENT_ENV("RPVG_HIP_NO_SEARCH_GATE") != nullptr;
-    ctx->search_gate_held = !open_gate && matrix_rows >= kSearchGateRows;
-    if (!ctx->search_gate_held) return;
-    hipEvent_t previous = nullptr;
-    {
-        std::lock_guard<std::mutex> lock(g_search_gate_mutex);
-        if (g_search_gate_owner && g_search_gate_owner != ctx && g_search_gate_owner->device == ctx->device) {
-            previous = g_search_gate_owner->search_done;
-            (void) hipStreamWaitEvent(stream, previous, 0);
-        }
-    }
-    if (previous && !searchLaunchesEarly()) (void) waitEvent(previous);
+    HipGateOps ops;
+    const bool inside = g_search_gate.enter(ops, ctx->search_seat, stream, matrix_rows, open_gate,
+                                            release_behind_tile ? rpvg_search_gate::kReleaseTile : rpvg_search_gate::kReleaseWhole, !searchLaunchesEarly());
+    ctx->search_gate_span = inside ? ctx->spanBegin(FAM_GATE, stream) : -1;
+}
+
+static void searchGateSpanEnd(rpvg_hip_ctx * ctx) {
+    ctx->spanEnd(ctx->search_gate_span);
+    ctx->search_gate_span = -1;
+}
+
+static void searchGateReleaseBehindTile(rpvg_hip_ctx * ctx, hipStream_t stream) {
+    if (!(ctx->search_seat.held && ctx->search_seat.turn)) return;
+    HipGateOps ops;
+    g_search_gate.releaseBehindTile(ops, ctx->search_seat, stream);
+    searchGateSpanEnd(ctx);
 }
 
 static void searchGateLeave(rpvg_hip_ctx * ctx, hipStream_t stream) {
-    if (!ctx->search_gate_held) return;
-    ctx->search_gate_held = false;
-    std::lock_guard<std::mutex> lock(g_search_gate_mutex);
-    (void) hipEventRecord(ctx->search_done, stream);
-    g_search_gate_owner = ctx;
-}
-
-void searchGateForget(const rpvg_hip_ctx * ctx) {
-    std::lock_guard<std::mutex> lock(g_search_gate_mutex);
-    if (g_search_gate_owner == ctx) g_search_gate_owner = nullptr;
+    if (!ctx->search_seat.held) return;
+    HipGateOps ops;
+    g_search_gate.leave(ops, ctx->search_seat, stream);
+    searchGateSpanEnd(ctx);
+}
+
+void searchGateForget(const rpvg_hip_ctx * ctx) { g_search_gate.forget(ctx->search_seat); }
+
+static bool searchTailOnPriorityStream() {
+    const char * env = std::getenv("RPVG_HIP_SEARCH_TAIL_PRIORITY");
+    return env && std::atoi(env) != 0;
+}
+
+static hipError_t forkSearchTail(rpvg_hip_ctx * ctx) {
+    if (!ctx->collapse_stream || !ctx->tail_event) return hipSuccess;
+    hipError_t e = hipEventRecord(ctx->tail_event, ctx->stream);
+    if (e == hipSuccess) e = hipStreamWaitEvent(ctx->collapse_stream, ctx->tail_event, 0);
+    if (e == hipSuccess) ctx->search_tail = ctx->collapse_stream;
+    return e;
+}
+
+static void joinSearchTail(rpvg_hip_ctx * ctx) {
+    if (!ctx->search_tail) return;
+    (void) hipEventRecord(ctx->tail_event, ctx->search_tail);
+    (void) hipStreamWaitEvent(ctx->stream, ctx->tail_event, 0);
+    ctx->search_tail = nullptr;
 }
 
 struct rpvg_hip_pair_posteriors {
@@ -1019,6 +1049,12 @@
             pairTile2Kernel<<<dim3(pw.count), dim3(kTileBlock), tile_lds_bytes, st>>>(pw);
         }
 #endif
+        const bool released_here = ctx->search_seat.held && ctx->search_seat.turn;
+        searchGateReleaseBehindTile(ctx, st);
+        if (released_here && w.tail_may_move && searchTailOnPriorityStream()) {
+            ok(forkSearchTail(ctx));
+            st = pairSearchTailStream(ctx);
+        }
     } else {
         TableWork tw;
         tw.item_matrix = w.d_item_matrix.ptr;
@@ -1188,16 +1224,19 @@
         }
     }
     span = ctx->spanBegin(FAM_LOGLIK);
-    searchGateEnter(ctx, st, std::accumulate(groups->h_num_rows.begin(), groups->h_num_rows.end(), uint64_t(0)));
+    const bool release_behind_tile = plan.pair_tiles && plan.num_big == M && M > 0 && !w.own_release && !searchGateWhole();
+    searchGateEnter(ctx, st, std::accumulate(groups->h_num_rows.begin(), groups->h_num_rows.end(), uint64_t(0)), release_behind_tile);
     if (side_kernels) ok(ctx->forkAux());
     const GroupMatricesView view = groups->view();
     if (plan.num_big > 0) ok(launchTablePart(ctx, groups, view, plan, w, runs_behind_search && e == hipSuccess));
+    if (release_behind_tile) searchGateLeave(ctx, st);
     launchSequentialParts(ctx, view, plan, w);
     if (side_kernels) ok(ctx->joinAux());
     ctx->spanEnd(span);
     ctx->stats.loglik_launches += (plan.num_big > 0 ? 2 : 0) + (plan.num_medium > 0) + (M > plan.num_big + plan.num_medium);
     ok(hipGetLastError());
     if (e != hipSuccess) {
+        joinSearchTail(ctx);
         (void) hipStreamSynchronize(st);
         searchFailed(e);
         return RPVG_HIP_ERR_RUNTIME;
@@ -1205,7 +1244,12 @@
     return RPVG_HIP_OK;
 }
 
-void leavePairSearch(rpvg_hip_ctx * ctx) { searchGateLeave(ctx, ctx->stream); }
+void leavePairSearch(rpvg_hip_ctx * ctx) {
+    searchGateLeave(ctx, ctx->stream);
+    joinSearchTail(ctx);
+}
+
+hipStream_t pairSearchTailStream(const rpvg_hip_ctx * ctx) { return ctx->search_tail ? ctx->search_tail : ctx->stream; }
 
 void accountPairSearch(rpvg_hip_ctx * ctx, const rpvg_hip_groups * groups, const PairSearchWork & w, const unsigned long long log_evals,
                        const uint64_t kept_pairs) {
@@ -1245,6 +1289,7 @@
 
     std::lock_guard<std::mutex> lock(ctx->mutex);
     PairSearchWork w;
+    w.own_release = true;
     {
         const int rc = queuePairSearch(ctx, groups, column_counts, min_rel_likelihood, w);
         if (rc != RPVG_HIP_OK) {
diff --git a/rpvg_amd/csrc/common.hpp b/rpvg_amd/csrc/common.hpp
--- a/rpvg_amd/csrc/common.hpp
+++ b/rpvg_amd/csrc/common.hpp
@@ -19,6 +19,7 @@
 
 #include "../../include/rpvg_hip.h"
 #include "search_plan.hpp"
+#include "search_gate.hpp"
 #include "em_plan.hpp"
 #include "batch_forms.hpp"
 
@@ -494,7 +495,7 @@
     return before + incl - v;
 }
 
-enum KernelFamily { FAM_EM_SPARSE = 0, FAM_EM_DENSE, FAM_LOGLIK, FAM_BUILD, FAM_H2D, FAM_COLLAPSE, FAM_EM_KERNEL, FAM_GIBBS, FAM_TILE, FAM_COUNT };
+enum KernelFamily { FAM_EM_SPARSE = 0, FAM_EM_DENSE, FAM_LOGLIK, FAM_BUILD, FAM_H2D, FAM_COLLAPSE, FAM_EM_KERNEL, FAM_GIBBS, FAM_TILE, FAM_GATE, FAM_COUNT };
 
 struct TimedSpan {
     hipEvent_t start, stop;
@@ -522,7 +523,10 @@
     static constexpr int kAuxStreams = 6;
     rpvg_hip_detail::SubsetEmHints subset_hints;
     rpvg_hip_detail::SubsetEmHints subset_full_hints;
-    bool search_gate_held = false;
+    rpvg_search_gate::Seat<hipEvent_t> search_seat;
+    int search_gate_span = -1;
+    hipStream_t search_tail = nullptr;
+    hipEvent_t tail_event = nullptr;
     int device = 0;
     hipStream_t stream = nullptr;
     hipStream_t aux[kAuxStreams] = {};
@@ -533,7 +537,6 @@
     hipStream_t copy_stream = nullptr;
     hipEvent_t copied = nullptr;
     hipEvent_t fork_event = nullptr;
-    hipEvent_t search_done = nullptr;
     hipEvent_t join_event[kAuxStreams] = {};
     hipError_t forkAux();
     hipError_t joinAux();
@@ -552,6 +555,8 @@
     std::vector<rpvg_hip_detail::TimedInterval> intervals;
     rpvg_hip_kernel_stats stats;
     rpvg_hip_independent_stats independent_stats{};
+    double search_gate_device_ms = 0;
+    uint64_t search_gate_device_spans = 0;
     rpvg_hip_detail::SubsetEmHints subset_independent_hints;
 
     int spanBegin(int family, hipStream_t on = nullptr, int sub = -1);
@@ -924,6 +929,8 @@
     DeviceBuffer<uint64_t> d_col_off, d_pair_cap_off, d_big_col_part_off, d_big_pair_part_off;
     DeviceBuffer<double> d_lf, d_marg, d_opt_raw, d_opt, d_out_value, d_part_marg, d_part_opt, d_part_pair, d_seq;
     UploadPack pack;
+    bool own_release = false;
+    bool tail_may_move = false;
     const uint64_t * extra_u64 = nullptr;
     size_t extra_u64_count = 0, extra_zero_bytes = 0;
     DeviceBuffer<uint64_t> d_extra_u64;
@@ -932,6 +939,7 @@
 int queuePairSearch(rpvg_hip_ctx * ctx, const rpvg_hip_groups * groups, const uint32_t * column_counts, double min_rel_likelihood,
                     PairSearchWork & w);
 void leavePairSearch(rpvg_hip_ctx * ctx);
+hipStream_t pairSearchTailStream(const rpvg_hip_ctx * ctx);
 void accountPairSearch(rpvg_hip_ctx * ctx, const rpvg_hip_groups * groups, const PairSearchWork & w, unsigned long long log_evals, uint64_t kept_pairs);
 
 struct CsrCollapseInput {
diff --git a/rpvg_amd/csrc/context.hip b/rpvg_amd/csrc/context.hip
--- a/rpvg_amd/csrc/context.hip
+++ b/rpvg_amd/csrc/context.hip
@@ -396,6 +396,7 @@
         case FAM_COLLAPSE: stats.collapse_ms += ms; break;
         case FAM_GIBBS: stats.gibbs_ms += ms; break;
         case FAM_TILE: stats.search_tile_ms += ms; stats.search_tile_launches += 1; break;
+        case FAM_GATE: search_gate_device_ms += ms; search_gate_device_spans += 1; return;
         case FAM_EM_KERNEL:
             if (s.sub >= 0 && s.sub < RPVG_HIP_EM_KERNELS) stats.em_kernel[s.sub].ms += ms;
             break;
@@ -559,7 +560,9 @@
     }
     if (e == hipSuccess) e = createMainStream(&ctx->collapse_stream, RPVG_EXPERIMENT_ENV("RPVG_HIP_COLLAPSE_PRIORITY") == nullptr || std::atoi(RPVG_EXPERIMENT_ENV("RPVG_HIP_COLLAPSE_PRIORITY")) != 0);
     if (e == hipSuccess) e = hipEventCreateWithFlags(&ctx->fork_event, hipEventDisableTiming);
-    if (e == hipSuccess) e = hipEventCreateWithFlags(&ctx->search_done, hipEventDisableTiming);
+    ctx->search_seat.device = device;
+    if (e == hipSuccess) e = hipEventCreateWithFlags(&ctx->search_seat.done, hipEventDisableTiming);
+    if (e == hipSuccess) e = hipEventCreateWithFlags(&ctx->tail_event, hipEventDisableTiming);
     if (e == hipSuccess) e = hipStreamCreateWithFlags(&ctx->copy_stream, hipStreamNonBlocking);
     if (e == hipSuccess) e = hipEventCreateWithFlags(&ctx->copied, hipEventDisableTiming);
     if (e == hipSuccess) {
@@ -629,7 +632,8 @@
     }
     if (ctx->grid_ready) (void) hipEventDestroy(ctx->grid_ready);
     searchGateForget(ctx);
-    if (ctx->search_done) (void) hipEventDestroy(ctx->search_done);
+    if (ctx->search_seat.done) (void) hipEventDestroy(ctx->search_seat.done);
+    if (ctx->tail_event) (void) hipEventDestroy(ctx->tail_event);
     bool last = false;
     {
         std::lock_guard<std::mutex> lock(g_pool_mutex);
@@ -763,8 +767,27 @@
     if (rc != RPVG_HIP_OK) return rc;
     memset(&ctx->stats, 0, sizeof(ctx->stats));
     ctx->independent_stats = rpvg_hip_independent_stats{};
+    ctx->search_seat.counts = rpvg_search_gate::Counts{};
+    ctx->search_gate_device_ms = 0;
+    ctx->search_gate_device_spans = 0;
     ctx->intervals.clear();
     (void) deviceClock(ctx->device, ctx->stream, true);
+    return RPVG_HIP_OK;
+}
+
+int rpvg_hip_search_gate_stats_get(rpvg_hip_ctx * ctx, rpvg_hip_search_gate_stats * stats_out) {
+    RPVG_REQUIRE(ctx != nullptr && stats_out != nullptr, "rpvg_hip_search_gate_stats_get: NULL argument");
+    std::lock_guard<std::mutex> lock(ctx->mutex);
+    RPVG_HIP_CHECK(hipSetDevice(ctx->device));
+    int rc = ctx->foldSpans();
+    if (rc != RPVG_HIP_OK) return rc;
+    const rpvg_search_gate::Counts & counts = ctx->search_seat.counts;
+    stats_out->searches_gated = counts.searches;
+    stats_out->tile_releases = counts.tile_releases;
+    stats_out->wait_host_ms = counts.wait_host_ms;
+    stats_out->hold_host_ms = counts.hold_host_ms;
+    stats_out->hold_device_ms = ctx->search_gate_device_ms;
+    stats_out->hold_device_spans = ctx->search_gate_device_spans;
     return RPVG_HIP_OK;
 }
 
diff --git a/rpvg_amd/csrc/search_gate.hpp b/rpvg_amd/csrc/search_gate.hpp
--- /dev/null
+++ b/rpvg_amd/csrc/search_gate.hpp
@@ -0,0 +1,132 @@
+#pragma once
+
+#include <chrono>
+#include <condition_variable>
+#include <cstdint>
+#include <map>
+#include <mutex>
+
+namespace rpvg_search_gate {
+
+constexpr uint64_t kSearchGateRows = 1ull << 17;
+
+enum Release { kReleaseWhole = 0, kReleaseTile = 1 };
+
+struct Counts {
+    uint64_t searches = 0;
+    uint64_t tile_releases = 0;
+    double wait_host_ms = 0;
+    double hold_host_ms = 0;
+};
+
+template <class Event>
+struct Seat {
+    Event done{};
+    int device = 0;
+    bool held = false;
+    bool turn = false;
+    std::chrono::steady_clock::time_point entered;
+    Counts counts;
+};
+
+template <class Ops>
+class Gate {
+  public:
+    using Event = typename Ops::Event;
+    using Stream = typename Ops::Stream;
+    using SeatT = Seat<Event>;
+
+    bool enter(Ops & ops, SeatT & seat, Stream stream, const uint64_t matrix_rows, const bool open, const Release release,
+               const bool host_waits) {
+        seat.held = !open && matrix_rows >= kSearchGateRows;
+        seat.turn = false;
+        if (!seat.held) return false;
+        const auto arrived = std::chrono::steady_clock::now();
+        Event previous{};
+        bool wait = false;
+        {
+            std::unique_lock<std::mutex> lock(mutex_);
+            Line & line = lines_[seat.device];
+            if (release == kReleaseTile) {
+                const uint64_t mine = line.next_turn++;
+                turn_cv_.wait(lock, [&]() { return line.serving == mine; });
+                seat.turn = true;
+            }
+            if (line.owner && line.owner != &seat) {
+                previous = line.owner->done;
+                wait = true;
+                ops.streamWait(stream, previous);
+            }
+        }
+        if (wait && host_waits) ops.hostWait(previous);
+        seat.entered = std::chrono::steady_clock::now();
+        seat.counts.searches += 1;
+        seat.counts.wait_host_ms += std::chrono::duration<double, std::milli>(seat.entered - arrived).count();
+        return true;
+    }
+
+    void releaseBehindTile(Ops & ops, SeatT & seat, Stream stream) {
+        if (seat.held && seat.turn) release(ops, seat, stream);
+    }
+
+    void leave(Ops & ops, SeatT & seat, Stream stream) {
+        if (seat.held) release(ops, seat, stream);
+    }
+
+    void forget(const SeatT & seat) {
+        bool served = false;
+        {
+            std::lock_guard<std::mutex> lock(mutex_);
+            auto it = lines_.find(seat.device);
+            if (it == lines_.end()) return;
+            if (it->second.owner == &seat) it->second.owner = nullptr;
+            if (seat.held && seat.turn) {
+                it->second.serving += 1;
+                served = true;
+            }
+        }
+        if (served) turn_cv_.notify_all();
+    }
+
+    const SeatT * owner(const int device) {
+        std::lock_guard<std::mutex> lock(mutex_);
+        auto it = lines_.find(device);
+        return it == lines_.end() ? nullptr : it->second.owner;
+    }
+
+    uint64_t inLine(const int device) {
+        std::lock_guard<std::mutex> lock(mutex_);
+        auto it = lines_.find(device);
+        return it == lines_.end() ? 0 : it->second.next_turn - it->second.serving;
+    }
+
+  private:
+    struct Line {
+        const SeatT * owner = nullptr;
+        uint64_t next_turn = 0, serving = 0;
+    };
+
+    void release(Ops & ops, SeatT & seat, Stream stream) {
+        const bool turn = seat.turn;
+        seat.held = false;
+        seat.turn = false;
+        {
+            std::lock_guard<std::mutex> lock(mutex_);
+            Line & line = lines_[seat.device];
+            ops.record(seat.done, stream);
+            line.owner = &seat;
+            if (turn) line.serving += 1;
+        }
+        if (turn) {
+            turn_cv_.notify_all();
+            seat.counts.tile_releases += 1;
+        }
+        seat.counts.hold_host_ms += std::chrono::duration<double, std::milli>(std::chrono::steady_clock::now() - seat.entered).count();
+    }
+
+    std::mutex mutex_;
+    std::condition_variable turn_cv_;
+    std::map<int, Line> lines_;
+};
+
+}
diff --git a/rpvg_amd/csrc/subset_em.hip b/rpvg_amd/csrc/subset_em.hip
--- a/rpvg_amd/csrc/subset_em.hip
+++ b/rpvg_amd/csrc/subset_em.hip
@@ -578,6 +578,7 @@
         search.extra_u64 = slot_off.data();
         search.extra_u64_count = M + 1;
         search.extra_zero_bytes = header_room + emQueuesBytes();
+        search.tail_may_move = true;
         rc = queuePairSearch(ctx, groups, column_counts, min_rel_likelihood, search);
         if (rc != RPVG_HIP_OK) return rc;
     } else {
@@ -644,8 +645,8 @@
     if (e == hipSuccess) ok(hipEventCreateWithFlags(&header_here, hipEventDisableTiming));
     if (e != hipSuccess) {
         setError("rpvg_hip_nested_subset_em: %s", hipGetErrorString(e));
+        leavePairSearch(ctx);
         (void) hipStreamSynchronize(st);
-        leavePairSearch(ctx);
         if (pinned_header) pinnedFree(pinned_header);
         if (header_here) (void) hipEventDestroy(header_here);
         return (e == hipErrorOutOfMemory) ? RPVG_HIP_ERR_ALLOC : RPVG_HIP_ERR_RUNTIME;
@@ -654,7 +655,8 @@
     MatrixTotals * bases = reinterpret_cast<MatrixTotals *>(d_bases.ptr);
 
     std::unique_ptr<HostScope> part_scope(new HostScope("subset em: select + offsets + expand queued"));
-    int span = ctx->spanBegin(FAM_BUILD);
+    hipStream_t ts = pairSearchTailStream(ctx);
+    int span = ctx->spanBegin(FAM_BUILD, ts);
     SelectArgs sa;
     sa.num_matrices = M;
     sa.pair_count = search.d_tail.ptr;
@@ -680,8 +682,8 @@
     sa.totals = totals;
     sa.header = header;
     sa.big_matrices = d_big_matrices.ptr;
-    subsetSelectSmallKernel<<<dim3(M), dim3(64), 0, st>>>(sa);
-    subsetSelectWideKernel<<<dim3(std::min<uint32_t>(M, 128)), dim3(256), 0, st>>>(sa);
+    subsetSelectSmallKernel<<<dim3(M), dim3(64), 0, ts>>>(sa);
+    subsetSelectWideKernel<<<dim3(std::min<uint32_t>(M, 128)), dim3(256), 0, ts>>>(sa);
     const bool check_build = !groups->build_checked && groups->build_error_flag.ptr;
     OffsetsArgs oa;
     oa.pair_count = search.d_tail.ptr;
@@ -700,10 +702,10 @@
     oa.seg_first = d_seg_first.ptr;
     oa.path_off = d_path_off.ptr;
     oa.col_off = d_col_off.ptr;
-    subsetOffsetsKernel<<<dim3(1), dim3(1024), 0, st>>>(oa);
+    subsetOffsetsKernel<<<dim3(1), dim3(1024), 0, ts>>>(oa);
     SubsetHeader * h_header = static_cast<SubsetHeader *>(pinned_header);
-    ok(hipMemcpyAsync(h_header, header, sizeof(SubsetHeader), hipMemcpyDeviceToHost, st));
-    ok(hipEventRecord(header_here, st));
+    ok(hipMemcpyAsync(h_header, header, sizeof(SubsetHeader), hipMemcpyDeviceToHost, ts));
+    ok(hipEventRecord(header_here, ts));
     ExpandArgs ea;
     ea.num_matrices = M;
     ea.header = header;
@@ -733,7 +735,7 @@
     ea.item_problem = d_item_problem.ptr;
     ea.segment_rows = emFillSegmentRows();
     ea.subset_off = d_subset_off.ptr;
-    subsetExpandKernel<<<dim3(M), dim3(256), 0, st>>>(ea);
+    subsetExpandKernel<<<dim3(M), dim3(256), 0, ts>>>(ea);
     ok(hipGetLastError());
     ctx->spanEnd(span);
     ctx->stats.build_launches += 4;
diff --git a/rpvg_amd/engine.py b/rpvg_amd/engine.py
--- a/rpvg_amd/engine.py
+++ b/rpvg_amd/engine.py
@@ -35,6 +35,7 @@
         L.rpvg_amd_engine_stats_get.argtypes = [C.c_void_p, C.c_void_p]
         L.rpvg_amd_engine_stats_reset.argtypes = [C.c_void_p]
         L.rpvg_amd_engine_independent_stats_get.argtypes = [C.c_void_p, C.c_void_p]
+        L.rpvg_amd_engine_search_gate_stats_get.argtypes = [C.c_void_p, C.c_void_p]
         L.rpvg_amd_run_generators_after.restype = C.c_int
         L.rpvg_amd_run_generators_after.argtypes = [C.c_void_p, C.c_void_p, C.c_char_p, C.POINTER(CParams), C.POINTER(C.c_uint32)]
         L.rpvg_amd_host_threads.restype = C.c_int
@@ -98,6 +99,7 @@
         L.rpvg_amd_pipeline_result.argtypes = [C.c_void_p, C.c_int]
         L.rpvg_amd_pipeline_stats_get.argtypes = [C.c_void_p, C.c_void_p, C.POINTER(C.c_double)]
         L.rpvg_amd_pipeline_stats_reset.argtypes = [C.c_void_p]
+        L.rpvg_amd_pipeline_search_gate_stats_get.argtypes = [C.c_void_p, C.c_void_p]
         L.rpvg_amd_pipeline_completions.argtypes = [C.c_void_p, C.c_void_p, C.c_uint64, C.POINTER(C.c_uint64)]
         L.rpvg_amd_result_view.argtypes = [C.c_void_p, C.POINTER(CEstimatesView)]
         L.rpvg_amd_result_free.argtypes = [C.c_void_p]
@@ -155,6 +157,12 @@
         if lib().rpvg_amd_engine_independent_stats_get(self.handle, C.byref(s)) != 0:
             raise hip.EngineError(f"stats failed: {_err()}")
         return {n: int(getattr(s, n)) for n, _ in s._fields_}
+
+    def search_gate_stats(self) -> dict:
+        s = hip.CSearchGateStats()
+        if lib().rpvg_amd_engine_search_gate_stats_get(self.handle, C.byref(s)) != 0:
+            raise hip.EngineError(f"stats failed: {_err()}")
+        return s.as_dict()
 
     def reset_stats(self):
         if lib().rpvg_amd_engine_stats_reset(self.handle) != 0:
@@ -442,6 +450,12 @@
         out["worker_finish_ms_per_batch"], out["worker_estimate_ms_per_batch"], out["worker_idle_ms_per_batch"] = up[3] * 1e3, up[4] * 1e3, up[5] * 1e3
         return out
 
+    def search_gate_stats(self) -> dict:
+        s = hip.CSearchGateStats()
+        if lib().rpvg_amd_pipeline_search_gate_stats_get(self.handle, C.byref(s)) != 0:
+            raise hip.EngineError(f"pipeline stats failed: {_err()}")
+        return s.as_dict()
+
     def reset_stats(self):
         if lib().rpvg_amd_pipeline_stats_reset(self.handle) != 0:
             raise hip.EngineError(f"pipeline stats reset failed: {_err()}")
diff --git a/rpvg_amd/hip.py b/rpvg_amd/hip.py
--- a/rpvg_amd/hip.py
+++ b/rpvg_amd/hip.py
@@ -47,6 +47,7 @@
     "rpvg_hip_align_index_alignments_collapsed",
     "rpvg_hip_batch_rows_sizes", "rpvg_hip_batch_rows_get",
     "rpvg_hip_segment_sort_words",
+    "rpvg_hip_search_gate_stats_get",
 ]
 
 COMM_ID_BYTES = 128
@@ -101,6 +102,15 @@
                 ("set_posterior", C.POINTER(C.c_double)), ("set_abundance", C.POINTER(C.c_double))]
 
 
+class CSubsetEmView(C.Structure):
+    _fields_ = [("num_matrices", C.c_uint32), ("subset_off", C.POINTER(C.c_uint64)), ("weight", C.POINTER(C.c_double)),
+                ("path_off", C.POINTER(C.c_uint64)), ("path", C.POINTER(C.c_uint32)), ("col_off", C.POINTER(C.c_uint64)),
+                ("col_path", C.POINTER(C.c_uint32)), ("abundances", C.POINTER(C.c_double)), ("noise_count", C.POINTER(C.c_double)),
+                ("total_count", C.POINTER(C.c_double)), ("iterations", C.POINTER(C.c_uint32)), ("set_count", C.POINTER(C.c_uint32)),
+                ("cluster_noise_count", C.POINTER(C.c_double)), ("set_first", C.POINTER(C.c_uint32)), ("set_second", C.POINTER(C.c_uint32)),
+                ("set_posterior", C.POINTER(C.c_double)), ("set_abundance", C.POINTER(C.c_double))]
+
+
 class CIndependentSpec(C.Structure):
     _fields_ = [("num_clusters", C.c_uint32), ("matrix_off", C.c_void_p), ("group_size", C.c_uint32), ("column_counts", C.c_void_p),
                 ("log_freq", C.c_void_p), ("min_hap_prob", C.c_double), ("max_em_its", C.c_uint32), ("max_rel_em_conv", C.c_double),
@@ -124,6 +134,14 @@
 
 class CIndependentStats(C.Structure):
     _fields_ = [("calls_completed", C.c_uint64), ("draws", C.c_uint64), ("subsets", C.c_uint64)]
+
+
+class CSearchGateStats(C.Structure):
+    _fields_ = [("searches_gated", C.c_uint64), ("tile_releases", C.c_uint64), ("wait_host_ms", C.c_double), ("hold_host_ms", C.c_double),
+                ("hold_device_ms", C.c_double), ("hold_device_spans", C.c_uint64)]
+
+    def as_dict(self) -> dict:
+        return {name: getattr(self, name) for name, _ in self._fields_}
 
 
 def independent_limits() -> CIndependentLimits:
@@ -642,6 +660,48 @@
         finally:
             lib().rpvg_hip_subset_em_free(h)
 
+    def nested_subset_em(self, column_counts, min_rel_likelihood: float, min_hap_prob: float, max_em_its: int = 10000,
+                         max_rel_em_conv: float = 1e-3, collapse_precision: float = 0.0) -> dict:
+        cc = np.ascontiguousarray(column_counts, dtype=np.uint32)
+        h = C.c_void_p()
+        _check(lib().rpvg_hip_nested_subset_em(self.ctx.handle, self.batch.handle, self.handle, C.c_void_p(cc.ctypes.data if cc.size else None),
+                                               C.c_double(float(min_rel_likelihood)), C.c_double(float(min_hap_prob)), C.c_uint32(max_em_its),
+                                               C.c_double(float(max_rel_em_conv)), C.c_double(float(collapse_precision)), C.byref(h)),
+               "rpvg_hip_nested_subset_em")
+        try:
+            v = CSubsetEmView()
+            _check(lib().rpvg_hip_subset_em_get(h, C.byref(v)), "rpvg_hip_subset_em_get")
+            M = int(v.num_matrices)
+
+            def take(pointer, n, dtype):
+                if n == 0 or not pointer:
+                    return np.zeros(0, dtype=dtype)
+                return np.ctypeslib.as_array(pointer, shape=(n,)).copy()
+
+            out = {"num_matrices": M}
+            out["subset_off"] = take(v.subset_off, M + 1, np.uint64) if M else np.zeros(1, np.uint64)
+            S = int(out["subset_off"][-1])
+            out["path_off"] = take(v.path_off, S + 1, np.uint64) if S else np.zeros(1, np.uint64)
+            out["col_off"] = take(v.col_off, S + 1, np.uint64) if S else np.zeros(1, np.uint64)
+            L, Cn = int(out["path_off"][-1]), int(out["col_off"][-1])
+            out["weight"] = take(v.weight, S, np.float64)
+            out["path"] = take(v.path, L, np.uint32)
+            out["col_path"] = take(v.col_path, Cn, np.uint32)
+            out["abundances"] = take(v.abundances, Cn, np.float64)
+            out["noise_count"] = take(v.noise_count, S, np.float64)
+            out["total_count"] = take(v.total_count, S, np.float64)
+            out["iterations"] = take(v.iterations, S, np.uint32)
+            merged = bool(v.set_count)
+            out["set_count"] = take(v.set_count, M if merged else 0, np.uint32)
+            out["cluster_noise_count"] = take(v.cluster_noise_count, M if merged else 0, np.float64)
+            out["set_first"] = take(v.set_first, L if merged else 0, np.uint32)
+            out["set_second"] = take(v.set_second, L if merged else 0, np.uint32)
+            out["set_posterior"] = take(v.set_posterior, L if merged else 0, np.float64)
+            out["set_abundance"] = take(v.set_abundance, 2 * L if merged else 0, np.float64)
+            return out
+        finally:
+            lib().rpvg_hip_subset_em_free(h)
+
     def nested_independent_subset_em(self, matrix_off, group_size: int, min_hap_prob: float, generator_words, column_counts=None, log_freq=None,
                                      max_em_its: int = 10000, max_rel_em_conv: float = 1e-3, collapse_precision: float = 0.0,
                                      keep_draws: bool = False) -> dict:
@@ -1055,6 +1115,11 @@
         _check(lib().rpvg_hip_stats_get(self.handle, C.byref(s)), "rpvg_hip_stats_get")
         return s.as_dict()
 
+    def search_gate_stats(self) -> dict:
+        s = CSearchGateStats()
+        _check(lib().rpvg_hip_search_gate_stats_get(self.handle, C.byref(s)), "rpvg_hip_search_gate_stats_get")
+        return s.as_dict()
+
     def independent_stats(self) -> dict:
         s = CIndependentStats()
         _check(lib().rpvg_hip_independent_stats_get(self.handle, C.byref(s)), "rpvg_hip_independent_stats_get")
diff --git a/rpvg_amd/host/batch_pipeline.cpp b/rpvg_amd/host/batch_pipeline.cpp
--- a/rpvg_amd/host/batch_pipeline.cpp
+++ b/rpvg_amd/host/batch_pipeline.cpp
@@ -384,6 +384,18 @@
     }
 
     HipEngine::stats(engines, stats_out);
+}
+
+void BatchPipeline::searchGateStats(rpvg_hip_search_gate_stats * stats_out) const {
+
+    std::vector<const HipEngine *> engines;
+
+    for (auto & engine: worker_engines) {
+
+        engines.emplace_back(engine.get());
+    }
+
+    HipEngine::searchGateStats(engines, stats_out);
 }
 
 void BatchPipeline::resetStats() const {
diff --git a/rpvg_amd/host/batch_pipeline.hpp b/rpvg_amd/host/batch_pipeline.hpp
--- a/rpvg_amd/host/batch_pipeline.hpp
+++ b/rpvg_amd/host/batch_pipeline.hpp
@@ -37,6 +37,8 @@
 
         void stats(rpvg_hip_kernel_stats * stats_out) const;
         void resetStats() const;
+
+        void searchGateStats(rpvg_hip_search_gate_stats * stats_out) const;
 
         double meanUploadSeconds(uint64_t * batches_out = nullptr) const;
 
diff --git a/rpvg_amd/host/hip_engine.cpp b/rpvg_amd/host/hip_engine.cpp
--- a/rpvg_amd/host/hip_engine.cpp
+++ b/rpvg_amd/host/hip_engine.cpp
@@ -129,6 +129,31 @@
         stats_out->calls_completed += lane_stats.calls_completed;
         stats_out->draws += lane_stats.draws;
         stats_out->subsets += lane_stats.subsets;
+    }
+}
+
+void HipEngine::searchGateStats(const std::vector<const HipEngine *> & engines, rpvg_hip_search_gate_stats * stats_out) {
+
+    *stats_out = rpvg_hip_search_gate_stats{0, 0, 0, 0, 0, 0};
+
+    for (auto & engine: engines) {
+
+        std::vector<rpvg_hip_ctx *> contexts(1, engine->context);
+        const auto lane_contexts = engine->laneContexts();
+        contexts.insert(contexts.end(), lane_contexts.begin(), lane_contexts.end());
+
+        for (auto & ctx: contexts) {
+
+            rpvg_hip_search_gate_stats ctx_stats;
+            check(rpvg_hip_search_gate_stats_get(ctx, &ctx_stats), "rpvg_hip_search_gate_stats_get");
+
+            stats_out->searches_gated += ctx_stats.searches_gated;
+            stats_out->tile_releases += ctx_stats.tile_releases;
+            stats_out->wait_host_ms += ctx_stats.wait_host_ms;
+            stats_out->hold_host_ms += ctx_stats.hold_host_ms;
+            stats_out->hold_device_ms += ctx_stats.hold_device_ms;
+            stats_out->hold_device_spans += ctx_stats.hold_device_spans;
+        }
     }
 }
 
diff --git a/rpvg_amd/host/hip_engine.hpp b/rpvg_amd/host/hip_engine.hpp
--- a/rpvg_amd/host/hip_engine.hpp
+++ b/rpvg_amd/host/hip_engine.hpp
@@ -59,6 +59,8 @@
 
         void independentStats(rpvg_hip_independent_stats * stats_out) const;
 
+        static void searchGateStats(const std::vector<const HipEngine *> & engines, rpvg_hip_search_gate_stats * stats_out);
+
         static void stats(const std::vector<const HipEngine *> & engines, rpvg_hip_kernel_stats * stats_out);
 
         static int deviceCount();
diff --git a/rpvg_amd/host/runner_capi.cpp b/rpvg_amd/host/runner_capi.cpp
--- a/rpvg_amd/host/runner_capi.cpp
+++ b/rpvg_amd/host/runner_capi.cpp
@@ -343,6 +343,15 @@
     });
 }
 
+int rpvg_amd_engine_search_gate_stats_get(void * engine, rpvg_hip_search_gate_stats * stats_out) {
+
+    return guardedInt([&]() -> int {
+
+        HipEngine::searchGateStats(std::vector<const HipEngine *>(1, static_cast<Engine *>(engine)->hip.get()), stats_out);
+        return 0;
+    });
+}
+
 int rpvg_amd_engine_stats_reset(void * engine) {
 
     return guardedInt([&]() -> int {
@@ -1298,6 +1307,15 @@
             pipeline->pipeline->workerSeconds(mean_upload_seconds_out + 3, mean_upload_seconds_out + 4, mean_upload_seconds_out + 5);
         }
 
+        return 0;
+    });
+}
+
+int rpvg_amd_pipeline_search_gate_stats_get(void * pipeline_handle, rpvg_hip_search_gate_stats * stats_out) {
+
+    return guardedInt([&]() -> int {
+
+        static_cast<Pipeline *>(pipeline_handle)->pipeline->searchGateStats(stats_out);
         return 0;
     });
 }
```
